# LUP-LuftbildUmweltPlanung/UNet

Measured on AMD Instinct MI355X. Metric: 512x512 tiles/sec fwd+bwd (4-ch->5-class U-Net), higher is better.
Workload: dtype f32

## Files before the change

include/unet_hip.h:

```cpp
#ifndef UNET_HIP_H
#define UNET_HIP_H

#include <stddef.h>
#include <stdint.h>

#ifdef __cplusplus
extern "C" {
#endif

#define UNET_OK 0
#define UNET_E_BADARG (-1)
#define UNET_E_UNSUPPORTED (-2)
#define UNET_E_HIP (-3)

#define UNET_ABI_VERSION 8

int unet_abi_version(void);
const char* unet_last_error(void);

#define UNET_F32 0
#define UNET_BF16 1
typedef uint16_t unet_bf16;

typedef struct {
    int conv_splitk;
    int mfma_shape;
    int f32_big_tile;
    int bf16_big_tile;
    int t256_tiles_per_wg;
    int t256_sliver;
    int conv1x1_gemm;
    int wgrad_mfma_shape;
    int wgrad_bf16_k4;
    int wgrad_1x1;
    int wgrad_narrow;
    int plan_batch;
    int wgrad_wgs;
    int conv_smallcin;
    int conv_head1x1;
} unet_tuning;
void unet_tuning_default(unet_tuning* t);


#define UNET_CONV_RELU 1
#define UNET_CONV_MASK 4

#define UNET_CONV_FWD 0
#define UNET_CONV_DGRAD 1

typedef struct {
    const float* x; int x_cs, x_co;
    const float* wp;
    const float* bias;
    const float* res; int res_cs, res_co;
    const float* mask; int mask_cs, mask_co;
    float* y; int y_cs, y_co;
    int N, IH, IW, Cin;
    int OH, OW, Cout;
    int ks, stride;
    int kind, flags;
    float* colsum;
    float* colsumsq;
    int cout_begin, cout_count;
    long long wp_img_stride;
    int dtype;
    int y_f32;
    float* splitk_ws;
    size_t splitk_ws_floats;
    const unet_tuning* tuning;
    int pixel_shuffle;
    const void* ps_tail;
    int ps_tail_cs, ps_tail_co;
    int ps_tail_c, ps_tail_at;
} unet_conv_desc;

int unet_conv2d_colsum_rows(const unet_conv_desc* d);
int unet_conv2d(const unet_conv_desc* d, void* stream);
size_t unet_conv2d_splitk_workspace(const unet_conv_desc* d);
int unet_conv2d_variant(const unet_conv_desc* d);
size_t unet_pack_weights_size(int Cout, int Cin, int ks, int mode);
int unet_pack_weights(const float* w, float* wp, int Cout, int Cin, int ks, int mode, void* stream);
int unet_pack_weights_strided(const float* w, long long so, long long sr, float* wp, int O, int R, void* stream);
size_t unet_pack_weights_size_bf16(int Cout, int Cin, int ks, int mode);
int unet_pack_weights_bf16(const float* w, unet_bf16* wp, int Cout, int Cin, int ks, int mode, void* stream);
typedef struct {
    const float* w;
    void* wp;
    int Cout, Cin, ks, mode;
    const float* out_scale;
} unet_pack_job;
size_t unet_pack_batch_table_bytes(int njobs);
int unet_pack_batch_build(const unet_pack_job* jobs, int njobs, int dtype, void* table_host, unsigned* total_blocks);
int unet_pack_batch_run(const void* table_dev, int njobs, unsigned total_blocks, int dtype, void* stream);
typedef struct {
    const float* x; int x_cs, x_co;
    const float* dy; int dy_cs, dy_co;
    float* dw;
    float* dbias;
    int N, IH, IW, Cin, OH, OW, Cout, ks, stride;
    float* workspace; size_t workspace_floats;
    int accumulate;
    int dtype;
    const unet_tuning* tuning;
} unet_wgrad_desc;
size_t unet_conv2d_wgrad_workspace(const unet_wgrad_desc* d);
int unet_conv2d_wgrad(const unet_wgrad_desc* d, void* stream);

int unet_bn_stats_rows(long long P);
int unet_bn_stats(const float* x, int x_cs, int x_co, long long P, int C, float* partial, void* stream);
int unet_bn_finalize(const float* psum, const float* psumsq, int rows, long long count, int C,
                     const float* gamma, const float* beta, float* running_mean, float* running_var,
                     float momentum, float eps,
                     float* scale, float* shift, float* save_mean, float* save_invstd, long long* batches_tracked, void* stream);
int unet_bn_eval_coeffs(const float* gamma, const float* beta, const float* running_mean, const float* running_var,
                        float eps, int C, float* scale, float* shift, void* stream);
int unet_affine_act(const float* x, int x_cs, int x_co, const float* scale, const float* shift,
                    const float* x2, int x2_cs, int x2_co, const float* scale2, const float* shift2,
                    float* y, int y_cs, int y_co, long long P, int C, int relu, void* stream);
int unet_bn_bwd_reduce(const float* dout, int d_cs, int d_co, const float* out, int o_cs, int o_co,
                       const float* x, int x_cs, int x_co, const float* mean, const float* invstd,
                       long long P, int C, float* partial, void* stream);
int unet_bn_bwd_finalize(const float* partial, int rows, long long count, int C,
                         float* dgamma, float* dbeta, float* c1, float* c2, void* stream);
int unet_bn_bwd_apply(const float* dout, int d_cs, int d_co, const float* out, int o_cs, int o_co,
                      const float* x, int x_cs, int x_co, const float* mean, const float* invstd,
                      const float* gamma, const float* c1, const float* c2,
                      float* dx, int dx_cs, int dx_co, float* gout, int g_cs, int g_co, int g_accumulate,
                      long long P, int C, void* stream);

int unet_maxpool3x3s2(const float* x, int x_cs, int x_co, float* y, int y_cs, int y_co, uint8_t* idx,
                      int N, int IH, int IW, int C, int OH, int OW, void* stream);
int unet_maxpool3x3s2_bwd(const float* dy, int dy_cs, int dy_co, const uint8_t* idx, float* dx, int dx_cs, int dx_co,
                          int N, int IH, int IW, int C, int OH, int OW, int accumulate, void* stream);
int unet_avgpool2_ceil(const float* x, int x_cs, int x_co, float* y, int y_cs, int y_co,
                       int N, int IH, int IW, int C, int OH, int OW, void* stream);
int unet_avgpool2_ceil_bwd(const float* dy, int dy_cs, int dy_co, float* dx, int dx_cs, int dx_co,
                           int N, int IH, int IW, int C, int OH, int OW, int accumulate, void* stream);

int unet_shuffle_blur(const float* yc, int yc_cs, int yc_co, float* X, int X_cs, int X_co,
                      int N, int h, int w, int Cu, int do_blur, void* stream);
int unet_shuffle_blur_bwd(const float* dX, int dX_cs, int dX_co, const float* yc, int yc_cs, int yc_co,
                          float* dyc, int dyc_cs, int dyc_co, int N, int h, int w, int Cu, int do_blur, void* stream);
int unet_shuffle_bwd_xmask(const float* dX, int dX_cs, int dX_co, const float* X, int X_cs, int X_co,
                           float* dyc, int dyc_cs, int dyc_co, int N, int h, int w, int Cu, void* stream);
int unet_resize_nearest(const float* x, int x_cs, int x_co, float* y, int y_cs, int y_co,
                        int N, int IH, int IW, int OH, int OW, int C, void* stream);
int unet_resize_nearest_bwd(const float* dy, int dy_cs, int dy_co, float* dx, int dx_cs, int dx_co,
                            int N, int IH, int IW, int OH, int OW, int C, void* stream);
int unet_nchw_to_nhwc(const float* x, float* y, int y_cs, int y_co, int N, int C, int H, int W, void* stream);
int unet_nhwc_to_nchw(const float* x, int x_cs, int x_co, float* y, int N, int C, int H, int W, void* stream);
int unet_copy_slice(const float* x, int x_cs, int x_co, float* y, int y_cs, int y_co, long long P, int C,
                    int accumulate, void* stream);
int unet_relu_mask(const float* g, int g_cs, int g_co, const float* ref, int r_cs, int r_co,
                   float* y, int y_cs, int y_co, long long P, int C, void* stream);
int unet_colsum(const float* x, int x_cs, int x_co, long long P, int C, float* out, float* workspace, void* stream);
size_t unet_colsum_workspace(long long P, int C);
int unet_dot(const float* x, int x_cs, int x_co, const float* y, int y_cs, int y_co, long long P, int C, float* out,
             float* workspace, void* stream);

size_t unet_ce_workspace(long long P);
int unet_ce_fwd(const float* z, int z_cs, int z_co, const int64_t* target, const float* weight, long long P, int C,
                float* loss , float* denom , float* workspace, void* stream);
int unet_ce_fwd_parts(const float* z, int z_cs, int z_co, const int64_t* target, const float* weight, long long P, int C,
                      float* numden , float* workspace, void* stream);
int unet_ce_bwd(const float* z, int z_cs, int z_co, const int64_t* target, const float* weight, long long P, int C,
                const float* denom, float gscale, float* dz, int dz_cs, int dz_co, void* stream);
int unet_ce_fwd_pw(const float* z, int z_cs, int z_co, const int64_t* target, const float* pixel_weight, long long P, int C,
                   float* loss , float* denom , float* workspace, void* stream);
int unet_ce_fwd_parts_pw(const float* z, int z_cs, int z_co, const int64_t* target, const float* pixel_weight, long long P, int C,
                         float* numden , float* workspace, void* stream);
int unet_ce_bwd_pw(const float* z, int z_cs, int z_co, const int64_t* target, const float* pixel_weight, long long P, int C,
                   const float* denom, float gscale, float* dz, int dz_cs, int dz_co, void* stream);
int unet_focal_fwd(const float* z, int z_cs, int z_co, const int64_t* target, const float* weight, long long P, int C, float gamma,
                   float* loss , float* workspace, void* stream);
int unet_focal_bwd(const float* z, int z_cs, int z_co, const int64_t* target, const float* weight, long long P, int C, float gamma,
                   float gscale, float* dz, int dz_cs, int dz_co, void* stream);
size_t unet_dice_workspace(int B, long long HW, int C);
int unet_dice_fwd(const float* z, int z_cs, int z_co, const int64_t* target, int B, long long HW, int C, float smooth, int square_in_union,
                  long long mean_div, float* loss , float* coef , float* workspace, void* stream);
int unet_dice_bwd(const float* z, int z_cs, int z_co, const int64_t* target, int B, long long HW, int C, int square_in_union,
                  const float* coef, float gscale, float* dz, int dz_cs, int dz_co, void* stream);
size_t unet_combined_workspace(int B, long long HW, int C);
int unet_combined_fwd(const float* z, int z_cs, int z_co, const int64_t* target, const float* weight, int B, long long HW, int C, float gamma,
                      float smooth, int square_in_union, long long mean_div, float* terms , float* coef , float* workspace,
                      void* stream);
int unet_combined_bwd(const float* z, int z_cs, int z_co, const int64_t* target, const float* weight, int B, long long HW, int C, float gamma,
                      int square_in_union, const float* coef, float fscale, float dscale, float* dz, int dz_cs, int dz_co, void* stream);
int unet_regloss_fwd(const float* z, int z_cs, int z_co, const float* target, long long P, int kind, float beta,
                     float* loss , float* workspace, void* stream);
int unet_regloss_bwd(const float* z, int z_cs, int z_co, const float* target, long long P, int kind, float beta, float gscale,
                     float* dz, int dz_cs, int dz_co, void* stream);
int unet_softmax_argmax(const float* z, int z_cs, int z_co, int N, int H, int W, int C,
                        float* probs_nchw , int64_t* argmax , void* stream);

int unet_row_softmax(const float* x, int x_cs, int x_co, float* y, int y_cs, int y_co, long long P, int C, void* stream);
int unet_row_softmax_bwd(const float* y, int y_cs, int y_co, const float* dy, int dy_cs, int dy_co,
                         float* dx, int dx_cs, int dx_co, long long P, int C, void* stream);

int unet_adam_step(float* p, const float* g, float* m, float* v, const uint8_t* code, long long n,
                   const float* lr , float mom, float sqr_mom, float eps, float wd, int step,
                   float grad_scale, void* stream);

int unet_adam_hyper_floats(void);
int unet_adam_fill_hyper(float* hyper_host, const float* lr , float mom, float sqr_mom, float eps, float wd, int step,
                         float grad_scale);
int unet_adam_step_dev(float* p, const float* g, float* m, float* v, const uint8_t* code, long long n,
                       const float* hyper_dev, void* stream);

int unet_mosaic_accumulate(const float* probs_nchw, int C, int th, int tw, float* mosaic ,
                           int32_t* count , int MH, int MW, int y0, int x0, void* stream);
int unet_mosaic_finalize(float* mosaic, const int32_t* count, int C, int MH, int MW, uint8_t* argmax, void* stream);
int unet_mosaic_accumulate_weighted(const float* probs_nchw, int C, int th, int tw, const float* wy, const float* wx, float* mosaic,
                                    int32_t* count, float* wsum, int MH, int MW, int y0, int x0, void* stream);

#define UNET_RASTER_U8 0
#define UNET_RASTER_U16 1
#define UNET_RASTER_I16 2
#define UNET_RASTER_I32 3
#define UNET_RASTER_F32 4
int unet_raster_nodata_zero(void* raster, int rtype, int bands, long long pixels, double nodata, void* stream);
int unet_window_nonzero(const void* raster, int rtype, int bands, long long band_stride, int row_stride, const int32_t* windows, int n,
                        int th, int tw, unsigned long long* counts, void* stream);
int unet_window_gather(const void* src, int rtype, int bands, long long src_stride, long long band_stride, int row_stride,
                       const int32_t* windows, int n, int th, int tw, int div255_twice, void* x, int x_cs, int x_co, int dtype, void* stream);
int unet_mosaic_accumulate_windows(const float* z, int z_cs, int z_co, int C, int th, int tw, const int32_t* windows, int n, int origin_y,
                                   int origin_x, int mode, float* mosaic, int32_t* count, int MH, int MW, int row_lo, int row_hi,
                                   void* stream);
int unet_mosaic_finalize_rows(float* mosaic, const int32_t* count, int C, int MH, int MW, int row0, int nrows, uint8_t* argmax,
                              const float* fill_host, void* stream);
int unet_mosaic_accumulate_windows_weighted(const float* z, int z_cs, int z_co, int C, int th, int tw, const int32_t* windows, int n,
                                            int origin_y, int origin_x, int mode, float* mosaic, int32_t* count, int MH, int MW, int row_lo,
                                            int row_hi, const float* wy, const float* wx, float* wsum, void* stream);
int unet_mosaic_finalize_rows_weighted(float* mosaic, const int32_t* count, const float* wsum, int C, int MH, int MW, int row0, int nrows,
                                       uint8_t* argmax, const float* fill_host, void* stream);
// ... 122 lines not shown
```

unet_amd/_lib.py:

```python
from __future__ import annotations

import ctypes as C
import os
import re
from pathlib import Path

import torch

_HERE = Path(__file__).resolve().parent
LIB_PATH = _HERE / "lib" / "libunet_hip.so"
HEADER = _HERE.parent / "include" / "unet_hip.h"

UNET_OK = 0
CONV_RELU = 1
CONV_MASK = 4
CONV_FWD = 0
CONV_DGRAD = 1
F32 = 0
BF16 = 1

c_float_p = C.POINTER(C.c_float)
vp = C.c_void_p


class Tuning(C.Structure):
    _fields_ = [(n, C.c_int) for n in ("conv_splitk", "mfma_shape", "f32_big_tile", "bf16_big_tile", "t256_tiles_per_wg", "t256_sliver",
                                       "conv1x1_gemm", "wgrad_mfma_shape", "wgrad_bf16_k4", "wgrad_1x1", "wgrad_narrow", "plan_batch", "wgrad_wgs", "conv_smallcin", "conv_head1x1")]

    @classmethod
    def default(cls, **over) -> "Tuning":
        t = cls()
        lib.unet_tuning_default(C.byref(t))
        for k, v in over.items():
            if k not in dict(cls._fields_):
                raise KeyError(f"unet_tuning has no field {k!r}")
            setattr(t, k, int(v))
        return t


class ConvDesc(C.Structure):
    _fields_ = [
        ("x", vp), ("x_cs", C.c_int), ("x_co", C.c_int),
        ("wp", vp),
        ("bias", vp),
        ("res", vp), ("res_cs", C.c_int), ("res_co", C.c_int),
        ("mask", vp), ("mask_cs", C.c_int), ("mask_co", C.c_int),
        ("y", vp), ("y_cs", C.c_int), ("y_co", C.c_int),
        ("N", C.c_int), ("IH", C.c_int), ("IW", C.c_int), ("Cin", C.c_int),
        ("OH", C.c_int), ("OW", C.c_int), ("Cout", C.c_int),
        ("ks", C.c_int), ("stride", C.c_int),
        ("kind", C.c_int), ("flags", C.c_int),
        ("colsum", vp),
        ("colsumsq", vp),
        ("cout_begin", C.c_int), ("cout_count", C.c_int),
        ("wp_img_stride", C.c_longlong),
        ("dtype", C.c_int), ("y_f32", C.c_int),
        ("splitk_ws", vp), ("splitk_ws_floats", C.c_size_t),
        ("tuning", C.POINTER(Tuning)),
        ("pixel_shuffle", C.c_int),
        ("ps_tail", vp), ("ps_tail_cs", C.c_int), ("ps_tail_co", C.c_int), ("ps_tail_c", C.c_int), ("ps_tail_at", C.c_int),
    ]


class WgradDesc(C.Structure):
    _fields_ = [
        ("x", vp), ("x_cs", C.c_int), ("x_co", C.c_int),
        ("dy", vp), ("dy_cs", C.c_int), ("dy_co", C.c_int),
        ("dw", vp),
        ("dbias", vp),
        ("N", C.c_int), ("IH", C.c_int), ("IW", C.c_int), ("Cin", C.c_int),
        ("OH", C.c_int), ("OW", C.c_int), ("Cout", C.c_int), ("ks", C.c_int), ("stride", C.c_int),
        ("workspace", vp), ("workspace_floats", C.c_size_t),
        ("accumulate", C.c_int),
        ("dtype", C.c_int),
        ("tuning", C.POINTER(Tuning)),
    ]


PIXEL_MAX_PROGS, PIXEL_MAX_OPS, PIXEL_MAX_RECTS, BLUR_MAX_IMAGES, BLUR_MAX_KSIZE = 8, 8, 32, 16, 31
PIXEL_BRIGHTNESS_CONTRAST, PIXEL_GAMMA, PIXEL_GAUSS_NOISE, PIXEL_FILL_RECTS, PIXEL_CHANNEL_DROP, PIXEL_CHANNEL_PERMUTE = 1, 2, 3, 4, 5, 6
PIXEL_PER_CHANNEL = 0x100


class PixelOp(C.Structure):
    _fields_ = [("code", C.c_uint32), ("u0", C.c_uint32), ("u1", C.c_uint32), ("f0", C.c_float), ("f1", C.c_float)]


class PixelProg(C.Structure):
    _fields_ = [("image", C.c_uint32), ("nops", C.c_uint32), ("nrects", C.c_uint32), ("reserved", C.c_uint32),
                ("ops", PixelOp * PIXEL_MAX_OPS), ("rects", (C.c_uint16 * 4) * PIXEL_MAX_RECTS)]


class RectSet(C.Structure):
    _fields_ = [("image", C.c_uint32), ("nrects", C.c_uint32), ("rects", (C.c_uint16 * 4) * PIXEL_MAX_RECTS)]


FIELD_MAX_IMAGES, FIELD_MAX_CELLS, ELASTIC_MAX_IMAGES, ELASTIC_MAX_KSIZE = 16, 16, 64, 401
FIELD_DENSE, FIELD_GRID, FIELD_OPTICAL = 0, 1, 2


class FieldImage(C.Structure):
    _fields_ = [("fired", C.c_int32), ("pre", C.c_float * 6), ("optical", C.c_float * 3), ("nodes", (C.c_float * (FIELD_MAX_CELLS + 1)) * 2)]


class ElasticImage(C.Structure):
    _fields_ = [("key0", C.c_uint32), ("key1", C.c_uint32), ("alpha", C.c_float), ("fired", C.c_int32), ("same_dxdy", C.c_int32)]


class PackJob(C.Structure):
    _fields_ = [("w", vp), ("wp", vp), ("Cout", C.c_int), ("Cin", C.c_int), ("ks", C.c_int), ("mode", C.c_int), ("out_scale", vp)]


def declared_symbols() -> list[str]:
    txt = HEADER.read_text()
    txt = re.sub(r"/\*.*?\*/", "", txt, flags=re.S)
    return sorted(set(re.findall(r"\b(unet_[a-z0-9_]+)\s*\(", txt)))


def _load() -> C.CDLL:
    if not LIB_PATH.exists():
        raise ImportError(
            f"{LIB_PATH} not found: build it with `python -m unet_amd.build` (hipcc --offload-arch=gfx950). "
            "The MI355X path has no CPU fallback.")
    lib = C.CDLL(str(LIB_PATH))
    missing = [s for s in declared_symbols() if not hasattr(lib, s)]
    if missing:
        raise ImportError(f"libunet_hip.so does not export: {missing}")
    return lib


lib = _load()

i, ll, f, sz = C.c_int, C.c_longlong, C.c_float, C.c_size_t
_sig = {
    "unet_abi_version": (i, []),
    "unet_last_error": (C.c_char_p, []),
    "unet_conv2d_colsum_rows": (i, [C.POINTER(ConvDesc)]),
    "unet_conv2d": (i, [C.POINTER(ConvDesc), vp]),
    "unet_conv2d_variant": (i, [C.POINTER(ConvDesc)]),
    "unet_conv2d_splitk_workspace": (sz, [C.POINTER(ConvDesc)]),
    "unet_tuning_default": (None, [C.POINTER(Tuning)]),
    "unet_pack_batch_table_bytes": (sz, [i]),
    "unet_pack_batch_build": (i, [C.POINTER(PackJob), i, i, vp, C.POINTER(C.c_uint)]),
    "unet_pack_batch_run": (i, [vp, i, C.c_uint, i, vp]),
    "unet_pack_weights_size": (sz, [i, i, i, i]),
    "unet_pack_weights": (i, [vp, vp, i, i, i, i, vp]),
    "unet_pack_weights_strided": (i, [vp, ll, ll, vp, i, i, vp]),
    "unet_row_softmax": (i, [vp, i, i, vp, i, i, ll, i, vp]),
    "unet_row_softmax_bwd": (i, [vp, i, i, vp, i, i, vp, i, i, ll, i, vp]),
    "unet_conv2d_wgrad_workspace": (sz, [C.POINTER(WgradDesc)]),
    "unet_conv2d_wgrad": (i, [C.POINTER(WgradDesc), vp]),
    "unet_bn_stats_rows": (i, [ll]),
    "unet_bn_stats": (i, [vp, i, i, ll, i, vp, vp]),
    "unet_bn_finalize": (i, [vp, vp, i, ll, i, vp, vp, vp, vp, f, f, vp, vp, vp, vp, vp, vp]),
    "unet_bn_eval_coeffs": (i, [vp, vp, vp, vp, f, i, vp, vp, vp]),
    "unet_affine_act": (i, [vp, i, i, vp, vp, vp, i, i, vp, vp, vp, i, i, ll, i, i, vp]),
    "unet_bn_bwd_reduce": (i, [vp, i, i, vp, i, i, vp, i, i, vp, vp, ll, i, vp, vp]),
    "unet_bn_bwd_finalize": (i, [vp, i, ll, i, vp, vp, vp, vp, vp]),
    "unet_bn_bwd_apply": (i, [vp, i, i, vp, i, i, vp, i, i, vp, vp, vp, vp, vp, vp, i, i, vp, i, i, i, ll, i, vp]),
    "unet_maxpool3x3s2": (i, [vp, i, i, vp, i, i, vp, i, i, i, i, i, i, vp]),
    "unet_maxpool3x3s2_bwd": (i, [vp, i, i, vp, vp, i, i, i, i, i, i, i, i, i, vp]),
    "unet_avgpool2_ceil": (i, [vp, i, i, vp, i, i, i, i, i, i, i, i, vp]),
    "unet_avgpool2_ceil_bwd": (i, [vp, i, i, vp, i, i, i, i, i, i, i, i, i, vp]),
    "unet_shuffle_blur": (i, [vp, i, i, vp, i, i, i, i, i, i, i, vp]),
    "unet_shuffle_blur_bwd": (i, [vp, i, i, vp, i, i, vp, i, i, i, i, i, i, i, vp]),
    "unet_shuffle_bwd_xmask": (i, [vp, i, i, vp, i, i, vp, i, i, i, i, i, i, vp]),
    "unet_resize_nearest": (i, [vp, i, i, vp, i, i, i, i, i, i, i, i, vp]),
    "unet_resize_nearest_bwd": (i, [vp, i, i, vp, i, i, i, i, i, i, i, i, vp]),
    "unet_nchw_to_nhwc": (i, [vp, vp, i, i, i, i, i, i, vp]),
    "unet_nhwc_to_nchw": (i, [vp, i, i, vp, i, i, i, i, vp]),
    "unet_copy_slice": (i, [vp, i, i, vp, i, i, ll, i, i, vp]),
    "unet_relu_mask": (i, [vp, i, i, vp, i, i, vp, i, i, ll, i, vp]),
    "unet_colsum": (i, [vp, i, i, ll, i, vp, vp, vp]),
    "unet_colsum_workspace": (sz, [ll, i]),
    "unet_dot": (i, [vp, i, i, vp, i, i, ll, i, vp, vp, vp]),
    "unet_ce_workspace": (sz, [ll]),
    "unet_ce_fwd": (i, [vp, i, i, vp, vp, ll, i, vp, vp, vp, vp]),
    "unet_ce_fwd_parts": (i, [vp, i, i, vp, vp, ll, i, vp, vp, vp]),
    "unet_ce_bwd": (i, [vp, i, i, vp, vp, ll, i, vp, f, vp, i, i, vp]),
    "unet_ce_fwd_pw": (i, [vp, i, i, vp, vp, ll, i, vp, vp, vp, vp]),
    "unet_ce_fwd_parts_pw": (i, [vp, i, i, vp, vp, ll, i, vp, vp, vp]),
    "unet_ce_bwd_pw": (i, [vp, i, i, vp, vp, ll, i, vp, f, vp, i, i, vp]),
    "unet_focal_fwd": (i, [vp, i, i, vp, vp, ll, i, f, vp, vp, vp]),
    "unet_focal_bwd": (i, [vp, i, i, vp, vp, ll, i, f, f, vp, i, i, vp]),
    "unet_dice_workspace": (sz, [i, ll, i]),
    "unet_dice_fwd": (i, [vp, i, i, vp, i, ll, i, f, i, ll, vp, vp, vp, vp]),
    "unet_dice_bwd": (i, [vp, i, i, vp, i, ll, i, i, vp, f, vp, i, i, vp]),
    "unet_combined_workspace": (sz, [i, ll, i]),
    "unet_combined_fwd": (i, [vp, i, i, vp, vp, i, ll, i, f, f, i, ll, vp, vp, vp, vp]),
    "unet_combined_bwd": (i, [vp, i, i, vp, vp, i, ll, i, f, i, vp, f, f, vp, i, i, vp]),
    "unet_regloss_fwd": (i, [vp, i, i, vp, ll, i, f, vp, vp, vp]),
    "unet_regloss_bwd": (i, [vp, i, i, vp, ll, i, f, f, vp, i, i, vp]),
    "unet_softmax_argmax": (i, [vp, i, i, i, i, i, i, vp, vp, vp]),
    "unet_adam_step": (i, [vp, vp, vp, vp, vp, ll, c_float_p, f, f, f, f, i, f, vp]),
    "unet_adam_hyper_floats": (i, []),
    "unet_adam_fill_hyper": (i, [c_float_p, c_float_p, f, f, f, f, i, f]),
    "unet_adam_step_dev": (i, [vp, vp, vp, vp, vp, ll, vp, vp]),
    "unet_mosaic_accumulate": (i, [vp, i, i, i, vp, vp, i, i, i, i, vp]),
    "unet_mosaic_finalize": (i, [vp, vp, i, i, i, vp, vp]),
    "unet_raster_nodata_zero": (i, [vp, i, i, ll, C.c_double, vp]),
    "unet_window_nonzero": (i, [vp, i, i, ll, i, vp, i, i, i, vp, vp]),
    "unet_window_gather": (i, [vp, i, i, ll, ll, i, vp, i, i, i, i, vp, i, i, i, vp]),
    "unet_mosaic_accumulate_windows": (i, [vp, i, i, i, i, i, vp, i, i, i, i, vp, vp, i, i, i, i, vp]),
    "unet_tiff_lzw_decode": (ll, [vp, ll, vp, ll]),
    "unet_tiff_packbits_decode": (ll, [vp, ll, vp, ll]),
    "unet_mosaic_finalize_rows": (i, [vp, vp, i, i, i, i, i, vp, c_float_p, vp]),
    "unet_tiles_stage": (i, [vp, i, i, i, i, i, i, C.c_ulonglong, C.c_ulonglong, vp, vp]),
    "unet_mask_stage": (i, [vp, i, i, i, i, C.c_ulonglong, C.c_ulonglong, vp, i, vp]),
    "unet_dice_counts": (i, [vp, vp, ll, i, vp, vp]),
    "unet_warp_affine": (i, [vp, vp, i, i, i, i, c_float_p, i, i, f, vp]),
    "unet_warp_affine_mask": (i, [vp, vp, i, i, i, i, c_float_p, i, C.c_double, vp]),
    "unet_warp_field": (i, [vp, vp, i, i, i, i, i, C.POINTER(FieldImage), vp, i, i, i, i, f, vp]),
    "unet_warp_field_mask": (i, [vp, vp, i, i, i, i, i, C.POINTER(FieldImage), vp, i, i, i, C.c_double, vp]),
    "unet_elastic_field": (i, [vp, vp, i, i, i, C.POINTER(ElasticImage), c_float_p, i, vp]),
    "unet_pixel_ops": (i, [vp, i, i, i, i, vp, i, vp]),
    "unet_fill_rects_mask": (i, [vp, i, i, i, i, vp, i, C.c_double, vp]),
    "unet_blur_separable": (i, [vp, vp, i, i, i, i, C.POINTER(C.c_int), c_float_p, vp]),
    "unet_window_gather_oriented": (i, [vp, i, i, ll, ll, i, vp, i, i, i, i, vp, i, i, i, i, vp]),
    "unet_nchw_to_nhwc_oriented": (i, [vp, vp, i, i, i, i, i, i, i, i, vp]),
    "unet_tta_accumulate": (i, [vp, i, i, i, i, i, i, i, i, i, vp, i, i, vp, vp, vp]),
    "unet_mosaic_accumulate_weighted": (i, [vp, i, i, i, vp, vp, vp, vp, vp, i, i, i, i, vp]),
    "unet_mosaic_accumulate_windows_weighted": (i, [vp, i, i, i, i, i, vp, i, i, i, i, vp, vp, i, i, i, i, vp, vp, vp, vp]),
    "unet_mosaic_finalize_rows_weighted": (i, [vp, vp, vp, i, i, i, i, i, vp, c_float_p, vp]),
    "unet_cc_tile_shape": (None, [C.POINTER(C.c_int), C.POINTER(C.c_int)]),
    "unet_cc_label": (i, [vp, i, i, i, vp, vp, vp]),
    "unet_cc_sizes": (i, [vp, i, i, vp, vp]),
    "unet_sieve_round": (i, [vp, vp, i, i, i, ll, i, vp, vp, vp, vp, vp]),
    "unet_majority_filter": (i, [vp, vp, i, i, i, i, vp]),
    "unet_postprocess_counters": (i, [vp, C.POINTER(C.c_int32), vp]),
    "unet_edt_workspace": (sz, [i, i, i]),
    "unet_border_edt": (i, [vp, i, i, i, i, i, vp, vp, vp]),
    "unet_border_weight": (i, [vp, vp, vp, i, f, C.c_double, ll, vp, vp]),
}
for _n in ("bn_stats", "affine_act", "bn_bwd_reduce", "bn_bwd_apply", "maxpool3x3s2", "maxpool3x3s2_bwd", "avgpool2_ceil",
           "avgpool2_ceil_bwd", "shuffle_blur", "shuffle_blur_bwd", "shuffle_bwd_xmask", "resize_nearest", "resize_nearest_bwd", "nchw_to_nhwc", "copy_slice", "ce_bwd", "ce_bwd_pw", "focal_bwd",
           "dice_bwd", "combined_bwd"):
    _sig[f"unet_{_n}_bf16"] = _sig[f"unet_{_n}"]
for _n in ("pack_weights_strided", "row_softmax", "row_softmax_bwd", "relu_mask", "dot"):
    _sig[f"unet_{_n}_bf16"] = _sig[f"unet_{_n}"]
_sig["unet_sa_fused_supported"] = (i, [i, i])
_sig["unet_sa_pack_elems"] = (sz, [i, i])
_sig["unet_sa_pack_bf16"] = (i, [vp, i, i, i, i, i, vp, vp])
_sig["unet_sa_fwd_bf16"] = (i, [vp, i, i, i, i, i, vp, vp, i, i, vp, vp])
_sig["unet_sa_rowdot_bf16"] = (i, [vp, i, i, vp, i, i, i, i, i, vp, vp])
_sig["unet_sa_bwd_bf16"] = (i, [vp, i, i, i, i, i, vp, i, i, vp, vp, vp, vp, vp, vp, vp])
_sig["unet_cast_slice_bf16"] = (i, [vp, i, i, vp, i, i, ll, i, vp])
_sig["unet_pack_weights_size_bf16"] = _sig["unet_pack_weights_size"]
_sig["unet_pack_weights_bf16"] = _sig["unet_pack_weights"]

for _name, (_res, _args) in _sig.items():
    _fn = getattr(lib, _name)
    _fn.restype = _res
    _fn.argtypes = _args

_undeclared = [s for s in declared_symbols() if s not in _sig]
if _undeclared:
    raise ImportError(f"ctypes signatures missing for: {_undeclared}")

if lib.unet_abi_version() != 8:
    raise ImportError("libunet_hip.so ABI version mismatch; rebuild with `python -m unet_amd.build --force`")


class UnetHipError(RuntimeError):
    pass


def check(rc: int, what: str = "") -> None:
    if rc != UNET_OK:
        msg = lib.unet_last_error().decode(errors="replace")
        raise UnetHipError(f"{what}: rc={rc}: {msg}")
```

unet_amd/csrc/conv_bf16.hip:

```cpp

#include "conv_common.h"

namespace {

using namespace unetconv;

typedef __bf16 bf16x8 __attribute__((ext_vector_type(8)));
typedef __bf16 bf16x4 __attribute__((ext_vector_type(4)));
typedef float f32x4 __attribute__((ext_vector_type(4)));
typedef unsigned short u16;

__device__ __forceinline__ f32x4 ld_bf16x4(const u16* p) {
    const uint2 u = *reinterpret_cast<const uint2*>(p);
    return (f32x4){__uint_as_float(u.x << 16), __uint_as_float(u.x & 0xffff0000u), __uint_as_float(u.y << 16), __uint_as_float(u.y & 0xffff0000u)};
}
__device__ __forceinline__ void st_bf16x4(u16* p, f32x4 v) {
    const bf16x4 h = {(__bf16)v[0], (__bf16)v[1], (__bf16)v[2], (__bf16)v[3]};
    *reinterpret_cast<uint2*>(p) = __builtin_bit_cast(uint2, h);
}

template <int TW, int MT, int NT, int WM, int WN, int HIT>
__global__ __launch_bounds__(WM* WN * 64, HIT == 4 ? 3 : 2) void conv_bf16_kernel(const KArgs a, const int y_f32) {
    constexpr int BM = WM * MT * 32, BN = WN * NT * 32, TH = BM / TW, NTH = WM * WN * 64;
    constexpr int M16 = 2 * MT, N16 = 2 * NT;
// ... 634 lines not shown
#pragma unroll
                        for (int m = 0; m < MH; ++m) v[m] += ld4(resb + (size_t)pidx[m] * a.res_cs + cc);
                    }
                    if (relu) {
#pragma unroll
                        for (int m = 0; m < MH; ++m)
#pragma unroll
                            for (int q = 0; q < 4; ++q) v[m][q] = fmaxf(v[m][q], 0.f);
                    }
                    if (maskb != nullptr) {
#pragma unroll
                        for (int m = 0; m < MH; ++m) {
                            const f32x4 mv = ld4(maskb + (size_t)pidx[m] * a.mask_cs + cc);
#pragma unroll
                            for (int q = 0; q < 4; ++q) v[m][q] = mv[q] > 0.f ? v[m][q] : 0.f;
                        }
                    }
                    float* yb = a.y + (a.cps ? (size_t)blockIdx.y * a.slab : (size_t)0) + img_pix * a.y_cs + a.y_co;
#pragma unroll
                    for (int m = 0; m < MH; ++m)
                        if (cvalid && pval[m]) *reinterpret_cast<f32x4*>(yb + (size_t)pidx[m] * a.y_cs + c4) = v[m];
                }
            }
        } else {
            f32x4 bvn[NL];
#pragma unroll
            for (int n = 0; n < NL; ++n) {
                const int c4 = n0c + TILE_COL(n) + 4 * kq;
                bvn[n] = (f32x4){0.f, 0.f, 0.f, 0.f};
                if (a.bias != nullptr) {
                    if (c4 + 3 < a.Cout) bvn[n] = *reinterpret_cast<const f32x4*>(a.bias + c4);
                    else {
#pragma unroll
                        for (int q = 0; q < 4; ++q) bvn[n][q] = (c4 + q < a.Cout) ? a.bias[c4 + q] : 0.f;
                    }
                }
            }
            int pidx2[2][MH / 2];
            bool pval2[2][MH / 2];
#pragma unroll
            for (int h = 0; h < 2; ++h)
#pragma unroll
                for (int j = 0; j < MH / 2; ++j) {
                    const int pix = (wm * M16 + ((h * MH + 2 * j + (kq & 1)) ^ (r * MH))) * 16 + l15;
                    const int oy = oy0c + pix / TW, ox = ox0c + pix % TW;
                    pval2[h][j] = oy < a.OH && ox < a.OW;
                    pidx2[h][j] = pval2[h][j] ? (oy * a.OW + ox) : 0;
                }
#pragma unroll
            for (int h = 0; h < 2; ++h) {
#pragma unroll
            for (int n = 0; n < NL; ++n) {
                if (n == NF && h != 0) continue;
                const int c8 = n0c + TILE_COL(n) + 8 * (kq >> 1);
                const int cc8 = c8 < a.n_end ? c8 : 0;
#pragma unroll
                for (int m = 0; m < MH; ++m) acc[h * MH + m][n] += bvn[n];
                if (resb != nullptr) {
                    uint4 rr[MH / 2];
#pragma unroll
                    for (int j = 0; j < MH / 2; ++j) rr[j] = *reinterpret_cast<const uint4*>(resb + (size_t)pidx2[h][j] * a.res_cs + cc8);
#pragma unroll
                    for (int j = 0; j < MH / 2; ++j) {
                        const auto s0 = __builtin_amdgcn_permlane16_swap(rr[j].x, rr[j].z, false, false);
                        const auto s1 = __builtin_amdgcn_permlane16_swap(rr[j].y, rr[j].w, false, false);
                        acc[h * MH + 2 * j][n] += unpack(s0[0], s1[0]);
                        acc[h * MH + 2 * j + 1][n] += unpack(s0[1], s1[1]);
                    }
                }
                if (relu) {
#pragma unroll
                    for (int m = 0; m < MH; ++m)
#pragma unroll
                        for (int q = 0; q < 4; ++q) acc[h * MH + m][n][q] = fmaxf(acc[h * MH + m][n][q], 0.f);
                }
                if (maskb != nullptr) {
                    uint4 rr[MH / 2];
#pragma unroll
                    for (int j = 0; j < MH / 2; ++j) rr[j] = *reinterpret_cast<const uint4*>(maskb + (size_t)pidx2[h][j] * a.mask_cs + cc8);
#pragma unroll
                    for (int j = 0; j < MH / 2; ++j) {
                        const auto s0 = __builtin_amdgcn_permlane16_swap(rr[j].x, rr[j].z, false, false);
                        const auto s1 = __builtin_amdgcn_permlane16_swap(rr[j].y, rr[j].w, false, false);
                        const f32x4 m0 = unpack(s0[0], s1[0]), m1 = unpack(s0[1], s1[1]);
#pragma unroll
                        for (int q = 0; q < 4; ++q) {
                            acc[h * MH + 2 * j][n][q] = m0[q] > 0.f ? acc[h * MH + 2 * j][n][q] : 0.f;
                            acc[h * MH + 2 * j + 1][n][q] = m1[q] > 0.f ? acc[h * MH + 2 * j + 1][n][q] : 0.f;
                        }
                    }
                }
            }
            }
            const __amdgpu_buffer_rsrc_t rsy = __builtin_amdgcn_make_buffer_rsrc(reinterpret_cast<u16*>(a.y) + img_pix * a.y_cs + a.y_co, 0,
                                                                                  __builtin_amdgcn_readfirstlane(a.OH * a.OW * a.y_cs * 2), 0x00020000);
#pragma unroll
            for (int h = 0; h < 2; ++h) {
#pragma unroll
            for (int j = 0; j < MH / 2; ++j) {
#pragma unroll
                for (int n = 0; n < NL; ++n) {
                    if (n == NF && h != 0) continue;
                    const int c8 = n0c + TILE_COL(n) + 8 * (kq >> 1);
                    const bool cvalid8 = c8 < a.n_end;
                    const f32x4 va = acc[h * MH + 2 * j][n], vb = acc[h * MH + 2 * j + 1][n];
                    const bf16x4 x_ = {(__bf16)va[0], (__bf16)va[1], (__bf16)va[2], (__bf16)va[3]};
                    const bf16x4 y_ = {(__bf16)vb[0], (__bf16)vb[1], (__bf16)vb[2], (__bf16)vb[3]};
                    const uint2 xu = __builtin_bit_cast(uint2, x_), yu = __builtin_bit_cast(uint2, y_);
                    const auto s0 = __builtin_amdgcn_permlane16_swap(xu.x, yu.x, false, false);
                    const auto s1 = __builtin_amdgcn_permlane16_swap(xu.y, yu.y, false, false);
                    typedef unsigned v4u __attribute__((ext_vector_type(4)));
                    const unsigned vo = (cvalid8 && pval2[h][j]) ? (unsigned)(pidx2[h][j] * a.y_cs + c8) * 2u : OOB;
                    __builtin_amdgcn_raw_buffer_store_b128((v4u){s0[0], s1[0], s0[1], s1[1]}, rsy, (int)vo, 0, 0);
                }
            }
            }
        }
#ifdef UNET_STAMPS
        ste_ += STAMP() - se0_;
#endif
        if (!more_tiles) break;
#pragma unroll
        for (int m = 0; m < M16; ++m)
#pragma unroll
            for (int n = 0; n < N16; ++n) acc[m][n] = (f32x4){0.f, 0.f, 0.f, 0.f};
    }
    wait_cnt<0, true>(b0, hreg);
#undef T256_MFMA
#undef T256_LOAD_HALO
#undef T256_STORE_HALO
#undef T256_STORE_HALO_T
#undef T256_SETUP
#undef MOFF
#undef TOFF
#undef TILE_COL
#ifdef UNET_STAMPS
    if (g_stamps != nullptr && tid == 0) {
        asm volatile("s_waitcnt vmcnt(0)" ::: "memory");
        unsigned long long* o = g_stamps + (size_t)blockIdx.x * 24;
#pragma unroll
        for (int i = 0; i < 10; ++i) o[8 + i] = stwt_[i];
        o[0] = st0_; o[1] = st1_; o[2] = stl_; o[3] = STAMP(); o[4] = stw_; o[5] = stb_; o[6] = (unsigned long long)__builtin_amdgcn_s_memrealtime();
        o[7] = 1; o[18] = ste_; o[19] = (unsigned long long)(tend - wg * tpw);
    }
#endif
}

#ifdef UNET_STAMPS
extern "C" int unet_debug_set_stamps(unsigned long long* buf) {
    return hipMemcpyToSymbol(HIP_SYMBOL(g_stamps), &buf, sizeof(buf)) == hipSuccess ? 0 : -3;
}
#endif


template <int NTOT, int TW, typename T, bool SLV = false>
int launch_t256n(const Plan& p, int y_f32, hipStream_t st) {
    const int ntiles = p.k.mtiles * p.k.ntn;
    int tpw = p.tune.t256_tiles_per_wg > 0 ? p.tune.t256_tiles_per_wg : ntiles / 2048;
    tpw = tpw < 1 ? 1 : (tpw > 16 ? 16 : tpw);
    dim3 grid = p.grid;
    grid.x = (unsigned)unet::roundup(unet::cdiv(ntiles, tpw), 8);
    return launch_big_lds<conv_bf16_t256_kernel<NTOT, TW, T, SLV>>(grid, dim3(256), (size_t)2 * (256 / TW + 2) * (TW + 2) * T256_ROWB, st, p.k, y_f32, tpw, p.bn);
}

template <int TW, typename T>
int launch_t256_tiles(const Plan& p, int tiles, int y_f32, hipStream_t st) {
    switch (tiles) {
        case 8: return launch_t256n<8, TW, T>(p, y_f32, st);
        case 7: return launch_t256n<7, TW, T>(p, y_f32, st);
        case 6: return launch_t256n<6, TW, T>(p, y_f32, st);
        case 5: return launch_t256n<5, TW, T>(p, y_f32, st);
        case 4: return launch_t256n<4, TW, T>(p, y_f32, st);
        case 3: return launch_t256n<3, TW, T>(p, y_f32, st);
        case 2: return launch_t256n<2, TW, T>(p, y_f32, st);
        case 1: return launch_t256n<1, TW, T>(p, y_f32, st);
    }
    unet::set_error("conv: %d channel tiles in the 256-pixel tile", tiles);
    return (int)UNET_E_UNSUPPORTED;
}

template <typename T>
int launch_t256(const Plan& p, int y_f32, hipStream_t st) {
    const int cols = p.k.n_end - p.k.n_base, nblk = p.k.ntn, full = p.bn / 16;
    const int last_tiles = (cols - (nblk - 1) * p.bn + 15) / 16;
    auto one = [&](const Plan& q, int tiles) {
        if constexpr (sizeof(T) == 4) {
            const int last_w = (q.k.n_end - q.k.n_base) - (q.k.ntn - 1) * q.bn - (tiles - 1) * 16;
            if (q.tune.t256_sliver && tiles == 7 && q.tw == 32 && last_w >= 1 && last_w <= 4) return launch_t256n<7, 32, T, true>(q, y_f32, st);
        }
        if (q.tw == 32) return launch_t256_tiles<32, T>(q, tiles, y_f32, st);
        if (q.tw == 16) return launch_t256_tiles<16, T>(q, tiles, y_f32, st);
        unet::set_error("conv: tile width %d in the 256-pixel tile", q.tw);
        return (int)UNET_E_UNSUPPORTED;
    };
    if (nblk == 1 || last_tiles == full) return one(p, nblk == 1 ? last_tiles : full);
    Plan q = p;
    q.k.ntn = nblk - 1; q.k.n_end = p.k.n_base + (nblk - 1) * p.bn;
    int rc = one(q, full);
    if (rc != UNET_OK) return rc;
    q = p;
    q.k.ntn = 1; q.k.n_base = p.k.n_base + (nblk - 1) * p.bn;
    return one(q, last_tiles);
}

__global__ void pack_weights_bf16_kernel(const float* __restrict__ w, u16* __restrict__ wp, int Cout, int Cin, int T, int mode, int nchunks,
                                         int outPad, size_t total) {
    for (size_t i = (size_t)blockIdx.x * blockDim.x + threadIdx.x; i < total; i += (size_t)gridDim.x * blockDim.x)
        wp[i] = __builtin_bit_cast(u16, (__bf16)bf16_image_value(w, Cout, Cin, T, mode, nchunks, outPad, i));
}

__global__ void pack_weights_strided_bf16_kernel(const u16* __restrict__ w, long long so, long long sr, u16* __restrict__ wp, int O, int R,
                                                 int outPad, size_t total) {
    for (size_t i = (size_t)blockIdx.x * blockDim.x + threadIdx.x; i < total; i += (size_t)gridDim.x * blockDim.x) {
        const int rr = (int)(i & 31);
        const size_t j = i >> 5;
        const int o = (int)(j % outPad), r = (int)(j / outPad) * 32 + rr;
        wp[i] = (o < O && r < R) ? w[(long long)o * so + (long long)r * sr] : (u16)0;
    }
}

struct IgemmBf16 {
    template <int TW, int MT, int NT, int WM, int WN, int HIT>
    static int launch(const Plan& p, int y_f32, hipStream_t st) {
        return launch_big_lds<conv_bf16_kernel<TW, MT, NT, WM, WN, HIT>>(p.grid, dim3(WM * WN * 64), p.lds_bytes, st, p.k, y_f32);
    }
};

}

int unetconv::conv_generic_bf16(const Plan& p, int y_f32, hipStream_t st) { return launch_generic<IgemmBf16>(p, y_f32, st); }

int unetconv::conv_t256(const Plan& p0, int dtype, int y_f32, hipStream_t st) {
    Plan p = p0;
    p.k.sliver = p.k.taps[0].dy[0] > 0 ? 1 : 0;
    if (dtype == UNET_BF16) return launch_t256<unsigned short>(p, y_f32, st);
    p.k.fold = 0;
    return launch_t256<float>(p, 1, st);
}

extern "C" size_t unet_pack_weights_size_bf16(int Cout, int Cin, int ks, int mode) {
    const int T = ks * ks;
    const int red = mode == 1 ? Cout : Cin, out = mode == 1 ? Cin : Cout;
    return bf16_image_elems(red, unet::roundup(out, 128), T);
}

extern "C" int unet_pack_weights_strided_bf16(const unet_bf16* w, long long so, long long sr, unet_bf16* wp, int O, int R, void* stream) {
    UNET_CHECK_ARG(w && wp && O > 0 && R > 0, "pack_weights_strided_bf16: bad args");
    const int outPad = unet::roundup(O, 128);
    const size_t total = bf16_image_elems(R, outPad, 1);
    hipLaunchKernelGGL(pack_weights_strided_bf16_kernel, dim3(unet::ew_grid((long long)total, 256)), dim3(256), 0, (hipStream_t)stream, w, so, sr, wp,
                       O, R, outPad, total);
    UNET_CHECK_LAUNCH();
    return UNET_OK;
}

extern "C" int unet_pack_weights_bf16(const float* w, unet_bf16* wp, int Cout, int Cin, int ks, int mode, void* stream) {
    UNET_CHECK_ARG(w && wp, "pack_weights_bf16: null pointer");
    UNET_CHECK_ARG((ks == 1 || ks == 3) && (mode == 0 || mode == 1 || (mode == 2 && ks == 1 && Cout % 64 == 0)) && Cout > 0 && Cin > 0, "pack_weights_bf16: bad args");
    const int T = ks * ks;
    const int red = mode == 1 ? Cout : Cin, out = mode == 1 ? Cin : Cout;
    const int nchunks = unet::cdiv(red, KCB), outPad = unet::roundup(out, 128);
    const size_t total = bf16_image_elems(red, outPad, T);
    hipLaunchKernelGGL(pack_weights_bf16_kernel, dim3(unet::ew_grid((long long)total, 256)), dim3(256), 0, (hipStream_t)stream, w, wp, Cout,
                       Cin, T, mode, nchunks, outPad, total);
    UNET_CHECK_LAUNCH();
    return UNET_OK;
}
```

unet_amd/csrc/conv_common.h:

```cpp
#pragma once
#include "common.h"

namespace unetconv {

constexpr int KC = 16;
constexpr int LDK = 20;
constexpr int KCB = 32;
constexpr int LDKB = 24;

struct TapSet {
    int n;
    int min_dy, min_dx;
    int ext_y, ext_x;
    int py, px;
    signed char dy[9], dx[9], widx[9];
    unsigned long long dpack, wpack;
};

struct KArgs {
    const float* x; const float* wp; const float* bias; const float* res; const float* mask;
    float* y; float* colsum; float* colsumsq;
    int x_cs, x_co, res_cs, res_co, mask_cs, mask_co, y_cs, y_co;
    int N, IH, IW, Cin, Cin4;
    int OH, OW, Cout;
    int S, OS, TSH, TSW, tiles_y, tiles_x, ntn;
    int nchunks, coutPad, flags, mtiles;
    int n_base, n_end;
    int fold;
    int sliver;
    const float* wsl;
    long long wp_stride;
    int cps;
    long long slab;
    TapSet taps[4];
};

__host__ __device__ inline bool f32_sliver(int out) { return out >= 16 && (out & 15) != 0 && (out & 15) <= 4; }
__host__ __device__ inline size_t f32_image_elems(int red, int out, int T) {
    const int nchunks = (red + 15) / 16, outPad = (out + 127) / 128 * 128;
    return (size_t)T * nchunks * outPad * 16 + (f32_sliver(out) ? (size_t)T * nchunks * 64 : 0);
}
__device__ inline float f32_sliver_value(const float* __restrict__ w, int Cout, int Cin, int T, int mode, int nchunks, size_t i) {
    const int pos = (int)(i & 15), j = (int)((i >> 4) & 3);
    const int chunk = (int)((i >> 6) % nchunks), tap = (int)((i >> 6) / nchunks);
    const int red = mode == 0 ? Cin : Cout, out = mode == 0 ? Cout : Cin;
    const bool tail = (red & 15) != 0 && chunk == nchunks - 1;
    const int r = chunk * 16 + (tail ? (4 * (pos & 3) + (pos >> 2)) : pos);
    const int o = (out & ~15) + j;
    if (r >= red || o >= out) return 0.f;
    return mode == 0 ? w[((size_t)o * Cin + r) * T + tap] : w[((size_t)r * Cin + o) * T + tap];
}

__host__ __device__ inline bool bf16_fold_tail(int red, int T) { return T == 9 && (red & 31) != 0 && (red & 31) <= 8; }
__host__ __device__ inline size_t bf16_image_elems(int red, int out_pad, int T) {
    return (size_t)(T * ((red + 31) / 32) + (bf16_fold_tail(red, T) ? 3 : 0)) * out_pad * 32;
}
__host__ __device__ inline int ps_filter_of(int q, int Cout) { const int nf = Cout >> 2; return 4 * (q % nf) + q / nf; }
__device__ inline float bf16_image_value(const float* __restrict__ w, int Cout, int Cin, int T, int mode, int nchunks, int outPad, size_t i) {
    const int rr = (int)(i & 31);
    size_t j = i >> 5;
    const int o = (int)(j % outPad);
    const int slab = (int)(j / outPad);
    const int red = mode == 1 ? Cout : Cin;
    int tap, r;
    if (slab < T * nchunks) {
        tap = slab / nchunks;
        r = (slab % nchunks) * 32 + rr;
    } else {
        tap = 4 * (slab - T * nchunks) + (rr >> 3);
        r = (nchunks - 1) * 32 + (rr & 7);
        if (tap >= T) return 0.f;
    }
    if (r >= red) return 0.f;
    if (mode == 2) return o < Cout ? w[((size_t)ps_filter_of(o, Cout) * Cin + r) * T + tap] : 0.f;
    if (mode == 0) return o < Cout ? w[((size_t)o * Cin + r) * T + tap] : 0.f;
    return o < Cin ? w[((size_t)r * Cin + o) * T + tap] : 0.f;
}

typedef float v4f __attribute__((ext_vector_type(4)));
typedef unsigned long long u64;
__device__ __forceinline__ u64 sgpr_ptr(const void* p) {
    const u64 b = reinterpret_cast<u64>(p);
    const unsigned lo = __builtin_amdgcn_readfirstlane((unsigned)b), hi = __builtin_amdgcn_readfirstlane((unsigned)(b >> 32));
    return ((u64)hi << 32) | lo;
}
template <int TSTR, int N>
__device__ __forceinline__ void gld_b(v4f (&d)[N], unsigned voff, const char* p) {
    static_assert(N == 2 || N == 4, "operand-B tiles per wave");
    const u64 s0 = sgpr_ptr(p);
    if constexpr (N == 2) {
        asm volatile("s_nop 4\n\tglobal_load_dwordx4 %0, %2, %3\n\tglobal_load_dwordx4 %1, %2, %3 offset:%4"
                     : "=&v"(d[0]), "=&v"(d[1]) : "v"(voff), "s"(s0), "n"(TSTR));
    } else {
        const u64 s1 = sgpr_ptr(p + 2 * TSTR);
        asm volatile("s_nop 4\n\tglobal_load_dwordx4 %0, %4, %5\n\tglobal_load_dwordx4 %1, %4, %5 offset:%7\n\t"
                     "global_load_dwordx4 %2, %4, %6\n\tglobal_load_dwordx4 %3, %4, %6 offset:%7"
                     : "=&v"(d[0]), "=&v"(d[1]), "=&v"(d[2]), "=&v"(d[3]) : "v"(voff), "s"(s0), "s"(s1), "n"(TSTR));
    }
}
template <int TSTR, int N>
__device__ __forceinline__ void gld_bl(v4f (&d)[N], unsigned voff, unsigned voff_last, const char* p) {
    static_assert(N == 2 || N == 4, "operand-B tiles per wave");
    const u64 s0 = sgpr_ptr(p);
    if constexpr (N == 2) {
        asm volatile("s_nop 4\n\tglobal_load_dwordx4 %0, %2, %4\n\tglobal_load_dwordx4 %1, %3, %4 offset:%5"
                     : "=&v"(d[0]), "=&v"(d[1]) : "v"(voff), "v"(voff_last), "s"(s0), "n"(TSTR));
    } else {
        const u64 s1 = sgpr_ptr(p + 2 * TSTR);
        asm volatile("s_nop 4\n\tglobal_load_dwordx4 %0, %4, %6\n\tglobal_load_dwordx4 %1, %4, %6 offset:%8\n\t"
                     "global_load_dwordx4 %2, %4, %7\n\tglobal_load_dwordx4 %3, %5, %7 offset:%8"
                     : "=&v"(d[0]), "=&v"(d[1]), "=&v"(d[2]), "=&v"(d[3]) : "v"(voff), "v"(voff_last), "s"(s0), "s"(s1), "n"(TSTR));
    }
}
template <int N>
__device__ __forceinline__ void gld_halo(v4f (&h)[N], const unsigned (&vo)[N], const void* p, bool fetch) {
    static_assert(N == 4 || N == 6 || N == 10, "halo items per thread");
    const u64 sb = sgpr_ptr(p);
    const u64 on = sgpr_ptr(reinterpret_cast<const void*>(fetch ? ~0ull : 0ull));
    u64 sv;
    if constexpr (N == 4) {
        asm volatile("s_and_saveexec_b64 %[sv], %[on]\n\ts_nop 4\n\t"
                     "global_load_dwordx4 %[h0], %[o0], %[sb]\n\tglobal_load_dwordx4 %[h1], %[o1], %[sb]\n\t"
                     "global_load_dwordx4 %[h2], %[o2], %[sb]\n\tglobal_load_dwordx4 %[h3], %[o3], %[sb]\n\t"
                     "s_mov_b64 exec, %[sv]"
                     : [h0] "+v"(h[0]), [h1] "+v"(h[1]), [h2] "+v"(h[2]), [h3] "+v"(h[3]), [sv] "=&s"(sv)
                     : [o0] "v"(vo[0]), [o1] "v"(vo[1]), [o2] "v"(vo[2]), [o3] "v"(vo[3]), [sb] "s"(sb), [on] "s"(on)
                     : "scc");
    } else if constexpr (N == 6) {
        asm volatile("s_and_saveexec_b64 %[sv], %[on]\n\ts_nop 4\n\t"
                     "global_load_dwordx4 %[h0], %[o0], %[sb]\n\tglobal_load_dwordx4 %[h1], %[o1], %[sb]\n\t"
                     "global_load_dwordx4 %[h2], %[o2], %[sb]\n\tglobal_load_dwordx4 %[h3], %[o3], %[sb]\n\t"
                     "global_load_dwordx4 %[h4], %[o4], %[sb]\n\tglobal_load_dwordx4 %[h5], %[o5], %[sb]\n\t"
                     "s_mov_b64 exec, %[sv]"
                     : [h0] "+v"(h[0]), [h1] "+v"(h[1]), [h2] "+v"(h[2]), [h3] "+v"(h[3]), [h4] "+v"(h[4]), [h5] "+v"(h[5]), [sv] "=&s"(sv)
                     : [o0] "v"(vo[0]), [o1] "v"(vo[1]), [o2] "v"(vo[2]), [o3] "v"(vo[3]), [o4] "v"(vo[4]), [o5] "v"(vo[5]), [sb] "s"(sb), [on] "s"(on)
                     : "scc");
    } else {
        asm volatile("s_and_saveexec_b64 %[sv], %[on]\n\ts_nop 4\n\t"
                     "global_load_dwordx4 %[h0], %[o0], %[sb]\n\tglobal_load_dwordx4 %[h1], %[o1], %[sb]\n\t"
                     "global_load_dwordx4 %[h2], %[o2], %[sb]\n\tglobal_load_dwordx4 %[h3], %[o3], %[sb]\n\t"
                     "global_load_dwordx4 %[h4], %[o4], %[sb]\n\tglobal_load_dwordx4 %[h5], %[o5], %[sb]\n\t"
                     "global_load_dwordx4 %[h6], %[o6], %[sb]\n\tglobal_load_dwordx4 %[h7], %[o7], %[sb]\n\t"
                     "global_load_dwordx4 %[h8], %[o8], %[sb]\n\tglobal_load_dwordx4 %[h9], %[o9], %[sb]\n\t"
                     "s_mov_b64 exec, %[sv]"
                     : [h0] "+v"(h[0]), [h1] "+v"(h[1]), [h2] "+v"(h[2]), [h3] "+v"(h[3]), [h4] "+v"(h[4]), [h5] "+v"(h[5]),
                       [h6] "+v"(h[6]), [h7] "+v"(h[7]), [h8] "+v"(h[8]), [h9] "+v"(h[9]), [sv] "=&s"(sv)
                     : [o0] "v"(vo[0]), [o1] "v"(vo[1]), [o2] "v"(vo[2]), [o3] "v"(vo[3]), [o4] "v"(vo[4]), [o5] "v"(vo[5]),
                       [o6] "v"(vo[6]), [o7] "v"(vo[7]), [o8] "v"(vo[8]), [o9] "v"(vo[9]), [sb] "s"(sb), [on] "s"(on)
                     : "scc");
    }
}
__device__ __forceinline__ void gld_halo4_sl(v4f (&h)[4], const unsigned (&vo)[4], const void* p, bool fetch, v4f& sl, unsigned vosl,
                                             const void* psl, u64 msl) {
    const u64 sb = sgpr_ptr(p), sbl = sgpr_ptr(psl);
    const u64 on = sgpr_ptr(reinterpret_cast<const void*>(fetch ? ~0ull : 0ull));
    const u64 ms = sgpr_ptr(reinterpret_cast<const void*>(msl));
    u64 sv;
    asm volatile("s_and_saveexec_b64 %[sv], %[on]\n\ts_nop 4\n\t"
                 "global_load_dwordx4 %[h0], %[o0], %[sb]\n\tglobal_load_dwordx4 %[h1], %[o1], %[sb]\n\t"
                 "global_load_dwordx4 %[h2], %[o2], %[sb]\n\tglobal_load_dwordx4 %[h3], %[o3], %[sb]\n\t"
                 "s_and_b64 exec, exec, %[ms]\n\ts_nop 0\n\t"
                 "global_load_dwordx4 %[sl], %[osl], %[sbl]\n\t"
                 "s_mov_b64 exec, %[sv]"
                 : [h0] "+v"(h[0]), [h1] "+v"(h[1]), [h2] "+v"(h[2]), [h3] "+v"(h[3]), [sl] "+v"(sl), [sv] "=&s"(sv)
                 : [o0] "v"(vo[0]), [o1] "v"(vo[1]), [o2] "v"(vo[2]), [o3] "v"(vo[3]), [osl] "v"(vosl), [sb] "s"(sb), [sbl] "s"(sbl),
                   [on] "s"(on), [ms] "s"(ms)
                 : "scc");
}
__device__ __forceinline__ void wait_loads_sl(v4f (&b)[4], v4f (&h)[4], v4f& sl) {
    asm volatile("s_waitcnt vmcnt(0)" : "+v"(b[0]), "+v"(b[1]), "+v"(b[2]), "+v"(b[3]), "+v"(h[0]), "+v"(h[1]), "+v"(h[2]), "+v"(h[3]), "+v"(sl));
}
template <int NB, int NH>
__device__ __forceinline__ void wait_loads(v4f (&b)[NB], v4f (&h)[NH]) {
    static_assert((NB == 2 || NB == 4) && (NH == 4 || NH == 6 || NH == 10), "register groups");
#define UNET_H4 "+v"(h[0]), "+v"(h[1]), "+v"(h[2]), "+v"(h[3])
#define UNET_H6 UNET_H4, "+v"(h[4]), "+v"(h[5])
#define UNET_H10 UNET_H4, "+v"(h[4]), "+v"(h[5]), "+v"(h[6]), "+v"(h[7]), "+v"(h[8]), "+v"(h[9])
    if constexpr (NB == 4 && NH == 6) asm volatile("s_waitcnt vmcnt(0)" : "+v"(b[0]), "+v"(b[1]), "+v"(b[2]), "+v"(b[3]), UNET_H6);
    else if constexpr (NB == 2 && NH == 6) asm volatile("s_waitcnt vmcnt(0)" : "+v"(b[0]), "+v"(b[1]), UNET_H6);
    else if constexpr (NB == 2 && NH == 4) asm volatile("s_waitcnt vmcnt(0)" : "+v"(b[0]), "+v"(b[1]), UNET_H4);
    else if constexpr (NB == 2) asm volatile("s_waitcnt vmcnt(0)" : "+v"(b[0]), "+v"(b[1]), UNET_H10);
    else if constexpr (NH == 4) asm volatile("s_waitcnt vmcnt(0)" : "+v"(b[0]), "+v"(b[1]), "+v"(b[2]), "+v"(b[3]), UNET_H4);
    else asm volatile("s_waitcnt vmcnt(0)" : "+v"(b[0]), "+v"(b[1]), "+v"(b[2]), "+v"(b[3]), UNET_H10);
#undef UNET_H4
#undef UNET_H6
#undef UNET_H10
}

struct Plan {
    KArgs k;
    int tw, bm, bn, hit, nparity, mf, max_hpix;
    size_t lds_bytes;
    dim3 grid;
    int splits, cp;
    size_t ws_floats;
    unet_tuning tune;
};


__device__ __forceinline__ float ld_act(const float* p) { return *p; }
__device__ __forceinline__ float ld_act(const unsigned short* p) { return __uint_as_float((unsigned)*p << 16); }
__device__ __forceinline__ void st_act(float* p, float v) { *p = v; }
__device__ __forceinline__ void st_act(unsigned short* p, float v) { *p = __builtin_bit_cast(unsigned short, (__bf16)v); }

template <auto Kern, typename... Args>
int launch_big_lds(dim3 grid, dim3 block, size_t lds_bytes, hipStream_t st, const Args&... args) {
    static unsigned long long configured = 0;
    if (unet::first_use_on_device(&configured))
        UNET_CHECK_HIP(hipFuncSetAttribute((const void*)Kern, hipFuncAttributeMaxDynamicSharedMemorySize, 160 * 1024));
    hipLaunchKernelGGL(Kern, grid, block, lds_bytes, st, args...);
    UNET_CHECK_LAUNCH();
    return UNET_OK;
}

template <typename K, int TW, int HIT>
int launch_bn(const Plan& p, int y_f32, hipStream_t st) {
    if (p.bm == 64) {
        if (p.bn == 64) return K::template launch<TW, 1, 1, 2, 2, HIT>(p, y_f32, st);
        return K::template launch<TW, 1, 2, 2, 2, HIT>(p, y_f32, st);
    }
    switch (p.bn) {
        case 32: return K::template launch<TW, 1, 1, 4, 1, HIT>(p, y_f32, st);
        case 64: return K::template launch<TW, 2, 1, 2, 2, HIT>(p, y_f32, st);
        default: return K::template launch<TW, 2, 2, 2, 2, HIT>(p, y_f32, st);
    }
}
template <typename K, int HIT>
int launch_tw(const Plan& p, int y_f32, hipStream_t st) {
    switch (p.tw) {
        case 32: return launch_bn<K, 32, HIT>(p, y_f32, st);
        case 16: return launch_bn<K, 16, HIT>(p, y_f32, st);
        default: return launch_bn<K, 8, HIT>(p, y_f32, st);
    }
}
template <typename K>
int launch_generic(const Plan& p, int y_f32, hipStream_t st) {
    if (p.bm == 256 || p.hit == 6) {
        unet::set_error("conv: inconsistent plan (the 256-pixel tile / halo item count 6 on the generic kernels)");
        return UNET_E_UNSUPPORTED;
    }
    return p.hit == 10 ? launch_tw<K, 10>(p, y_f32, st) : launch_tw<K, 4>(p, y_f32, st);
}

int conv_generic_f32(const Plan& p, hipStream_t st);
int conv_generic_bf16(const Plan& p, int y_f32, hipStream_t st);
int conv_t256(const Plan& p, int dtype, int y_f32, hipStream_t st);
int splitk_reduce(const unet_conv_desc* d, const Plan& p, hipStream_t st);
bool conv_smallk_applies(const unet_conv_desc* d);
int conv_smallk(const unet_conv_desc* d, hipStream_t st);
bool conv_smallcin_applies(const unet_conv_desc* d);
int conv_smallcin(const unet_conv_desc* d, hipStream_t st);
bool conv_head1x1_applies(const unet_conv_desc* d);
int conv_head1x1(const unet_conv_desc* d, hipStream_t st);
bool conv_gemm1x1_applies(const unet_conv_desc* d);
int conv_gemm1x1(const unet_conv_desc* d, hipStream_t st);
int conv_gemm1x1_ps_check(const unet_conv_desc* d);

}
```

unet_amd/csrc/conv_dispatch.hip:

```cpp
#include <stdlib.h>

#include "conv_common.h"

namespace unetconv {
static int env_int(const char* name, int dflt) {
    const char* e = getenv(name);
    return (e != nullptr && e[0] != 0) ? atoi(e) : dflt;
}
const unet_tuning& tuning_defaults() {
    static const unet_tuning t = [] {
        unet_tuning v;
        v.conv_splitk = env_int("UNET_CONV_SPLITK", 1);
        v.mfma_shape = 16;
        v.f32_big_tile = 1;
        v.bf16_big_tile = 1;
        v.t256_tiles_per_wg = 0;
        v.t256_sliver = env_int("UNET_T256_SLIVER", 1);
        v.conv1x1_gemm = env_int("UNET_CONV1X1_GEMM", 0);
        v.wgrad_mfma_shape = 32;
        v.wgrad_bf16_k4 = 1;
        v.wgrad_1x1 = 1;
        v.wgrad_narrow = 1;
        v.plan_batch = 0;
        v.wgrad_wgs = env_int("UNET_WGRAD_WGS", 0);
        v.conv_smallcin = env_int("UNET_CONV_SMALLCIN", 1);
        v.conv_head1x1 = env_int("UNET_CONV_HEAD1X1", 1);
        return v;
    }();
    return t;
}
}

extern "C" void unet_tuning_default(unet_tuning* t) {
    if (t != nullptr) *t = unetconv::tuning_defaults();
}

namespace {

using namespace unetconv;

int make_plan(const unet_conv_desc* d, Plan* p, int kc, int vec, int mf, int big_tile, int splitk, int plan_batch) {
    UNET_CHECK_ARG(d != nullptr, "conv: null desc");
    UNET_CHECK_ARG(d->x && d->wp && d->y, "conv: null tensor pointer");
    UNET_CHECK_ARG(d->ks == 1 || d->ks == 3, "conv: ks must be 1 or 3 (got %d)", d->ks);
    UNET_CHECK_ARG(d->stride == 1 || d->stride == 2, "conv: stride must be 1 or 2 (got %d)", d->stride);
    UNET_CHECK_ARG(!(d->ks == 1 && d->stride != 1), "conv: 1x1 stride 2 unsupported");
    UNET_CHECK_ARG(d->N > 0 && d->IH > 0 && d->IW > 0 && d->OH > 0 && d->OW > 0 && d->Cin > 0 && d->Cout > 0, "conv: bad dims");
    UNET_CHECK_ARG(unet::slice_ok_v(d->x_cs, d->x_co, d->Cin, vec), "conv: bad x slice cs=%d co=%d C=%d", d->x_cs, d->x_co, d->Cin);
    UNET_CHECK_ARG(unet::slice_ok_v(d->y_cs, d->y_co, d->Cout, d->y_f32 ? 4 : vec), "conv: bad y slice cs=%d co=%d C=%d", d->y_cs, d->y_co, d->Cout);
    UNET_CHECK_ARG(unet::aligned16(d->x) && unet::aligned16(d->wp), "conv: x/wp must be 16-byte aligned");
    if (d->res) UNET_CHECK_ARG(unet::slice_ok_v(d->res_cs, d->res_co, d->Cout, vec), "conv: bad res slice");
    if (d->flags & UNET_CONV_MASK) UNET_CHECK_ARG(d->mask && unet::slice_ok_v(d->mask_cs, d->mask_co, d->Cout, vec), "conv: bad mask slice");
    const int pad = (d->ks - 1) / 2;
    if (d->kind == UNET_CONV_FWD) {
        UNET_CHECK_ARG(d->OH == (d->IH + 2 * pad - d->ks) / d->stride + 1 && d->OW == (d->IW + 2 * pad - d->ks) / d->stride + 1,
                       "conv fwd: output dims %dx%d inconsistent with input %dx%d ks %d stride %d", d->OH, d->OW, d->IH, d->IW, d->ks, d->stride);
    } else if (d->kind == UNET_CONV_DGRAD) {
        UNET_CHECK_ARG(d->IH == (d->OH + 2 * pad - d->ks) / d->stride + 1 && d->IW == (d->OW + 2 * pad - d->ks) / d->stride + 1,
                       "conv dgrad: grad dims %dx%d inconsistent with input dims %dx%d", d->IH, d->IW, d->OH, d->OW);
    } else {
        UNET_CHECK_ARG(false, "conv: bad kind %d", d->kind);
    }
    UNET_CHECK_ARG((long long)d->IH * d->IW * d->x_cs < (1ll << 31) && (long long)d->OH * d->OW * d->y_cs < (1ll << 31) &&
                       (long long)d->OH * d->OW * (d->res ? d->res_cs : 1) < (1ll << 31) &&
                       (long long)d->OH * d->OW * ((d->flags & UNET_CONV_MASK) ? d->mask_cs : 1) < (1ll << 31),
                   "conv: image too large for 32-bit in-image offsets");

    KArgs& k = p->k;
    memset(&k, 0, sizeof(k));
    k.x = d->x; k.wp = d->wp; k.bias = d->bias; k.res = d->res; k.mask = (d->flags & UNET_CONV_MASK) ? d->mask : nullptr;
    k.y = d->y; k.colsum = d->colsum; k.colsumsq = d->colsumsq;
    k.x_cs = d->x_cs; k.x_co = d->x_co; k.res_cs = d->res_cs; k.res_co = d->res_co;
    k.mask_cs = d->mask_cs; k.mask_co = d->mask_co; k.y_cs = d->y_cs; k.y_co = d->y_co;
    k.N = d->N; k.IH = d->IH; k.IW = d->IW; k.Cin = d->Cin; k.Cin4 = unet::roundup(d->Cin, vec);
    k.OH = d->OH; k.OW = d->OW; k.Cout = d->Cout;
    const int cols = d->cout_count > 0 ? d->cout_count : d->Cout;
    UNET_CHECK_ARG(d->cout_begin >= 0 && (d->cout_begin & 15) == 0 && d->cout_begin + cols <= d->Cout, "conv: bad cout range [%d,+%d) of %d",
                   d->cout_begin, cols, d->Cout);
    k.n_base = d->cout_begin; k.n_end = d->cout_begin + cols;
    UNET_CHECK_ARG(d->wp_img_stride >= 0 && (d->wp_img_stride & 3) == 0, "conv: bad wp_img_stride");
    k.wp_stride = d->wp_img_stride;
    k.flags = d->flags;
    k.nchunks = unet::cdiv(d->Cin, kc);
    k.coutPad = unet::roundup(d->Cout, 128);
    p->nparity = 1;
    k.S = 1; k.OS = 1; k.TSH = d->OH; k.TSW = d->OW;

    const int T = d->ks * d->ks;
    if (d->kind == UNET_CONV_FWD) {
        k.S = d->stride;
        TapSet& t = k.taps[0];
        t.n = T; t.min_dy = -pad; t.min_dx = -pad; t.ext_y = d->ks; t.ext_x = d->ks; t.py = t.px = 0;
        for (int r = 0; r < d->ks; ++r)
            for (int s = 0; s < d->ks; ++s) {
                const int i = r * d->ks + s;
                t.dy[i] = (signed char)(r - pad); t.dx[i] = (signed char)(s - pad); t.widx[i] = (signed char)i;
            }
    } else if (d->stride == 1) {
        TapSet& t = k.taps[0];
        t.n = T; t.min_dy = -pad; t.min_dx = -pad; t.ext_y = d->ks; t.ext_x = d->ks; t.py = t.px = 0;
        for (int r = 0; r < d->ks; ++r)
            for (int s = 0; s < d->ks; ++s) {
                const int i = r * d->ks + s;
                t.dy[i] = (signed char)(pad - r); t.dx[i] = (signed char)(pad - s); t.widx[i] = (signed char)i;
            }
    } else {
        k.OS = 2; k.TSH = (d->OH + 1) / 2; k.TSW = (d->OW + 1) / 2;
        p->nparity = 4;
        for (int py = 0; py < 2; ++py)
            for (int px = 0; px < 2; ++px) {
                TapSet& t = k.taps[py * 2 + px];
                int rs[2], rdy[2], nr, ss[2], sdx[2], ns;
                if (py == 0) { nr = 1; rs[0] = 1; rdy[0] = 0; } else { nr = 2; rs[0] = 0; rdy[0] = 1; rs[1] = 2; rdy[1] = 0; }
                if (px == 0) { ns = 1; ss[0] = 1; sdx[0] = 0; } else { ns = 2; ss[0] = 0; sdx[0] = 1; ss[1] = 2; sdx[1] = 0; }
                t.n = nr * ns; t.min_dy = 0; t.min_dx = 0; t.ext_y = (py == 0) ? 1 : 2; t.ext_x = (px == 0) ? 1 : 2;
                t.py = py; t.px = px;
                int i = 0;
                for (int a = 0; a < nr; ++a)
                    for (int b = 0; b < ns; ++b, ++i) {
                        t.dy[i] = (signed char)rdy[a]; t.dx[i] = (signed char)sdx[b]; t.widx[i] = (signed char)(rs[a] * 3 + ss[b]);
                    }
            }
    }

    for (int z = 0; z < p->nparity; ++z) {
        TapSet& t = k.taps[z];
        t.dpack = 0; t.wpack = 0;
        for (int i = 0; i < t.n; ++i) {
            const int dyi = t.dy[i] - t.min_dy, dxi = t.dx[i] - t.min_dx;
            UNET_CHECK_ARG(dyi >= 0 && dyi < 4 && dxi >= 0 && dxi < 4 && t.widx[i] >= 0 && t.widx[i] < 16, "conv: tap table out of range");
            t.dpack |= (unsigned long long)(dyi | (dxi << 2)) << (4 * i);
            t.wpack |= (unsigned long long)t.widx[i] << (4 * i);
        }
    }

    p->tw = k.TSW >= 32 ? 32 : (k.TSW >= 16 ? 16 : 8);
    p->bn = cols <= 32 ? 32 : (cols <= 64 ? 64 : 128);
    p->bm = 128;
    p->hit = (k.S == 2) ? 10 : 4;
    p->mf = mf;
    auto blocks = [&](int bm, int bn) {
        const int th_ = bm / p->tw;
        return (long long)(plan_batch > 0 ? plan_batch : d->N) * unet::cdiv(k.TSH, th_) * unet::cdiv(k.TSW, p->tw) * unet::cdiv(cols, bn) * p->nparity;
    };
    p->splits = 1; p->cp = 0; p->ws_floats = 0;
    bool split = false;
    int nb_first = 0;
    if (kc == 16 && big_tile && big_tile != 2 && d->ks == 3 && k.S == 1 && p->nparity == 1 && mf == 16 && d->colsum == nullptr && d->colsumsq == nullptr &&
        (p->tw == 32 || p->tw == 16) && p->bn == 128 && blocks(256, 128) < 256)
        nb_first = blocks(256, 64) >= 256 ? 64 : (blocks(256, 32) >= 256 ? 32 : 0);
    if (nb_first) p->bn = nb_first;
    if (!nb_first && splitk && mf == 16 && p->nparity == 1 && d->colsum == nullptr && d->colsumsq == nullptr && k.nchunks >= 8 && blocks(128, p->bn) < (splitk > 1 ? splitk : (kc == 32 ? 400 : 256))) {
        const int smax = k.nchunks / 2 < 32 ? k.nchunks / 2 : 32;
        if (p->bn >= 64 && blocks(128, p->bn) * smax < 384) {
            p->bm = 64;
            if (p->bn == 128 && blocks(64, 128) * smax < 384) p->bn = 64;
        }
        const long long b = blocks(p->bm, p->bn);
        int sp = (int)((384 + b - 1) / b);
        if (sp > smax) sp = smax;
        if (sp >= 2) {
            split = true;
            k.cps = unet::cdiv(k.nchunks, sp);
            p->splits = unet::cdiv(k.nchunks, k.cps);
            p->cp = unet::roundup(cols, 4);
            k.slab = (long long)d->N * d->OH * d->OW * p->cp;
            p->ws_floats = (size_t)p->splits * k.slab;
        } else {
            p->bm = 128;
            p->bn = cols <= 32 ? 32 : (cols <= 64 ? 64 : 128);
        }
    }
    const bool f32_fit = kc != 16 || (mf == 16 && d->colsum == nullptr && d->colsumsq == nullptr);
    const bool big_ok = big_tile && f32_fit && d->ks == 3 && p->bm == 128 && (p->bn == 128 || big_tile != 2) && (p->tw == 32 || (p->tw == 16 && big_tile != 2)) && k.S == 1 && p->nparity == 1 &&
                        blocks(256, p->bn) >= (big_tile >= 3 ? 64 * (big_tile - 2) : (big_tile == 2 ? 512 : (kc == 16 ? 256 : 64))) &&
                        (long long)d->IH * d->IW * d->x_cs * (kc == 16 ? 4 : 2) < (1ll << 31) - 65536 &&
                        (long long)d->OH * d->OW * d->y_cs * 4 < (1ll << 31) - 65536;
    if (!split && !(big_ok && big_tile != 2) && p->bn >= 64 && blocks(128, p->bn) < 400) {
        p->bm = 64;
        if (p->bn == 128 && blocks(64, 128) < 400) p->bn = 64;
    }
    if (big_ok && p->bm == 128) {
        p->bm = 256;
        p->hit = 6;
    }
    const int th = p->bm / p->tw;
    k.tiles_y = unet::cdiv(k.TSH, th);
    k.tiles_x = unet::cdiv(k.TSW, p->tw);
    k.ntn = unet::cdiv(cols, p->bn);
    UNET_CHECK_ARG(k.n_base + k.ntn * p->bn <= k.coutPad, "conv: cout range leaves the packed filter image");
    UNET_CHECK_ARG((long long)d->IH * d->IW * d->x_cs < (1ll << 31) && (long long)d->OH * d->OW * d->y_cs < (1ll << 31) &&
                   (d->res == nullptr || (long long)d->OH * d->OW * d->res_cs < (1ll << 31)) &&
                   (d->mask == nullptr || (long long)d->OH * d->OW * d->mask_cs < (1ll << 31)),
                   "conv: one image of a tensor exceeds 2^31 elements");
    const long long mtiles_ll = (long long)d->N * k.tiles_y * k.tiles_x;
    UNET_CHECK_ARG(mtiles_ll * k.ntn < (1ll << 31) - 8, "conv: grid too large (%lld pixel tiles x %d channel blocks)", mtiles_ll, k.ntn);
    k.mtiles = (int)mtiles_ll;
    int max_hpix = 0;
    for (int z = 0; z < p->nparity; ++z) {
        const int hh = (th - 1) * k.S + k.taps[z].ext_y, hw = (p->tw - 1) * k.S + k.taps[z].ext_x;
        if (hh * hw > max_hpix) max_hpix = hh * hw;
    }
    UNET_CHECK_ARG(max_hpix * 4 <= p->hit * 256, "conv: halo tile too large (%d pixels)", max_hpix);
    p->max_hpix = max_hpix;
    p->lds_bytes = (size_t)(32 + 2 * max_hpix * LDK + (p->mf == 16 ? 0 : 2 * p->bn * LDK)) * sizeof(float);
    k.sliver = 0; k.wsl = nullptr;
    if (kc == 16 && p->mf == 16 && p->bm == 128 && p->bn == 128 && p->hit == 4 && p->nparity == 1 && f32_sliver(d->Cout) && k.n_end == d->Cout &&
        d->wp_img_stride == 0 && d->colsum == nullptr && d->colsumsq == nullptr && p->splits == 1) {
        k.sliver = 1;
        k.wsl = d->wp + (size_t)T * k.nchunks * k.coutPad * 16;
        p->lds_bytes += (size_t)2 * 9 * 64 * sizeof(float);
    }
    p->grid = dim3((unsigned)unet::roundup((int)((long long)k.mtiles * k.ntn), p->mf == 16 ? 8 : 1), (unsigned)p->splits, (unsigned)p->nparity);
    UNET_CHECK_ARG((long long)k.mtiles * k.ntn < (1ll << 31), "conv: grid too large");
    return UNET_OK;
}

bool splitk_redirect(const unet_conv_desc* d, Plan* p) {
    if (p->splits <= 1) return true;
    if (d->splitk_ws == nullptr || d->splitk_ws_floats < p->ws_floats) return false;
    KArgs& k = p->k;
    k.bias = nullptr; k.res = nullptr; k.mask = nullptr; k.flags = 0;
    k.y = d->splitk_ws - k.n_base;
    k.y_cs = p->cp; k.y_co = 0;
    return true;
}

int plan_f32(const unet_conv_desc* d, Plan* p, int splitk = -1) {
    UNET_CHECK_ARG(d != nullptr, "conv: null desc");
    const unet_tuning t = tuning_of(d->tuning);
    UNET_CHECK_ARG(t.mfma_shape == 16 || t.mfma_shape == 32, "conv: unet_tuning.mfma_shape must be 16 or 32 (start from unet_tuning_default())");
    const int rc = make_plan(d, p, KC, 4, t.mfma_shape, t.f32_big_tile ? 1 : 0, splitk < 0 ? t.conv_splitk : splitk, t.plan_batch);
    p->tune = t;
    return rc;
}
int plan_bf16(const unet_conv_desc* d, Plan* p, int splitk = -1) {
    UNET_CHECK_ARG(d != nullptr, "conv: null desc");
    const unet_tuning t = tuning_of(d->tuning);
    int rc = make_plan(d, p, KCB, 8, 16, t.bf16_big_tile, splitk < 0 ? t.conv_splitk : splitk, t.plan_batch);
    p->tune = t;
    if (rc != UNET_OK) return rc;
    UNET_CHECK_ARG(d->colsum == nullptr && d->colsumsq == nullptr, "conv bf16: column sums are not available in the bf16 kernel");
    p->lds_bytes = (size_t)(32 + 2 * p->max_hpix * LDKB) * sizeof(float);
    p->k.fold = (p->nparity == 1 && p->splits == 1 && bf16_fold_tail(d->Cin, d->ks * d->ks)) ? 1 : 0;
    UNET_CHECK_ARG(d->Cout % 4 == 0 || d->y_co + unet::roundup(d->Cout, 4) <= d->y_cs, "conv bf16: the output slice must own its 4-channel padding");
    UNET_CHECK_ARG(unet::aligned16(d->y) && (!d->res || unet::aligned16(d->res)) && (!d->mask || unet::aligned16(d->mask)),
                   "conv bf16: y/res/mask must be 16-byte aligned");
    return UNET_OK;
}
int plan(const unet_conv_desc* d, Plan* p, int splitk = -1) {
    return d != nullptr && d->dtype == UNET_BF16 ? plan_bf16(d, p, splitk) : plan_f32(d, p, splitk);
}

enum class Family { PixelShuffle, SmallK, SmallCin, Head1x1, Gemm1x1, T256, Generic };

int choose(const unet_conv_desc* d, Family* f, Plan* p) {
    if (d != nullptr && d->pixel_shuffle) {
        *f = Family::PixelShuffle;
        return conv_gemm1x1_ps_check(d);
    }
    int rc = plan(d, p);
    if (rc == UNET_OK && !splitk_redirect(d, p)) rc = plan(d, p, 0);
    if (rc != UNET_OK) return rc;
    if (conv_smallk_applies(d)) *f = Family::SmallK;
    else if (conv_smallcin_applies(d)) *f = Family::SmallCin;
    else if (conv_head1x1_applies(d)) *f = Family::Head1x1;
    else if (conv_gemm1x1_applies(d)) *f = Family::Gemm1x1;
    else *f = p->hit == 6 ? Family::T256 : Family::Generic;
    return UNET_OK;
}

int variant_id(Family f, const Plan& p) {
    switch (f) {
        case Family::PixelShuffle: case Family::Gemm1x1: return 8;
        case Family::SmallK: return 9;
        case Family::SmallCin: return 10;
        case Family::Head1x1: return 11;
        default: break;
    }
    const bool large = p.bm == 256 && p.bn == 128 && p.tw == 32 && (long long)p.k.mtiles * p.k.ntn >= 512;
    return p.tw * 10000 + p.bn * 10 + (p.hit == 10 ? 1 : 0) + (p.bm == 64 ? 5 : 0) + (p.bm == 256 ? (large ? 7 : 6) : 0) + (p.splits > 1 ? 1000000 * p.splits : 0);
}

}

extern "C" int unet_conv2d(const unet_conv_desc* d, void* stream) {
    UNET_CHECK_ARG(d == nullptr || d->pixel_shuffle || d->dtype == UNET_F32 || d->dtype == UNET_BF16, "conv: unknown dtype %d", d->dtype);
    Family f;
    Plan p;
    int rc = choose(d, &f, &p);
    if (rc != UNET_OK) return rc;
    hipStream_t st = (hipStream_t)stream;
    const bool bf = d->dtype == UNET_BF16;
    const int y_f32 = p.splits > 1 ? 1 : d->y_f32;
    switch (f) {
        case Family::PixelShuffle: case Family::Gemm1x1: return conv_gemm1x1(d, st);
        case Family::SmallK: return conv_smallk(d, st);
        case Family::SmallCin: return conv_smallcin(d, st);
        case Family::Head1x1: return conv_head1x1(d, st);
        case Family::T256: rc = conv_t256(p, d->dtype, y_f32, st); break;
        case Family::Generic: rc = bf ? conv_generic_bf16(p, y_f32, st) : conv_generic_f32(p, st); break;
    }
    if (rc != UNET_OK || p.splits <= 1) return rc;
    return splitk_reduce(d, p, st);
}

extern "C" int unet_conv2d_variant(const unet_conv_desc* d) {
    Family f;
    Plan p;
    const int rc = choose(d, &f, &p);
    return rc == UNET_OK ? variant_id(f, p) : rc;
}

extern "C" size_t unet_conv2d_splitk_workspace(const unet_conv_desc* d) {
    Plan p;
    if (d == nullptr || d->pixel_shuffle) return 0;
    return plan(d, &p) == UNET_OK ? p.ws_floats : 0;
}

extern "C" int unet_conv2d_colsum_rows(const unet_conv_desc* d) {
    Plan p;
    const int rc = plan_f32(d, &p, 0);
    if (rc != UNET_OK) return rc;
    const int wm = (p.bn == 32 && p.bm == 128) ? 4 : 2;
    return p.nparity * p.k.mtiles * wm;
}
```

unet_amd/csrc/conv_igemm.hip:

```cpp

#include "conv_common.h"

namespace {

using namespace unetconv;

typedef float f32x16 __attribute__((ext_vector_type(16)));


template <int HIT, int NTH>
__device__ __forceinline__ void ld_halo(float4 (&hreg)[HIT], const int (&goff)[HIT], const float* xb, int c0, int Cin4, int tid) {
#pragma unroll
    for (int it = 0; it < HIT; ++it) {
        const int q = (tid + it * NTH) & 3;
        const bool ok = goff[it] >= 0 && (c0 + 4 * q) < Cin4;
        hreg[it] = ok ? *reinterpret_cast<const float4*>(xb + goff[it] + c0) : make_float4(0.f, 0.f, 0.f, 0.f);
    }
}
template <int HIT, int NTH>
__device__ __forceinline__ void st_halo(const float4 (&hreg)[HIT], float* dst, int hpix4, int tid) {
#pragma unroll
    for (int it = 0; it < HIT; ++it) {
        const int e = tid + it * NTH;
        if (e < hpix4) *reinterpret_cast<float4*>(dst + (e >> 2) * LDK + (e & 3) * 4) = hreg[it];
// ... 794 lines not shown
    static constexpr int VEC = 8;
    __device__ static float w(const unsigned short* wp, int outPad, int tap, int o, int r) { return __uint_as_float((unsigned)wp[((size_t)tap * outPad + o) * 32 + r] << 16); }
};

typedef float f32x2 __attribute__((ext_vector_type(2)));

template <typename T, int PX, int NX>
__global__ __launch_bounds__(256) void conv3x3_smallcin_kernel(const T* __restrict__ x, int x_cs, int x_co, const T* __restrict__ wp, int Cin, int outPad,
                                                               const float* __restrict__ bias, T* __restrict__ y, int y_cs, int y_co, int IH, int IW,
                                                               int OH, int OW, int stride, long long P, int Cout, int groups, int relu) {
    constexpr int VEC = SmallK<T>::VEC;
    __shared__ float wl[9 * 8 * 64];
    const int cp = groups * 8;
    for (int i = threadIdx.x; i < 9 * 8 * cp; i += 256) {
        const int o = i % cp, r = (i / cp) & 7, t = i / (8 * cp);
        wl[i] = (r < Cin && o < Cout) ? SmallCin<T>::w(wp, outPad, t, o, r) : 0.f;
    }
    __syncthreads();
    const int ppb = 256 / groups;
    const int pl = (int)threadIdx.x / groups, gi = (int)threadIdx.x - pl * groups;
    if (pl >= ppb) return;
    const int c0 = VEC == 8 ? gi * 8 : gi * 4, c1 = VEC == 8 ? gi * 8 + 4 : groups * 4 + gi * 4;
    float bv[8];
#pragma unroll
    for (int j = 0; j < 4; ++j) {
        bv[j] = (bias != nullptr && c0 + j < Cout) ? bias[c0 + j] : 0.f;
        bv[4 + j] = (bias != nullptr && c1 + j < Cout) ? bias[c1 + j] : 0.f;
    }
    for (unsigned pb = blockIdx.x * (unsigned)(ppb * PX); pb < (unsigned)P; pb += gridDim.x * (unsigned)(ppb * PX)) {
        f32x2 o[PX][4];
        const T* xp[PX];
        int iy0[PX], ix0[PX];
#pragma unroll
        for (int q = 0; q < PX; ++q) {
            unsigned p = pb + (unsigned)(q * ppb + pl);
            if (p >= (unsigned)P) p = (unsigned)P - 1;
            const unsigned row = p / (unsigned)OW, img = row / (unsigned)OH;
            const int ox = (int)(p - row * (unsigned)OW), oy = (int)(row - img * (unsigned)OH);
            iy0[q] = oy * stride - 1;
            ix0[q] = ox * stride - 1;
            xp[q] = x + (size_t)img * IH * IW * x_cs + x_co + (iy0[q] * IW + ix0[q]) * x_cs;
#pragma unroll
            for (int j = 0; j < 4; ++j) o[q][j] = f32x2{0.f, 0.f};
        }
        float cur[PX][NX * VEC], nxt[PX][NX * VEC];
        auto load = [&](int t, float (&d)[PX][NX * VEC]) {
            const int ky = t / 3, kx = t - 3 * ky;
#pragma unroll
            for (int q = 0; q < PX; ++q) {
                const int iy = iy0[q] + ky, ix = ix0[q] + kx;
                const bool in = (unsigned)iy < (unsigned)IH && (unsigned)ix < (unsigned)IW;
#pragma unroll
                for (int h = 0; h < NX; ++h) {
                    float v[VEC];
                    SmallK<T>::ld(in ? xp[q] + (ky * IW + kx) * x_cs + h * VEC : x + x_co, v);
#pragma unroll
                    for (int j = 0; j < VEC; ++j) d[q][h * VEC + j] = in ? v[j] : 0.f;
                }
            }
        };
        load(0, cur);
#pragma unroll 1
        for (int t = 0; t < 9; ++t) {
            if (t < 8) load(t + 1, nxt);
            const float* wt = wl + t * 8 * cp;
#pragma unroll
            for (int r = 0; r < NX * VEC; ++r) {
                if (r < Cin) {
                    const f32x2 wa = *reinterpret_cast<const f32x2*>(wt + r * cp + c0), wb = *reinterpret_cast<const f32x2*>(wt + r * cp + c0 + 2);
                    const f32x2 wc = *reinterpret_cast<const f32x2*>(wt + r * cp + c1), wd = *reinterpret_cast<const f32x2*>(wt + r * cp + c1 + 2);
#pragma unroll
                    for (int q = 0; q < PX; ++q) {
                        const f32x2 a = {cur[q][r], cur[q][r]};
                        o[q][0] = __builtin_elementwise_fma(a, wa, o[q][0]);
                        o[q][1] = __builtin_elementwise_fma(a, wb, o[q][1]);
                        o[q][2] = __builtin_elementwise_fma(a, wc, o[q][2]);
                        o[q][3] = __builtin_elementwise_fma(a, wd, o[q][3]);
                    }
                }
            }
#pragma unroll
            for (int q = 0; q < PX; ++q)
#pragma unroll
                for (int r = 0; r < NX * VEC; ++r) cur[q][r] = nxt[q][r];
        }
#pragma unroll
        for (int q = 0; q < PX; ++q) {
            const unsigned p = pb + (unsigned)(q * ppb + pl);
            if (p >= (unsigned)P) break;
            float e[8];
#pragma unroll
            for (int j = 0; j < 8; ++j) {
                e[j] = o[q][j >> 1][j & 1] + bv[j];
                if (relu) e[j] = fmaxf(e[j], 0.f);
                if ((j < 4 ? c0 + j : c1 + j - 4) >= Cout) e[j] = 0.f;
            }
            T* yo = y + (size_t)p * y_cs + y_co;
            if constexpr (VEC == 8) SmallK<T>::st(yo + c0, e);
            else {
                const float lo[4] = {e[0], e[1], e[2], e[3]}, hi[4] = {e[4], e[5], e[6], e[7]};
                if (c0 < Cout) SmallK<T>::st(yo + c0, lo);
                if (c1 < Cout) SmallK<T>::st(yo + c1, hi);
            }
        }
    }
}

}

bool unetconv::conv_smallcin_applies(const unet_conv_desc* d) {
    const unet_tuning t = tuning_of(d->tuning);
    const int vec = d->dtype == UNET_BF16 ? 8 : 4;
    const int plan_n = t.plan_batch > 0 ? t.plan_batch : d->N;
    return t.conv_smallcin != 0 && d->ks == 3 && (d->stride == 1 || d->stride == 2) && d->kind == UNET_CONV_FWD && d->Cin <= 8 && d->Cout >= 16 && d->Cout <= 32 &&
           d->Cout % vec == 0 && d->res == nullptr && !(d->flags & UNET_CONV_MASK) && d->colsum == nullptr && d->colsumsq == nullptr &&
           d->cout_begin == 0 && (d->cout_count == 0 || d->cout_count == d->Cout) && d->wp_img_stride == 0 && !d->pixel_shuffle &&
           !(d->dtype == UNET_BF16 && d->y_f32) && d->Cout <= d->y_cs - d->y_co && unet::roundup(d->Cin, vec) <= d->x_cs - d->x_co &&
           (d->dtype != UNET_BF16 || (long long)plan_n * d->OH * d->OW >= (1ll << 18)) &&
           (long long)d->N * d->OH * d->OW < (1ll << 31) - 256 * 12 * 1024 && (long long)d->IH * d->IW * d->x_cs < (1ll << 31);
}

namespace {
template <typename T, int PX>
int launch_smallcin_px(const unet_conv_desc* d, hipStream_t st) {
    const long long P = (long long)d->N * d->OH * d->OW;
    const int groups = unet::cdiv(d->Cout, 8), ppb = 256 / groups * PX;
    long long blocks = (P + ppb - 1) / ppb;
    if (blocks > 256 * 12) blocks = 256 * 12;
    auto kern = conv3x3_smallcin_kernel<T, PX, 1>;
    if (d->Cin > SmallK<T>::VEC) kern = conv3x3_smallcin_kernel<T, PX, 8 / SmallK<T>::VEC>;
    hipLaunchKernelGGL(kern, dim3((unsigned)blocks), dim3(256), 0, st, (const T*)d->x, d->x_cs, d->x_co, (const T*)d->wp, d->Cin,
                       unet::roundup(d->Cout, 128), d->bias, (T*)d->y, d->y_cs, d->y_co, d->IH, d->IW, d->OH, d->OW, d->stride, P, d->Cout, groups,
                       (d->flags & UNET_CONV_RELU) ? 1 : 0);
    UNET_CHECK_LAUNCH();
    return UNET_OK;
}
template <typename T>
int launch_smallcin(const unet_conv_desc* d, hipStream_t st) {
    const long long P = (long long)d->N * d->OH * d->OW;
    const int ppb4 = 256 / unet::cdiv(d->Cout, 8) * 4;
    return (P + ppb4 - 1) / ppb4 >= 1024 ? launch_smallcin_px<T, 4>(d, st) : launch_smallcin_px<T, 1>(d, st);
}
}

int unetconv::conv_smallk(const unet_conv_desc* d, hipStream_t st) {
    return d->dtype == UNET_BF16 ? launch_smallk<unsigned short>(d, st) : launch_smallk<float>(d, st);
}
int unetconv::conv_smallcin(const unet_conv_desc* d, hipStream_t st) {
    return d->dtype == UNET_BF16 ? launch_smallcin<unsigned short>(d, st) : launch_smallcin<float>(d, st);
}

extern "C" size_t unet_pack_weights_size(int Cout, int Cin, int ks, int mode) {
    const int T = ks * ks;
    const int red = mode == 1 ? Cout : Cin, out = mode == 1 ? Cin : Cout;
    return unetconv::f32_image_elems(red, out, T);
}

extern "C" int unet_pack_weights_strided(const float* w, long long so, long long sr, float* wp, int O, int R, void* stream) {
    UNET_CHECK_ARG(w && wp && O > 0 && R > 0, "pack_weights_strided: bad args");
    const int nchunks = unet::cdiv(R, KC), outPad = unet::roundup(O, 128);
    const size_t total = (size_t)nchunks * outPad * KC;
    hipLaunchKernelGGL(pack_weights_strided_kernel, dim3(unet::ew_grid((long long)total, 256)), dim3(256), 0, (hipStream_t)stream, w, so, sr,
                       wp, O, R, nchunks, outPad, total);
    UNET_CHECK_LAUNCH();
    return UNET_OK;
}

extern "C" int unet_pack_weights(const float* w, float* wp, int Cout, int Cin, int ks, int mode, void* stream) {
    UNET_CHECK_ARG(w && wp, "pack_weights: null pointer");
    UNET_CHECK_ARG((ks == 1 || ks == 3) && (mode == 0 || mode == 1 || (mode == 2 && ks == 1 && Cout % 64 == 0)) && Cout > 0 && Cin > 0, "pack_weights: bad args");
    const int T = ks * ks;
    const int red = mode == 1 ? Cout : Cin, out = mode == 1 ? Cin : Cout;
    const int nchunks = unet::cdiv(red, KC), outPad = unet::roundup(out, 128);
    const size_t total = (size_t)T * nchunks * outPad * KC;
    hipLaunchKernelGGL(pack_weights_kernel, dim3(unet::ew_grid((long long)total, 256)), dim3(256), 0, (hipStream_t)stream,
                       w, wp, Cout, Cin, T, mode, nchunks, outPad, total);
    UNET_CHECK_LAUNCH();
    return UNET_OK;
}
```

unet_amd/csrc/pack_batch.hip:

```cpp

#include "conv_common.h"

namespace {

struct Job {
    const float* w;
    void* wp;
    const float* scale;
    int Cout, Cin, T, mode, nchunks, outPad;
    unsigned block_begin, pad_;
};
static_assert(sizeof(Job) == 56, "job table entry size");

constexpr int ELEMS_PER_BLOCK = 2048;

__global__ __launch_bounds__(256) void pack_batch_kernel(const Job* __restrict__ jobs, int njobs, int bf16) {
    int lo = 0, hi = njobs - 1;
    while (lo < hi) {
        const int mid = (lo + hi + 1) >> 1;
        if (jobs[mid].block_begin <= blockIdx.x) lo = mid; else hi = mid - 1;
    }
    const Job j = jobs[lo];
    const int KC = bf16 ? 32 : 16, sh = bf16 ? 5 : 4;
    const int red = j.mode == 1 ? j.Cout : j.Cin;
    const int out = j.mode == 1 ? j.Cin : j.Cout;
    const size_t main_f32 = (size_t)j.T * j.nchunks * j.outPad * KC;
    const size_t total = bf16 ? unetconv::bf16_image_elems(red, j.outPad, j.T) : unetconv::f32_image_elems(red, out, j.T);
    const size_t base = (size_t)(blockIdx.x - j.block_begin) * ELEMS_PER_BLOCK;
#pragma unroll
    for (int k = 0; k < ELEMS_PER_BLOCK / 256; ++k) {
        const size_t i = base + threadIdx.x + k * 256;
        if (i >= total) break;
        const bool scaled = j.scale != nullptr && j.mode == 0;
        if (bf16) {
            float v = unetconv::bf16_image_value(j.w, j.Cout, j.Cin, j.T, j.mode, j.nchunks, j.outPad, i);
            const int o = (int)((i >> 5) % j.outPad);
            if (scaled && o < j.Cout) v *= j.scale[o];
            reinterpret_cast<unsigned short*>(j.wp)[i] = __builtin_bit_cast(unsigned short, (__bf16)v);
            continue;
        }
        if (i >= main_f32) {
            float v = unetconv::f32_sliver_value(j.w, j.Cout, j.Cin, j.T, j.mode, j.nchunks, i - main_f32);
            const int o = (out & ~15) + (int)(((i - main_f32) >> 4) & 3);
            if (scaled && o < j.Cout) v *= j.scale[o];
            reinterpret_cast<float*>(j.wp)[i] = v;
            continue;
        }
        const int rr = (int)(i & (KC - 1));
        size_t q = i >> sh;
        const int o = (int)(q % j.outPad); q /= j.outPad;
        const int chunk = (int)(q % j.nchunks);
        const int tap = (int)(q / j.nchunks);
        const bool tail = (red & 15) != 0 && chunk == j.nchunks - 1;
        const int r = chunk * 16 + (tail ? (4 * (rr & 3) + (rr >> 2)) : rr);
        float v = 0.f;
        if (j.mode == 2) {
            if (o < j.Cout && r < j.Cin) v = j.w[((size_t)unetconv::ps_filter_of(o, j.Cout) * j.Cin + r) * j.T + tap];
        } else if (j.mode == 0) {
            if (o < j.Cout && r < j.Cin) v = j.w[((size_t)o * j.Cin + r) * j.T + tap] * (scaled ? j.scale[o] : 1.f);
        } else {
            if (o < j.Cin && r < j.Cout) v = j.w[((size_t)r * j.Cin + o) * j.T + tap];
        }
        reinterpret_cast<float*>(j.wp)[i] = v;
    }
}

}

extern "C" size_t unet_pack_batch_table_bytes(int njobs) { return (size_t)(njobs > 0 ? njobs : 0) * sizeof(Job); }

extern "C" int unet_pack_batch_build(const unet_pack_job* jobs, int njobs, int dtype, void* table_host, unsigned* total_blocks) {
    UNET_CHECK_ARG(jobs && table_host && total_blocks && njobs > 0, "pack_batch_build: bad args");
    UNET_CHECK_ARG(dtype == UNET_F32 || dtype == UNET_BF16, "pack_batch_build: unknown dtype %d", dtype);
    Job* t = reinterpret_cast<Job*>(table_host);
    const int KC = dtype == UNET_BF16 ? 32 : 16;
    unsigned long long blocks = 0;
    for (int i = 0; i < njobs; ++i) {
        const unet_pack_job& s = jobs[i];
        UNET_CHECK_ARG(s.w && s.wp && (s.ks == 1 || s.ks == 3) && (s.mode == 0 || s.mode == 1 || s.mode == 2) && s.Cout > 0 && s.Cin > 0,
                       "pack_batch_build: bad job %d", i);
        UNET_CHECK_ARG(s.mode != 2 || (s.ks == 1 && s.Cout % 64 == 0 && s.out_scale == nullptr), "pack_batch_build: job %d: mode 2 is a 1x1 filter with Cout %% 64 == 0", i);
        const int red = s.mode == 1 ? s.Cout : s.Cin, out = s.mode == 1 ? s.Cin : s.Cout;
        Job& j = t[i];
        j.w = s.w; j.wp = s.wp; j.scale = s.out_scale; j.Cout = s.Cout; j.Cin = s.Cin; j.T = s.ks * s.ks; j.mode = s.mode;
        j.nchunks = unet::cdiv(red, KC); j.outPad = unet::roundup(out, 128);
        j.block_begin = (unsigned)blocks; j.pad_ = 0;
        const size_t total = dtype == UNET_BF16 ? unetconv::bf16_image_elems(red, j.outPad, j.T) : unetconv::f32_image_elems(red, out, j.T);
        blocks += (total + ELEMS_PER_BLOCK - 1) / ELEMS_PER_BLOCK;
        UNET_CHECK_ARG(blocks < (1ull << 31), "pack_batch_build: too many blocks");
    }
    *total_blocks = (unsigned)blocks;
    return UNET_OK;
}

extern "C" int unet_pack_batch_run(const void* table_dev, int njobs, unsigned total_blocks, int dtype, void* stream) {
    UNET_CHECK_ARG(table_dev && njobs > 0 && total_blocks > 0, "pack_batch_run: bad args");
    UNET_CHECK_ARG(dtype == UNET_F32 || dtype == UNET_BF16, "pack_batch_run: unknown dtype %d", dtype);
    hipLaunchKernelGGL(pack_batch_kernel, dim3(total_blocks), dim3(256), 0, (hipStream_t)stream, reinterpret_cast<const Job*>(table_dev), njobs,
                       dtype == UNET_BF16 ? 1 : 0);
    UNET_CHECK_LAUNCH();
    return UNET_OK;
}
```

unet_amd/model.py:

```python
from __future__ import annotations

import contextlib
import os
from typing import Dict, List, Optional, Sequence, Tuple

import torch
import torch.nn as nn

from . import ops
from .modules import (BN_EPS, BN_MOM, ConvLayer, Ctx, Encoder, PixelShuffle_ICNR, ResBlock, UnetBlock, _BNExec, _ConvExec,
                      _kaiming_init)
from .ops import TS


class _Marker(nn.Module):
    def __init__(self, name):
        super().__init__()
        self._name = name

    def extra_repr(self):
        return self._name

    def forward(self, *a, **k):
        raise RuntimeError(f"{self._name} runs only inside HipDynamicUnet")


@contextlib.contextmanager
def skip_weight_init():
    saved = nn.init.kaiming_uniform_, nn.init.kaiming_normal_
    nn.init.kaiming_uniform_ = nn.init.kaiming_normal_ = lambda tensor, *a, **k: tensor
    try:
        yield
    finally:
        nn.init.kaiming_uniform_, nn.init.kaiming_normal_ = saved


class HipDynamicUnet(nn.Module):
    fold_eval_bn = os.environ.get("UNET_FOLD_BN", "1") != "0"

    def __init__(self, arch: str, n_in: int, n_out: int, img_size: Sequence[int] = (512, 512), self_attention: bool = False,
                 device="cuda", act_dtype: str = "f32"):
        super().__init__()
        if act_dtype not in ("f32", "bf16"):
            raise ValueError(f"act_dtype must be 'f32' or 'bf16', not {act_dtype!r}")
        self.act_dtype = act_dtype
        self.self_attention = bool(self_attention)
        self.arch, self.n_in, self.n_out = arch, n_in, n_out
        self.img_size = tuple(img_size)
        enc = Encoder(arch, n_in)
        self.sz_chg_idxs = sorted(enc.skip_channels, reverse=True)
        ni = enc.out_channels
        post_bn = nn.BatchNorm2d(ni, eps=BN_EPS, momentum=BN_MOM)
        with torch.no_grad():
            post_bn.bias.fill_(1e-3)
        middle = nn.Sequential(ConvLayer(ni, ni * 2, norm=None), ConvLayer(ni * 2, ni, norm=None))
        layers: List[nn.Module] = [enc, post_bn, nn.ReLU(), middle]
        xc = ni
        prev_sa = False
        for i, idx in enumerate(self.sz_chg_idxs):
            not_final = i != len(self.sz_chg_idxs) - 1
            sa = self_attention and (i == len(self.sz_chg_idxs) - 3)
            blk = UnetBlock(xc, enc.skip_channels[idx], final_div=not_final, blur=True, self_attention=sa, up_is_relu=not prev_sa)
            layers.append(blk)
            xc = blk.out_channels
            prev_sa = sa
        layers.append(PixelShuffle_ICNR(xc))
        layers.append(_Marker("ResizeToOrig"))
        layers.append(_Marker("MergeLayer(dense=True)"))
        self.up_c = xc
        xc += n_in
        layers.append(ResBlock(1, xc, xc, norm=None))
        layers.append(ConvLayer(xc, n_out, ks=1, norm=None, act=False))
        _kaiming_init(layers[3], layers[-2])
        self.layers = nn.ModuleList(layers)
        self.cat_c = xc
        vec = 8 if act_dtype == "bf16" else 4
        blocks = layers[4:4 + len(self.sz_chg_idxs)]
        ragged = [b.cu for b in blocks if b.cu % vec] + ([self.up_c] if act_dtype == "bf16" and self.up_c % vec else [])
        self.up_off, self.cat_p = self.up_c, self.cat_c
        if ragged and act_dtype == "bf16":
            for b in blocks:
                if b.cu % vec:
                    b.set_gap(vec)
            if self.up_c % vec:
                self.up_off = (self.up_c + vec - 1) // vec * vec
                self.cat_p = self.up_off + n_in
                gap = (self.up_c, self.up_off - self.up_c)
                rb, head = layers[-2], layers[-1]
                for cl in (rb.convpath[0], rb.convpath[1]):
                    cl.cx.set_gaps(in_gap=gap, out_gap=gap)
                    cl.nf = self.cat_p
                rb.nf = self.cat_p
                head.cx.set_gaps(in_gap=gap)
        elif ragged:
            raise ValueError(f"{arch}: decoder widths {ragged} are not multiples of {vec} channels")
        self._post_bx = _BNExec(post_bn)
        self._device = torch.device(device)
        self.ctx: Optional[Ctx] = None
        self._pack_tables: Dict[tuple, tuple] = {}
        self.flat_param: Optional[torch.Tensor] = None
        self.flat_grad: Optional[torch.Tensor] = None
        self._last: Dict[str, object] = {}
        self.grad_ready_hook = None
        if self._device.type == "cuda":
            self._materialize()

    def __getitem__(self, i):
        if isinstance(i, slice):
            return nn.Sequential(*list(self.layers)[i])
        return self.layers[i]

    def __len__(self):
        return len(self.layers)

    def _materialize(self):
        dev = self._device
        for b_name, b in list(self.named_buffers()):
            b.data = b.data.to(dev)
        params = list(self.parameters())
        offs, total = [], 0
        for p in params:
            offs.append(total)
            total += (p.numel() + 3) // 4 * 4
        self.flat_param = torch.zeros(total, dtype=torch.float32, device=dev)
        self.flat_grad = torch.zeros(total, dtype=torch.float32, device=dev)
        self._param_offsets = {}
        for p, o in zip(params, offs):
            view = self.flat_param[o:o + p.numel()].view(p.shape)
            view.copy_(p.data)
            p.data = view
            p.grad = self.flat_grad[o:o + p.numel()].view(p.shape)
            self._param_offsets[id(p)] = (o, p.numel())
        self.ctx = Ctx(dev, torch.bfloat16 if self.act_dtype == "bf16" else torch.float32)
        enc = self.layers[0]
        self._enc_child_offset = {}
        for i, child in enumerate(enc):
            ps = list(child.parameters())
            if ps:
                self._enc_child_offset[i] = min(self._param_offsets[id(p)][0] for p in ps)
        self._decoder_offset = min(self._param_offsets[id(p)][0] for l in list(self.layers)[1:] for p in l.parameters())
        self._layer_offset = {}
        for i, l in enumerate(self.layers):
            ps = list(l.parameters())
            if i >= 1 and ps:
                self._layer_offset[i] = min(self._param_offsets[id(p)][0] for p in ps)
        for m in self.modules():
            cx = getattr(m, "cx", None)
            if isinstance(cx, _ConvExec):
                cx.ctx = self.ctx

    def _pack_all(self, training: bool):
        cxs = self.__dict__.get("_cxs")
        if cxs is None:
            cxs = self.__dict__["_cxs"] = [m.cx for m in self.modules() if isinstance(getattr(m, "cx", None), _ConvExec)]
        jobs, marks = [], []
        for cx in cxs:
            cx.ensure_buffers(training)
            ver = cx.version()
            if cx._ver_f != ver:
                jobs.append((cx.wsrc(), cx.wp_f, 0, cx.fold_scale()))
                marks.append((cx, 0, ver))
            if training and cx._ver_d != ver:
                jobs.append((cx.wsrc(), cx.wp_d, 1, None))
                marks.append((cx, 1, ver))
            if cx.wp_s is not None and cx.wp_s.dtype == self.ctx.act_dtype and cx._ver_s != ver and not cx.gapped:
                jobs.append((cx.conv.weight.data, cx.wp_s, 2, None))
                marks.append((cx, 2, ver))
        if not jobs:
            return
        bf = self.ctx.act_dtype == torch.bfloat16
        side = self.ctx.side() if (training and self.ctx.overlap_now()) else None
        if side is None:
            ops.pack_jobs(jobs, bf, self._device, self._pack_tables)
        else:
            fwd = [j for j in jobs if j[2] != 1]
            bwd = [j for j in jobs if j[2] == 1]
            if fwd:
                ops.pack_jobs(fwd, bf, self._device, self._pack_tables)
            if bwd:
                ready = torch.cuda.Event()
                ready.record()
                side.wait_event(ready)
                with torch.cuda.stream(side):
                    ops.pack_jobs(bwd, bf, self._device, self._pack_tables)
                    self.ctx.pack_d_event = torch.cuda.Event()
                    self.ctx.pack_d_event.record()
                self.ctx._side_dirty = True
        for cx, mode, ver in marks:
            if mode == 0:
                cx._ver_f = ver
            elif mode == 2:
                cx._ver_s = ver
            else:
                cx._ver_d = ver

    def param_span(self, p: nn.Parameter) -> Tuple[int, int]:
        return self._param_offsets[id(p)]

    def mark_weights_dirty(self):
        self.ctx.weights_epoch += 1

    def zero_grad(self, set_to_none: bool = False):
        self.flat_grad.zero_()

    def _apply(self, fn, recurse=True):
        probe = fn(torch.zeros(1, device=self._device))
        if probe.device != self._device or probe.dtype != torch.float32:
            raise RuntimeError("HipDynamicUnet is bound to its device/dtype at construction (fp32 on cuda)")
        return self

    def load_state_dict(self, state_dict, strict=True):
        r = super().load_state_dict(state_dict, strict=strict)
        self.mark_weights_dirty()
        return r

    def _hip_forward(self, x: torch.Tensor, training: bool, orient: Optional[int] = None) -> TS:
        if isinstance(x, ops.WindowBatch):
            assert x.src.C == self.n_in, (x.src.C, self.n_in)
            N, H, W = x.n, x.th, x.tw
            put = x.write if orient is None else (lambda buf, at, _x=x: _x.write(buf, at, orient))
        else:
            assert x.is_cuda and x.dtype == torch.float32 and x.dim() == 4 and x.shape[1] == self.n_in, x.shape
            x = x.contiguous()
            N, _, H, W = x.shape
            if orient is None:
                put = lambda buf, at, _x=x: ops.nchw_to_nhwc(_x, ops.TS(buf, 0, buf.shape[3]), at=at)
            else:
                put = lambda buf, at, _x=x: ops.nchw_to_nhwc_oriented(_x, buf, at, orient)
        ctx = self.ctx
        ctx.training = training
        ctx.main_stream = None
        ctx.step_pixels = N * H * W
        ctx.fold_bn = bool(self.fold_eval_bn) and not training
        self._pack_all(training and ctx.need_grad)
        L = self.layers
        enc: Encoder = L[0]
        x0 = ctx.act(self, "x0", N, H, W, self.n_in, zero=True)
        put(x0.buf, 0)
        skips: Dict[int, TS] = {}
        h = x0
        for i, child in enumerate(enc):
            if i == 3:
                OH, OW = (h.H + 2 - 3) // 2 + 1, (h.W + 2 - 3) // 2 + 1
                y = ctx.act(child, "y", N, OH, OW, h.C)
                idx = ctx.vec(child, f"idx{N}x{OH}x{OW}", N * OH * OW * h.C, dtype=torch.uint8)
                ops.maxpool(h, y, idx)
                ctx.saved[(id(child), "x")] = h
                h = y
            elif i < 3:
                h = child.hip_fwd(ctx, h)
            else:
                for blk in child:
                    h = blk.hip_fwd(ctx, h)
            if i in self.sz_chg_idxs:
                skips[i] = h
        e = h
        scale, shift = self._post_bx.coeffs(ctx, e)
        m0 = ctx.act(self, "m0", e.N, e.H, e.W, e.C)
        ops.affine_act(e, m0, scale, shift, relu=True)
        ctx.saved[(id(self), "e")] = e
        h = m0
        for cl in L[3]:
            a = ctx.act(cl, "a", h.N, h.H, h.W, cl.nf)
            cl.cx.fwd(h, a, relu=True)
            ctx.saved[(id(cl), "x")] = h
            h = a
        for k, idx in enumerate(self.sz_chg_idxs):
            h = L[4 + k].hip_fwd(ctx, h, skips[idx])
        nb = 4 + len(self.sz_chg_idxs)
        X = ctx.act(self, "xcat", N, H, W, self.cat_p, zero=True)
        if not L[nb].hip_fwd(ctx, h, X.sub(0, self.up_c), (H, W), tail=(x0, self.up_off)):
            put(X.buf, self.up_off)
        o = L[nb + 3].hip_fwd(ctx, X)
        z = ctx.act(self, "logits", N, H, W, self.n_out, zero=True, dtype=torch.float32)
        head: ConvLayer = L[nb + 4]
        head.cx.fwd(o, z)
        ctx.saved[(id(head), "x")] = o
        self._last = {"skips": skips, "N": N, "H": H, "W": W, "z": z, "training": training}
        return z

    def _hip_backward(self, dz: TS):
        ctx = self.ctx
        L = self.layers
        enc: Encoder = L[0]
        last = self._last
        assert last.get("training", False), "backward needs a preceding training-mode forward"
        ctx.main_stream = torch.cuda.current_stream()
        if getattr(ctx, "pack_d_event", None) is not None:
            ctx.main_stream.wait_event(ctx.pack_d_event)
            ctx.pack_d_event = None
        skips: Dict[int, TS] = last["skips"]
        nb = 4 + len(self.sz_chg_idxs)
        head: ConvLayer = L[nb + 4]
        o: TS = ctx.saved[(id(head), "x")]
        do = head.bwd_from_dy(ctx, dz, mask=o)
        dX = L[nb + 3].bwd_nonorm(ctx, do, dx_channels=self.up_c)
        ctx.free(do)
        d = L[nb].hip_bwd(ctx, dX.sub(0, self.up_c))
        ctx.free(dX)
        hook = self.grad_ready_hook
        if hook is not None:
            user_hook = hook

            def hook(offset, _h=user_hook, _c=ctx):
                _c.side_join()
                _h(offset)
        if hook is not None:
            hook(self._layer_offset[nb])
        dskips: Dict[int, TS] = {}
        for k in range(len(self.sz_chg_idxs) - 1, -1, -1):
            idx = self.sz_chg_idxs[k]
            s = skips[idx]
            ds = ctx.tmp(s.N, s.H, s.W, s.C)
            dn = L[4 + k].hip_bwd(ctx, d, ds, False)
            ctx.free(d)
            d = dn
            dskips[idx] = ds
            if hook is not None:
                hook(self._layer_offset[4 + k])
        mids = list(L[3])
        for j in range(len(mids) - 1, -1, -1):
            xin: TS = ctx.saved[(id(mids[j]), "x")]
            dn = mids[j].bwd_from_dy(ctx, d, mask=xin)
            ctx.free(d)
            d = dn
        e: TS = ctx.saved[(id(self), "e")]
        de = ctx.tmp(e.N, e.H, e.W, e.C)
        self._post_bx.bwd(ctx, d, None, e, de)
        ctx.free(d)
        if hook is not None:
            hook(self._decoder_offset)
        d = de
        children = list(enc)
        for i in range(len(children) - 1, -1, -1):
            child = children[i]
            if i in dskips and i != len(children) - 1:
                ops.copy_slice(dskips[i], d, accumulate=True)
                ctx.free(dskips.pop(i))
            if i > 3:
                for blk in reversed(list(child)):
                    dn = blk.hip_bwd(ctx, d)
                    ctx.free(d)
                    d = dn
            elif i == 3:
                xin: TS = ctx.saved[(id(child), "x")]
# ... 270 lines not shown
```

unet_amd/modules.py:

```python
from __future__ import annotations

import collections
import math
import os
from typing import Dict, List, Optional, Tuple

import torch
import torch.nn as nn

from . import ops
from .ops import TS

BN_EPS = 1e-5
BN_MOM = 0.1



class Ctx:
    def __init__(self, device, act_dtype=torch.float32):
        self.device = device
        self.act_dtype = act_dtype
        self.training = True
        self.need_grad = True
        self._acts: Dict[tuple, TS] = {}
        self._vecs: Dict[tuple, torch.Tensor] = {}
        self._pool: Dict[tuple, list] = {}
        self._pool_all: List[torch.Tensor] = []
        self._pool_key: Dict[int, tuple] = {}
        self._pool_live: set = set()
        self._pool_flat: Dict[int, torch.Tensor] = {}
        self._ws: Optional[torch.Tensor] = None
        self.saved: Dict[tuple, object] = {}
        self.weights_epoch = 0
        self.bn_epoch = 0
        self.fold_bn = False
        mode = os.environ.get("UNET_WGRAD_STREAM", "1")
        self.wgrad_overlap = mode != "0"
        big = 1 << 62
        if mode == "all":
            self.wgrad_overlap_pixels, self.wgrad_overlap_min_pixels = big, 0
        elif act_dtype == torch.float32:
            self.wgrad_overlap_pixels, self.wgrad_overlap_min_pixels = 1 << 20, 0
        else:
            self.wgrad_overlap_pixels, self.wgrad_overlap_min_pixels = big, 1 << 20
        self.step_pixels = 0
        self.main_stream = None
        self._side: Optional[torch.cuda.Stream] = None
        self._side_ws: Optional[torch.Tensor] = None
        self._side_dirty = False
        self._side_tag: Dict[int, torch.cuda.Event] = {}
        self._side_pending = collections.deque()
        self.side_depth = int(os.environ.get("UNET_SIDE_DEPTH", "3"))

    def act(self, owner, tag, N, H, W, C, zero=False, dtype=None) -> TS:
        key = (id(owner), tag, N, H, W, C)
        t = self._acts.get(key)
        if t is None:
            t = ops.new_act(N, H, W, C, self.device, zero=zero, dtype=self.act_dtype if dtype is None else dtype)
            self._acts[key] = t
        return t

    def tmp(self, N, H, W, C, dtype=None) -> TS:
        dt = self.act_dtype if dtype is None else dtype
        cs = ops.rupv(C, dt)
        n = N * H * W * cs
        if cs != C:
            key = ("exact", N, H, W, C, dt)
            free = self._pool.setdefault(key, [])
            flat = free.pop() if free else None
        else:
            key = ("flat", dt)
            free = self._pool.setdefault(key, [])
            best = -1
            for i, b in enumerate(free):
                if b.numel() >= n and (best < 0 or b.numel() < free[best].numel()):
                    best = i
            flat = free.pop(best) if best >= 0 else None
        if flat is None:
            flat = torch.zeros(n, dtype=dt, device=self.device)
            self._pool_all.append(flat)
            self._pool_key[flat.data_ptr()] = key
        self._pool_live.add(flat.data_ptr())
        self._pool_flat[flat.data_ptr()] = flat
        return TS(flat[:n].view(N, H, W, cs), 0, C)

    def free(self, t: Optional[TS]):
        if t is None:
            return
        ptr = t.buf.data_ptr()
        key = self._pool_key.get(ptr)
        if key is None:
            return
        if ptr not in self._pool_live:
            raise RuntimeError("backward temporary freed twice")
        self._pool_live.discard(ptr)
        ev = self._side_tag.pop(ptr, None)
        if ev is not None:
            self._side_pending.append((ptr, key, ev))
            while len(self._side_pending) > self.side_depth:
                self._side_release_oldest()
            return
        self._pool[key].append(self._pool_flat[ptr])

    def side(self) -> Optional["torch.cuda.Stream"]:
        if not self.wgrad_overlap or self.device.type != "cuda":
            return None
        if self._side is None:
            self._side = torch.cuda.Stream(device=self.device)
        return self._side

    def overlap_now(self) -> bool:
        return self.wgrad_overlap and self.wgrad_overlap_min_pixels <= self.step_pixels <= self.wgrad_overlap_pixels

    def side_workspace(self, nfloats: int) -> torch.Tensor:
        if self._side_ws is None or self._side_ws.numel() < nfloats:
            old = self._side_ws
            with torch.cuda.stream(self._side):
                self._side_ws = torch.empty(max(nfloats, 1 << 20), dtype=torch.float32, device=self.device)
            if old is not None:
                old.record_stream(self._side)
        return self._side_ws

    def side_reads(self, t: Optional[TS], ev) -> None:
        if t is not None and t.buf.data_ptr() in self._pool_key:
            self._side_tag[t.buf.data_ptr()] = ev

    def _side_release_oldest(self):
        ptr, key, ev = self._side_pending.popleft()
        (self.main_stream or torch.cuda.current_stream()).wait_event(ev)
        self._pool[key].append(self._pool_flat[ptr])

    def side_join(self):
        if self._side is not None and self._side_dirty:
            (self.main_stream or torch.cuda.current_stream()).wait_stream(self._side)
            self._side_dirty = False
        while self._side_pending:
            ptr, key, _ = self._side_pending.popleft()
            self._pool[key].append(self._pool_flat[ptr])
        self._side_tag.clear()

    def vec(self, owner, tag, n, dtype=torch.float32) -> torch.Tensor:
        key = (id(owner), tag, n, dtype)
        t = self._vecs.get(key)
        if t is None:
            t = torch.zeros(n, dtype=dtype, device=self.device)
            self._vecs[key] = t
        return t

    def workspace(self, nfloats: int) -> torch.Tensor:
        if self._ws is None or self._ws.numel() < nfloats:
            self._ws = torch.empty(max(nfloats, 1 << 20), dtype=torch.float32, device=self.device)
        return self._ws

    def bytes_allocated(self) -> int:
        n = sum(t.buf.numel() * t.buf.element_size() for t in self._acts.values()) + sum(v.numel() * v.element_size() for v in self._vecs.values())
        n += sum(b.numel() * b.element_size() for b in self._pool_all)
        return n + (0 if self._ws is None else self._ws.numel() * 4)


def _no_forward(self, *a, **k):
    raise RuntimeError(f"{type(self).__name__} runs only inside HipDynamicUnet (HIP path); it has no eager forward")



FUSE_BN_STATS = False
FUSE_SHUFFLE = os.environ.get("UNET_FUSE_SHUFFLE", "1") != "0"
FUSE_CONCAT_TAIL = os.environ.get("UNET_FUSE_CONCAT_TAIL", "1") != "0"


class _ConvExec:

    def __init__(self, conv: nn.Conv2d):
        self.conv = conv
        self.ks = conv.kernel_size[0]
        self.stride = conv.stride[0]
        self.wp_f: Optional[torch.Tensor] = None
        self.wp_d: Optional[torch.Tensor] = None
        self.wp_s: Optional[torch.Tensor] = None
        self._ver_f = None
        self._ver_d = None
        self._ver_s = None
        self.ctx: Optional["Ctx"] = None
        self.fold: Optional["_BNExec"] = None
        self.in_gap: Optional[Tuple[int, int]] = None
        self.out_gap: Optional[Tuple[int, int]] = None
        self._wpad = self._bpad = self._gwpad = self._gbpad = None
        self._ver_pad = None
        self._ws_sizes: Dict[tuple, int] = {}

    def set_gaps(self, in_gap=None, out_gap=None):
        self.in_gap = in_gap if in_gap and in_gap[1] else None
        self.out_gap = out_gap if out_gap and out_gap[1] else None
        self._wpad = None

    @property
    def gapped(self) -> bool:
        return self.in_gap is not None or self.out_gap is not None

    @staticmethod
    def _segs(n, gap):
        if gap is None:
            return [(slice(0, n), slice(0, n))], n
        at, g = gap
        return [(slice(0, at), slice(0, at)), (slice(at, n), slice(at + g, n + g))], n + g

    def wsrc(self) -> torch.Tensor:
        w = self.conv.weight.data
        if not self.gapped:
            return w
        Cout, Cin = w.shape[:2]
        si, ci = self._segs(Cin, self.in_gap)
        so, co = self._segs(Cout, self.out_gap)
        if self._wpad is None:
            self._wpad = torch.zeros((co, ci) + tuple(w.shape[2:]), dtype=w.dtype, device=w.device)
            self._gwpad = torch.zeros_like(self._wpad)
            if self.conv.bias is not None:
                self._bpad = torch.zeros(co, dtype=w.dtype, device=w.device)
                self._gbpad = torch.zeros_like(self._bpad)
            self._ver_pad = None
        ver = (self.conv.weight._version, w.data_ptr(), 0 if self.ctx is None else self.ctx.weights_epoch)
        if self._ver_pad != ver:
            for lo, po in so:
                for li, pi in si:
                    self._wpad[po, pi].copy_(w[lo, li])
                if self._bpad is not None:
                    self._bpad[po].copy_(self.conv.bias.data[lo])
            self._ver_pad = ver
        return self._wpad

    def bsrc(self) -> Optional[torch.Tensor]:
        b = self.conv.bias
        if b is None:
            return None
        if not self.gapped:
            return b.data
        self.wsrc()
        return self._bpad

    def fold_scale(self) -> Optional[torch.Tensor]:
        if self.fold is None or self.ctx is None or not self.ctx.fold_bn:
            return None
        return self.fold.coeffs(self.ctx, None)[0]

    def packed(self, mode: int) -> torch.Tensor:
        ver = self.version()
        if mode == 0:
            if self.wp_f is None or self._ver_f != ver:
                self.ensure_buffers(False)
                ops.pack_jobs([(self.wsrc(), self.wp_f, 0, self.fold_scale())], self.wp_f.dtype == torch.bfloat16, self.wp_f.device)
                self._ver_f = ver
            return self.wp_f
        if mode == 2:
            dt = torch.float32 if self.ctx is None else self.ctx.act_dtype
            if self.wp_s is None or self.wp_s.dtype != dt or self._ver_s != ver:
                self.wp_s = ops.pack_weights(self.conv.weight.data, 2, self.wp_s, dtype=dt)
                self._ver_s = ver
            return self.wp_s
        if self.wp_d is None or self._ver_d != ver:
            self.ensure_buffers(True)
            ops.pack_jobs([(self.wsrc(), self.wp_d, 1, None)], self.wp_d.dtype == torch.bfloat16, self.wp_d.device)
            self._ver_d = ver
        return self.wp_d

    def version(self):
        w = self.conv.weight
        c = self.ctx
        folded = c is not None and c.fold_bn and self.fold is not None
        if not folded:
            return (w._version, w.data_ptr(), 0 if c is None else c.weights_epoch, -1)
        bn = self.fold.bn
        return (w._version, w.data_ptr(), c.weights_epoch, c.bn_epoch, bn.weight._version, bn.running_var._version, bn.running_mean._version,
                bn.bias._version)

    def ensure_buffers(self, with_dgrad: bool):
        dt = torch.float32 if self.ctx is None else self.ctx.act_dtype
        w = self.wsrc() if self.gapped else self.conv.weight
        Cout, Cin, ks, _ = w.shape
        size = ops.lib.unet_pack_weights_size_bf16 if dt == torch.bfloat16 else ops.lib.unet_pack_weights_size
        if self.wp_f is None or self.wp_f.dtype != dt:
            self.wp_f = torch.empty(size(Cout, Cin, ks, 0), dtype=dt, device=w.device)
            self._ver_f = None
        if with_dgrad and (self.wp_d is None or self.wp_d.dtype != dt):
            self.wp_d = torch.empty(size(Cout, Cin, ks, 1), dtype=dt, device=w.device)
            self._ver_d = None

    def out_hw(self, H, W):
        return ops.conv_out_hw(H, W, self.ks, self.stride)

    def fwd(self, x: TS, y: TS, relu=False, res: Optional[TS] = None):
        ops.conv2d(x, self.packed(0), y, self.ks, self.stride, bias=self.bsrc(), res=res, relu=relu)

    def fwd_stats(self, ctx: Ctx, x: TS, y: TS):
        assert self.conv.bias is None
        wp = self.packed(0)
        rows = ops.conv_colsum_rows(x, wp, y, self.ks, self.stride, 0)
        part = ctx.workspace(2 * rows * y.C)
        cs, cq = part[:rows * y.C], part[rows * y.C:]
        ops.conv2d(x, wp, y, self.ks, self.stride, colsum=cs, colsumsq=cq)
        return cs, cq, rows

    def bwd_w(self, ctx: Ctx, x: TS, dy: TS):
        side = ctx.side()
        if side is None or not ctx.overlap_now():
            self._bwd_w(ctx, x, dy, ctx.workspace)
            return
        main = ctx.main_stream or torch.cuda.current_stream()
        ready = torch.cuda.Event()
        ready.record(main)
        side.wait_event(ready)
        if self.gapped or ctx._side_ws is None:
            with torch.cuda.stream(side):
                self._bwd_w(ctx, x, dy, ctx.side_workspace)
        else:
            ops.set_stream_override(side.cuda_stream)
            try:
                self._bwd_w(ctx, x, dy, ctx.side_workspace)
            finally:
                ops.set_stream_override(None)
        done = torch.cuda.Event()
        done.record(side)
        ctx._side_dirty = True
        ctx.side_reads(dy, done)
        ctx.side_reads(x, done)

    def _bwd_w(self, ctx: Ctx, x: TS, dy: TS, workspace):
        w, b = self.conv.weight, self.conv.bias
        key = (x.N, x.H, x.W, x.C, x.cs, dy.C, dy.cs, x.bf16, ops.wgrad_tuning_key())
        n = self._ws_sizes.get(key)
        if n is None:
            n = self._ws_sizes[key] = ops.wgrad_workspace(x, dy, self.ks, self.stride, with_bias=b is not None)
        if self.gapped:
            self.wsrc()
            ops.conv2d_wgrad(x, dy, self._gwpad, self.ks, self.stride, workspace(n), dbias=None if b is None else self._gbpad)
            si, _ = self._segs(w.shape[1], self.in_gap)
            so, _ = self._segs(w.shape[0], self.out_gap)
            for lo, po in so:
                for li, pi in si:
                    w.grad[lo, li].copy_(self._gwpad[po, pi])
                if b is not None:
                    b.grad[lo].copy_(self._gbpad[po])
            return
        ops.conv2d_wgrad(x, dy, w.grad, self.ks, self.stride, workspace(n), dbias=None if b is None else b.grad)

    def bwd_x(self, dy: TS, dx: TS, res: Optional[TS] = None, mask: Optional[TS] = None):
        ops.conv2d_dgrad(dy, self.packed(1), dx, self.ks, self.stride, res=res, mask=mask)


class _BNExec:

    def __init__(self, bn: nn.BatchNorm2d):
        self.bn = bn
        self.C = bn.num_features

    def coeffs(self, ctx: Ctx, x: TS, partials=None) -> Tuple[torch.Tensor, torch.Tensor]:
        bn, C_ = self.bn, self.C
        scale, shift = ctx.vec(self, "scale", C_), ctx.vec(self, "shift", C_)
        if ctx.training:
            P = x.P
            if partials is None:
                rows = ops.bn_stats_rows(P)
                part = ctx.workspace(2 * rows * C_)
                ops.bn_stats(x, part)
                ps, pq = part, part[rows * C_:]
            else:
                ps, pq, rows = partials
            mean, invstd = ctx.vec(self, "mean", C_), ctx.vec(self, "invstd", C_)
            ops.bn_finalize(ps, pq, rows, P, C_, bn.weight.data, bn.bias.data, bn.running_mean, bn.running_var,
                            BN_MOM, BN_EPS, scale, shift, mean, invstd, bn.num_batches_tracked)
            ctx.bn_epoch += 1
            self._eval_key = None
        else:
            key = (ctx.weights_epoch, ctx.bn_epoch, bn.weight.data_ptr(), bn.running_mean.data_ptr(), bn.weight._version, bn.bias._version,
                   bn.running_mean._version, bn.running_var._version)
            if getattr(self, "_eval_key", None) != key:
                ops.bn_eval_coeffs(bn.weight.data, bn.bias.data, bn.running_mean, bn.running_var, BN_EPS, scale, shift)
                self._eval_key = key
        return scale, shift

    def bwd(self, ctx: Ctx, dout: TS, out: Optional[TS], x: TS, dx: TS, gout: Optional[TS] = None, g_accumulate=False):
        bn, C_ = self.bn, self.C
        P = x.P
        mean, invstd = ctx.vec(self, "mean", C_), ctx.vec(self, "invstd", C_)
        rows = ops.bn_stats_rows(P)
        part = ctx.workspace(2 * rows * C_)
        ops.bn_bwd_reduce(dout, out, x, mean, invstd, part)
        c1, c2 = ctx.vec(self, "c1", C_), ctx.vec(self, "c2", C_)
        ops.bn_bwd_finalize(part, rows, P, C_, bn.weight.grad, bn.bias.grad, c1, c2)
        ops.bn_bwd_apply(dout, out, x, mean, invstd, bn.weight.data, c1, c2, dx, gout=gout, g_accumulate=g_accumulate)



class ConvLayer(nn.Sequential):
    forward = _no_forward

    def __init__(self, ni, nf, ks=3, stride=1, norm: Optional[str] = "batch", act=True, bias_std=0.01, xtra: Optional[nn.Module] = None):
        bn = norm in ("batch", "batchzero")
        conv = nn.Conv2d(ni, nf, ks, stride=stride, padding=(ks - 1) // 2, bias=not bn)
        with torch.no_grad():
            if conv.bias is not None:
                conv.bias.normal_(0, bias_std) if bias_std != 0 else conv.bias.zero_()
            if act:
                nn.init.kaiming_uniform_(conv.weight)
        layers: List[nn.Module] = [conv]
        if bn:
            b = nn.BatchNorm2d(nf, eps=BN_EPS, momentum=BN_MOM)
            with torch.no_grad():
                b.bias.fill_(1e-3)
                b.weight.fill_(0.0 if norm == "batchzero" else 1.0)
            layers.append(b)
        if act:
            layers.append(nn.ReLU())
        if xtra is not None:
            layers.append(xtra)
        super().__init__(*layers)
        self.has_bn, self.has_act = bn, act
        self.cx = _ConvExec(conv)
        self.bx = _BNExec(self[1]) if bn else None
        self.cx.fold = self.bx
        self.nf = nf

    def hip_fwd(self, ctx: Ctx, x: TS) -> TS:
        OH, OW = self.cx.out_hw(x.H, x.W)
        if self.has_bn and ctx.fold_bn:
            a = ctx.act(self, "a", x.N, OH, OW, self.nf)
            self.fold_fwd(ctx, x, a)
        elif self.has_bn:
            y = ctx.act(self, "y", x.N, OH, OW, self.nf)
            scale, shift = self._conv_bn(ctx, x, y)
            a = ctx.act(self, "a", x.N, OH, OW, self.nf)
            ops.affine_act(y, a, scale, shift, relu=self.has_act)
        else:
            a = ctx.act(self, "a", x.N, OH, OW, self.nf)
            self.cx.fwd(x, a, relu=self.has_act)
        ctx.saved[(id(self), "x")] = x
        return a

    def fold_fwd(self, ctx: Ctx, x: TS, out: TS, res: Optional[TS] = None, relu: Optional[bool] = None):
        _, shift = self.bx.coeffs(ctx, None)
        ops.conv2d(x, self.cx.packed(0), out, self.cx.ks, self.cx.stride, bias=shift, res=res, relu=self.has_act if relu is None else relu)

    def raw_fwd(self, ctx: Ctx, x: TS) -> Tuple[TS, torch.Tensor, torch.Tensor]:
        OH, OW = self.cx.out_hw(x.H, x.W)
        y = ctx.act(self, "y", x.N, OH, OW, self.nf)
        scale, shift = self._conv_bn(ctx, x, y)
        ctx.saved[(id(self), "x")] = x
        return y, scale, shift

    def _conv_bn(self, ctx: Ctx, x: TS, y: TS):
        if ctx.training and FUSE_BN_STATS and ctx.act_dtype == torch.float32 and not (self.nf > 128 and 0 < self.nf % 128 <= 64):
            return self.bx.coeffs(ctx, y, self.cx.fwd_stats(ctx, x, y))
        self.cx.fwd(x, y)
        return self.bx.coeffs(ctx, y)

    def hip_bwd(self, ctx: Ctx, da: TS, need_dx=True, dx_res: Optional[TS] = None) -> Optional[TS]:
        assert self.has_bn
        x: TS = ctx.saved[(id(self), "x")]
        y = ctx.act(self, "y", da.N, da.H, da.W, self.nf)
        a = ctx.act(self, "a", da.N, da.H, da.W, self.nf)
        dy = ctx.tmp(da.N, da.H, da.W, self.nf)
        self.bx.bwd(ctx, da, a if self.has_act else None, y, dy)
        dx = self.bwd_from_dy(ctx, dy, need_dx, dx_res)
        ctx.free(dy)
        return dx

    def bwd_from_dy(self, ctx: Ctx, dy: TS, need_dx=True, dx_res: Optional[TS] = None, mask: Optional[TS] = None,
                    dx_channels: Optional[int] = None) -> Optional[TS]:
        x: TS = ctx.saved[(id(self), "x")]
        self.cx.bwd_w(ctx, x, dy)
        if not need_dx:
            return None
        dx = ctx.tmp(x.N, x.H, x.W, x.C)
        if dx_channels is not None and dx_channels < x.C and (dx_channels + 127) // 128 == (x.C + 127) // 128:
            self.cx.bwd_x(dy, dx.sub(0, dx_channels), res=None if dx_res is None else dx_res.sub(0, dx_channels),
                          mask=None if mask is None else mask.sub(0, dx_channels))
        else:
            self.cx.bwd_x(dy, dx, res=dx_res, mask=mask)
        return dx


class ResBlock(nn.Module):
    forward = _no_forward

    def __init__(self, expansion, ni, nf, stride=1, norm: Optional[str] = "batch"):
        super().__init__()
        norm2 = "batchzero" if norm == "batch" else norm
        nh = nf
        nf, ni = nf * expansion, ni * expansion
        if expansion == 1:
            convpath = [ConvLayer(ni, nh, 3, stride=stride, norm=norm), ConvLayer(nh, nf, 3, norm=norm2, act=False)]
        else:
            convpath = [ConvLayer(ni, nh, 1, norm=norm), ConvLayer(nh, nh, 3, stride=stride, norm=norm),
                        ConvLayer(nh, nf, 1, norm=norm2, act=False)]
        self.convpath = nn.Sequential(*convpath)
        idpath: List[nn.Module] = []
        if ni != nf:
            idpath.append(ConvLayer(ni, nf, 1, norm="batch", act=False))
        if stride != 1:
            idpath.insert(0, nn.AvgPool2d(stride, ceil_mode=True))
# ... 478 lines not shown
```

unet_amd/ops.py:

```python
from __future__ import annotations

import ctypes as C
from dataclasses import dataclass
from typing import Optional

import torch

from . import _lib as L
from ._lib import ConvDesc, WgradDesc, check, lib


import contextlib
import threading

_TUNE = threading.local()


@contextlib.contextmanager
def tuning(**fields):
    prev = getattr(_TUNE, "cur", None)
    cur = L.Tuning.default() if prev is None else L.Tuning.from_buffer_copy(prev)
    for k, v in fields.items():
        if k not in dict(L.Tuning._fields_):
            raise KeyError(f"unet_tuning has no field {k!r}")
# ... 174 lines not shown
    ent = None if cache is None else cache.get(key)
    if ent is None:
        arr = (L.PackJob * len(jobs))()
        for j, (w, wp, mode, sc) in zip(arr, jobs):
            assert w.is_contiguous() and w.dtype == torch.float32 and (sc is None or (sc.dtype == torch.float32 and sc.numel() >= w.shape[0]))
            j.w, j.wp = w.data_ptr(), wp.data_ptr()
            j.Cout, j.Cin, j.ks, j.mode = w.shape[0], w.shape[1], w.shape[2], mode
            j.out_scale = None if sc is None else sc.data_ptr()
        dt = L.BF16 if bf16 else L.F32
        host = torch.zeros(int(lib.unet_pack_batch_table_bytes(len(jobs))), dtype=torch.uint8)
        blocks = C.c_uint(0)
        check(lib.unet_pack_batch_build(arr, len(jobs), dt, host.data_ptr(), C.byref(blocks)), "pack_batch_build")
        ent = (host.to(device), len(jobs), int(blocks.value), dt)
        if cache is not None:
            cache[key] = ent
    table, n, blocks, dt = ent
    check(lib.unet_pack_batch_run(table.data_ptr(), n, blocks, dt, _stream()), "pack_batch_run")


def pack_weights_strided(w_base_ptr: int, so: int, sr: int, O: int, R: int, out: torch.Tensor) -> torch.Tensor:
    if out.dtype == torch.bfloat16:
        assert out.numel() >= lib.unet_pack_weights_size_bf16(O, R, 1, 0)
        check(lib.unet_pack_weights_strided_bf16(w_base_ptr, so, sr, out.data_ptr(), O, R, _stream()), "pack_weights_strided_bf16")
        return out
    assert out.numel() >= lib.unet_pack_weights_size(O, R, 1, 0)
    check(lib.unet_pack_weights_strided(w_base_ptr, so, sr, out.data_ptr(), O, R, _stream()), "pack_weights_strided")
    return out


def pack_size(O: int, R: int, dtype) -> int:
    return int((lib.unet_pack_weights_size_bf16 if dtype == torch.bfloat16 else lib.unet_pack_weights_size)(O, R, 1, 0))


def row_softmax(x: "TS", y: "TS"):
    _need_f32("row_softmax (logits)", x)
    fn = lib.unet_row_softmax_bf16 if y.bf16 else lib.unet_row_softmax
    check(fn(x.ptr, x.cs, x.co, y.ptr, y.cs, y.co, x.P, x.C, _stream()), "row_softmax")


def row_softmax_bwd(y: "TS", dy: "TS", dx: "TS"):
    _need_f32("row_softmax_bwd (dy)", dy)
    assert y.bf16 == dx.bf16
    fn = lib.unet_row_softmax_bwd_bf16 if y.bf16 else lib.unet_row_softmax_bwd
    check(fn(y.ptr, y.cs, y.co, dy.ptr, dy.cs, dy.co, dx.ptr, dx.cs, dx.co, y.P, y.C, _stream()), "row_softmax_bwd")


def sa_fused_supported(dp: int, C: int) -> bool:
    return bool(lib.unet_sa_fused_supported(int(dp), int(C)))


def sa_pack_elems(N: int, cc: int) -> int:
    return int(lib.unet_sa_pack_elems(int(N), int(cc)))


def sa_pack(x: "TS", out: torch.Tensor):
    assert x.bf16 and out.dtype == torch.bfloat16 and out.numel() >= x.N * sa_pack_elems(x.H * x.W, x.C)
    check(lib.unet_sa_pack_bf16(x.ptr, x.cs, x.co, x.C, x.N, x.H * x.W, out.data_ptr(), _stream()), "sa_pack")


def sa_rows(N: int) -> int:
    return (N + 63) // 64 * 64


def sa_fwd(qkv: "TS", dp: int, C: int, vpack: torch.Tensor, O: "TS", lse: torch.Tensor):
    assert qkv.bf16 and O.bf16 and qkv.co == 0 and lse.dtype == torch.float32 and O.C == C and O.P == qkv.P
    assert lse.numel() >= qkv.N * sa_rows(qkv.H * qkv.W) and vpack.numel() >= qkv.N * sa_pack_elems(qkv.H * qkv.W, C)
    check(lib.unet_sa_fwd_bf16(qkv.ptr, qkv.cs, dp, C, qkv.N, qkv.H * qkv.W, vpack.data_ptr(), O.ptr, O.cs, O.co, lse.data_ptr(), _stream()), "sa_fwd")


def sa_rowdot(a: "TS", o: "TS", D: torch.Tensor):
    assert a.bf16 and o.bf16 and a.C == o.C and a.P == o.P and D.dtype == torch.float32 and D.numel() >= a.N * sa_rows(a.H * a.W)
    check(lib.unet_sa_rowdot_bf16(a.ptr, a.cs, a.co, o.ptr, o.cs, o.co, a.N, a.H * a.W, a.C, D.data_ptr(), _stream()), "sa_rowdot")


def sa_bwd(qkv: "TS", dp: int, C: int, dO: "TS", dopack: torch.Tensor, gpack: torch.Tensor, fpack: torch.Tensor, lse: torch.Tensor,
           D: torch.Tensor, dqkv: "TS"):
    assert qkv.bf16 and dO.bf16 and dqkv.bf16 and qkv.co == 0 and dqkv.co == 0 and dqkv.cs == qkv.cs and dO.C == C and dO.P == qkv.P
    rows, N = qkv.N * sa_rows(qkv.H * qkv.W), qkv.H * qkv.W
    assert lse.dtype == torch.float32 and D.dtype == torch.float32 and lse.numel() >= rows and D.numel() >= rows
    assert dopack.numel() >= qkv.N * sa_pack_elems(N, C) and min(gpack.numel(), fpack.numel()) >= qkv.N * sa_pack_elems(N, dp)
    check(lib.unet_sa_bwd_bf16(qkv.ptr, qkv.cs, dp, C, qkv.N, qkv.H * qkv.W, dO.ptr, dO.cs, dO.co, dopack.data_ptr(), gpack.data_ptr(),
                               fpack.data_ptr(), lse.data_ptr(), D.data_ptr(), dqkv.ptr, _stream()), "sa_bwd")


def cast_slice(x: "TS", y: "TS"):
    assert not x.bf16 and y.bf16 and x.P == y.P and x.C == y.C
    check(lib.unet_cast_slice_bf16(x.ptr, x.cs, x.co, y.ptr, y.cs, y.co, x.P, x.C, _stream()), "cast_slice")


def _conv_desc(x: TS, wp: torch.Tensor, y: TS, ks: int, stride: int, kind: int, bias=None, res: Optional[TS] = None,
               mask: Optional[TS] = None, relu=False, colsum=None, colsumsq=None) -> ConvDesc:
    d = ConvDesc()
    d.x, d.x_cs, d.x_co = x.ptr, x.cs, x.co
    d.wp = wp.data_ptr()
    d.bias = _p(bias)
    if res is not None:
        d.res, d.res_cs, d.res_co = res.ptr, res.cs, res.co
    flags = L.CONV_RELU if relu else 0
    if mask is not None:
        d.mask, d.mask_cs, d.mask_co = mask.ptr, mask.cs, mask.co
        flags |= L.CONV_MASK
    d.y, d.y_cs, d.y_co = y.ptr, y.cs, y.co
    d.N, d.IH, d.IW, d.Cin = x.N, x.H, x.W, x.C
    d.OH, d.OW, d.Cout = y.H, y.W, y.C
    d.ks, d.stride, d.kind, d.flags = ks, stride, kind, flags
    d.colsum, d.colsumsq = _p(colsum), _p(colsumsq)
    d.tuning = _tuning_ptr()
    if x.bf16:
        assert wp.dtype == torch.bfloat16 and (res is None or res.bf16) and (mask is None or mask.bf16)
        d.dtype, d.y_f32 = L.BF16, int(not y.bf16)
    else:
        assert wp.dtype == torch.float32 and not y.bf16
    return d


class ConvProbe:

    def __init__(self, variant: int):
        self.variant = variant
        self.events = []
        self.flops = 0.0
        self.bytes = 0.0
        self.detail = []
        self.exclusive_of = None

    def summary(self):
        ms = [a.elapsed_time(b) for a, b in self.events]
        return {"launches": len(ms), "total_ms": sum(ms), "avg_ms": sum(ms) / max(1, len(ms)), "flops": self.flops, "bytes": self.bytes}


CONV_PROBE: Optional[ConvProbe] = None


_SPLITK_WS = {}
_SPLITK_RETIRED = []


def _splitk_ws(d: ConvDesc):
    need = int(lib.unet_conv2d_splitk_workspace(C.byref(d)))
    if need == 0:
        d.splitk_ws, d.splitk_ws_floats = None, 0
        return
    dev = _device_index()
    buf = _SPLITK_WS.get(dev)
    if buf is None or buf.numel() < need:
        if torch.cuda.is_current_stream_capturing():
            raise L.UnetHipError("split-K workspace would have to grow inside a hipGraph capture: run the eager warm-up at this geometry first")
        if buf is not None:
            _SPLITK_RETIRED.append(buf)
        buf = _SPLITK_WS[dev] = torch.empty(max(need, 1 << 22), dtype=torch.float32, device=f"cuda:{dev}")
    d.splitk_ws, d.splitk_ws_floats = buf.data_ptr(), buf.numel()


def _launch_conv_part(d: ConvDesc, what: str, alg_flops: float):
    _splitk_ws(d)
    pr = CONV_PROBE
    if pr is not None and lib.unet_conv2d_variant(C.byref(d)) % 1000000 == pr.variant:
        e0, e1 = torch.cuda.Event(enable_timing=True), torch.cuda.Event(enable_timing=True)
        if pr.exclusive_of is not None:
            torch.cuda.current_stream().wait_stream(pr.exclusive_of)
        e0.record()
        check(lib.unet_conv2d(C.byref(d), _stream()), what)
        e1.record()
        pr.events.append((e0, e1))
        pr.flops += alg_flops
        es = 2 if d.dtype == L.BF16 else 4
        co = d.cout_count or d.Cout
        pix_in, pix_out = d.N * d.IH * d.IW, d.N * d.OH * d.OW
        pr.bytes += (es * (pix_in * d.Cin + pix_out * co * (1 + (1 if d.res else 0) + (1 if d.mask else 0)))
                     + (4 - es) * pix_out * co * d.y_f32 + es * d.ks * d.ks * d.Cin * co)
        pr.detail.append((what, d.N, d.OH, d.OW, d.Cin, d.cout_count or d.Cout, d.ks, d.stride, alg_flops))
        return
    check(lib.unet_conv2d(C.byref(d), _stream()), what)


def _launch_conv(d: ConvDesc, what: str, alg_flops: float):
    Co = d.Cout
    r = Co % 128
    if Co > 128 and 0 < r <= 64 and not d.colsum:
        for b, n in ((0, Co - r), (Co - r, r)):
            d.cout_begin, d.cout_count = b, n
            _launch_conv_part(d, what, alg_flops * n / Co)
        d.cout_begin = d.cout_count = 0
        return
    _launch_conv_part(d, what, alg_flops)


def conv2d(x: TS, wp: torch.Tensor, y: TS, ks: int, stride: int = 1, bias=None, res=None, mask=None, relu=False,
           colsum=None, colsumsq=None, wp_img_stride: int = 0):
    d = _conv_desc(x, wp, y, ks, stride, L.CONV_FWD, bias, res, mask, relu, colsum, colsumsq)
    d.wp_img_stride = wp_img_stride
    _launch_conv(d, "conv2d", 2.0 * y.P * x.C * y.C * ks * ks)


def _ps_desc(x: TS, wp: torch.Tensor, X: TS, bias, relu: bool) -> ConvDesc:
    assert X.H == 2 * x.H and X.W == 2 * x.W and X.N == x.N and x.bf16 == X.bf16
    d = ConvDesc()
    d.x, d.x_cs, d.x_co = x.ptr, x.cs, x.co
    d.wp, d.bias = wp.data_ptr(), _p(bias)
    d.y, d.y_cs, d.y_co = X.ptr, X.cs, X.co
    d.N, d.IH, d.IW, d.Cin = x.N, x.H, x.W, x.C
    d.OH, d.OW, d.Cout = x.H, x.W, 4 * X.C
    d.ks, d.stride, d.kind, d.flags = 1, 1, L.CONV_FWD, (L.CONV_RELU if relu else 0)
    d.dtype = L.BF16 if x.bf16 else L.F32
    d.tuning = _tuning_ptr()
    d.pixel_shuffle = 1
    return d


def conv1x1_shuffle_applies(x: TS, X: TS) -> bool:
    d = _ps_desc(x, torch.empty(0), X, None, True)
    d.wp = 16
    return int(lib.unet_conv2d_variant(C.byref(d))) == 8


def conv1x1_shuffle_tail_ok(X: TS, tail: TS, at: int) -> bool:
    return (tail.bf16 == X.bf16 and (tail.N, tail.H, tail.W) == (X.N, X.H, X.W) and tail.cs % 4 == 0 and tail.co % 4 == 0 and at % 4 == 0
            and tail.co + rup4(tail.C) <= tail.cs and at >= X.co + X.C and at + rup4(tail.C) <= X.cs)


def conv1x1_shuffle(x: TS, wp_ps: torch.Tensor, X: TS, bias=None, relu=True, tail: Optional[TS] = None, tail_at: int = 0):
    d = _ps_desc(x, wp_ps, X, bias, relu)
    if tail is not None:
        assert conv1x1_shuffle_tail_ok(X, tail, tail_at)
        d.ps_tail, d.ps_tail_cs, d.ps_tail_co, d.ps_tail_c, d.ps_tail_at = tail.ptr, tail.cs, tail.co, tail.C, tail_at
    check(lib.unet_conv2d(C.byref(d), _stream()), "conv1x1_shuffle")


def shuffle_bwd_xmask(dX: TS, X: TS, dyc: TS):
    assert dyc.C == 4 * dX.C and dX.H == 2 * dyc.H and dX.W == 2 * dyc.W and X.C == dX.C
    check(_fn("shuffle_bwd_xmask", dX)(dX.ptr, dX.cs, dX.co, X.ptr, X.cs, X.co, dyc.ptr, dyc.cs, dyc.co, dyc.N, dyc.H, dyc.W, dX.C, _stream()),
          "shuffle_bwd_xmask")


def conv2d_variant(x: TS, wp: torch.Tensor, y: TS, ks: int, stride: int = 1, kind: int = 0) -> int:
    d = _conv_desc(x, wp, y, ks, stride, kind)
    _splitk_ws(d)
    return int(lib.unet_conv2d_variant(C.byref(d)))


def conv2d_dgrad(dy: TS, wp_dgrad: torch.Tensor, dx: TS, ks: int, stride: int = 1, res=None, mask=None, colsum=None):
    d = _conv_desc(dy, wp_dgrad, dx, ks, stride, L.CONV_DGRAD, None, res, mask, False, colsum, None)
    _launch_conv(d, "conv2d_dgrad", 2.0 * dy.P * dy.C * dx.C * ks * ks)


def conv_colsum_rows(x: TS, wp, y: TS, ks, stride, kind) -> int:
    d = _conv_desc(x, wp, y, ks, stride, kind)
    r = lib.unet_conv2d_colsum_rows(C.byref(d))
    if r < 0:
        check(r, "conv2d_colsum_rows")
    return r


def _wgrad_desc(x: TS, dy: TS, dw, dbias, ks, stride, ws, accumulate) -> WgradDesc:
    d = WgradDesc()
    d.x, d.x_cs, d.x_co = x.ptr, x.cs, x.co
    d.dy, d.dy_cs, d.dy_co = dy.ptr, dy.cs, dy.co
    d.dw, d.dbias = _p(dw), _p(dbias)
    d.N, d.IH, d.IW, d.Cin = x.N, x.H, x.W, x.C
    d.OH, d.OW, d.Cout = dy.H, dy.W, dy.C
    d.ks, d.stride = ks, stride
    d.workspace = _p(ws)
    d.workspace_floats = 0 if ws is None else ws.numel()
    d.accumulate = int(accumulate)
    d.tuning = _tuning_ptr()
    assert x.bf16 == dy.bf16
    d.dtype = L.BF16 if x.bf16 else L.F32
    return d


def wgrad_workspace(x: TS, dy: TS, ks, stride, with_bias=False) -> int:
    d = _wgrad_desc(x, dy, torch.empty(0), None, ks, stride, None, 0)
    d.dw = 1
    return int(lib.unet_conv2d_wgrad_workspace(C.byref(d)))


def conv2d_wgrad(x: TS, dy: TS, dw: torch.Tensor, ks: int, stride: int, ws: torch.Tensor, dbias=None, accumulate=False):
    d = _wgrad_desc(x, dy, dw, dbias, ks, stride, ws, accumulate)
    check(lib.unet_conv2d_wgrad(C.byref(d), _stream()), "conv2d_wgrad")



def bn_stats_rows(P: int) -> int:
    return lib.unet_bn_stats_rows(P)


def bn_stats(x: TS, partial: torch.Tensor):
    check(_fn("bn_stats", x)(x.ptr, x.cs, x.co, x.P, x.C, partial.data_ptr(), _stream()), "bn_stats")


def bn_finalize(psum, psumsq, rows, count, C_, gamma, beta, rmean, rvar, momentum, eps, scale, shift, smean, sinvstd, tracked=None):
    assert tracked is None or tracked.dtype == torch.int64
    check(lib.unet_bn_finalize(_p(psum), _p(psumsq), rows, count, C_, _p(gamma), _p(beta), _p(rmean), _p(rvar), momentum, eps,
                               _p(scale), _p(shift), _p(smean), _p(sinvstd), _p(tracked), _stream()), "bn_finalize")


def bn_eval_coeffs(gamma, beta, rmean, rvar, eps, scale, shift):
    check(lib.unet_bn_eval_coeffs(_p(gamma), _p(beta), _p(rmean), _p(rvar), eps, rmean.numel(), _p(scale), _p(shift), _stream()),
          "bn_eval_coeffs")


def affine_act(x: TS, y: TS, scale=None, shift=None, x2: Optional[TS] = None, scale2=None, shift2=None, relu=False):
    check(_fn("affine_act", x)(x.ptr, x.cs, x.co, _p(scale), _p(shift),
                              None if x2 is None else x2.ptr, 0 if x2 is None else x2.cs, 0 if x2 is None else x2.co,
                              _p(scale2), _p(shift2), y.ptr, y.cs, y.co, x.P, x.C, int(relu), _stream()), "affine_act")


def bn_bwd_reduce(dout: TS, out: Optional[TS], x: TS, mean, invstd, partial):
    check(_fn("bn_bwd_reduce", x)(dout.ptr, dout.cs, dout.co, None if out is None else out.ptr, 0 if out is None else out.cs,
                                 0 if out is None else out.co, x.ptr, x.cs, x.co, _p(mean), _p(invstd), x.P, x.C,
                                 partial.data_ptr(), _stream()), "bn_bwd_reduce")


def bn_bwd_finalize(partial, rows, count, C_, dgamma, dbeta, c1, c2):
    check(lib.unet_bn_bwd_finalize(_p(partial), rows, count, C_, _p(dgamma), _p(dbeta), _p(c1), _p(c2), _stream()), "bn_bwd_finalize")


def bn_bwd_apply(dout: TS, out: Optional[TS], x: TS, mean, invstd, gamma, c1, c2, dx: TS, gout: Optional[TS] = None,
                 g_accumulate=False):
    check(_fn("bn_bwd_apply", x)(dout.ptr, dout.cs, dout.co, None if out is None else out.ptr, 0 if out is None else out.cs,
                                0 if out is None else out.co, x.ptr, x.cs, x.co, _p(mean), _p(invstd), _p(gamma), _p(c1), _p(c2),
                                dx.ptr, dx.cs, dx.co, None if gout is None else gout.ptr, 0 if gout is None else gout.cs,
                                0 if gout is None else gout.co, int(g_accumulate), x.P, x.C, _stream()), "bn_bwd_apply")



def maxpool(x: TS, y: TS, idx: Optional[torch.Tensor]):
    check(_fn("maxpool3x3s2", x)(x.ptr, x.cs, x.co, y.ptr, y.cs, y.co, _p(idx), x.N, x.H, x.W, x.C, y.H, y.W, _stream()), "maxpool")


def maxpool_bwd(dy: TS, idx: torch.Tensor, dx: TS, accumulate=False):
    check(_fn("maxpool3x3s2_bwd", dy)(dy.ptr, dy.cs, dy.co, idx.data_ptr(), dx.ptr, dx.cs, dx.co, dx.N, dx.H, dx.W, dx.C, dy.H, dy.W,
                                    int(accumulate), _stream()), "maxpool_bwd")


def avgpool(x: TS, y: TS):
    check(_fn("avgpool2_ceil", x)(x.ptr, x.cs, x.co, y.ptr, y.cs, y.co, x.N, x.H, x.W, x.C, y.H, y.W, _stream()), "avgpool")


def avgpool_bwd(dy: TS, dx: TS, accumulate=False):
    check(_fn("avgpool2_ceil_bwd", dy)(dy.ptr, dy.cs, dy.co, dx.ptr, dx.cs, dx.co, dx.N, dx.H, dx.W, dx.C, dy.H, dy.W, int(accumulate),
                                     _stream()), "avgpool_bwd")



def shuffle_blur(yc: TS, X: TS, blur: bool):
    assert yc.C == 4 * X.C and X.H == 2 * yc.H and X.W == 2 * yc.W
    check(_fn("shuffle_blur", yc)(yc.ptr, yc.cs, yc.co, X.ptr, X.cs, X.co, yc.N, yc.H, yc.W, X.C, int(blur), _stream()), "shuffle_blur")


def shuffle_blur_bwd(dX: TS, yc: TS, dyc: TS, blur: bool):
    assert yc.C == 4 * dX.C and dX.H == 2 * yc.H and dX.W == 2 * yc.W
    check(_fn("shuffle_blur_bwd", dX)(dX.ptr, dX.cs, dX.co, yc.ptr, yc.cs, yc.co, dyc.ptr, dyc.cs, dyc.co, yc.N, yc.H, yc.W, dX.C,
                                    int(blur), _stream()), "shuffle_blur_bwd")


def resize_nearest(x: TS, y: TS):
    assert x.bf16 == y.bf16
    check(_fn("resize_nearest", x)(x.ptr, x.cs, x.co, y.ptr, y.cs, y.co, x.N, x.H, x.W, y.H, y.W, x.C, _stream()), "resize_nearest")


def resize_nearest_bwd(dy: TS, dx: TS):
    assert dy.bf16 == dx.bf16
    check(_fn("resize_nearest_bwd", dy)(dy.ptr, dy.cs, dy.co, dx.ptr, dx.cs, dx.co, dx.N, dx.H, dx.W, dy.H, dy.W, dx.C, _stream()),
          "resize_nearest_bwd")


def nchw_to_nhwc(x: torch.Tensor, y: TS, at: Optional[int] = None):
    N, C_, H, W = x.shape
    if at is None:
        assert x.is_contiguous() and y.C == C_
        check(_fn("nchw_to_nhwc", y)(x.data_ptr(), y.ptr, y.cs, y.co, N, C_, H, W, _stream()), "nchw_to_nhwc")
    else:
        assert x.is_contiguous() and y.co == 0 and at + C_ <= y.cs
        check(_fn("nchw_to_nhwc", y)(x.data_ptr(), y.ptr, y.cs, at, N, C_, H, W, _stream()), "nchw_to_nhwc")


def nhwc_to_nchw(x: TS, y: torch.Tensor):
    _need_f32("nhwc_to_nchw", x)
    assert y.is_contiguous()
    check(lib.unet_nhwc_to_nchw(x.ptr, x.cs, x.co, y.data_ptr(), x.N, x.C, x.H, x.W, _stream()), "nhwc_to_nchw")


def copy_slice(x: TS, y: TS, accumulate=False):
    check(_fn("copy_slice", x)(x.ptr, x.cs, x.co, y.ptr, y.cs, y.co, x.P, x.C, int(accumulate), _stream()), "copy_slice")


def relu_mask(g: TS, ref: TS, y: TS):
    assert g.bf16 == ref.bf16 == y.bf16
    check(_fn("relu_mask", g)(g.ptr, g.cs, g.co, ref.ptr, ref.cs, ref.co, y.ptr, y.cs, y.co, g.P, g.C, _stream()), "relu_mask")


def colsum_workspace(P, C_) -> int:
    return int(lib.unet_colsum_workspace(P, C_))


# ... 778 lines not shown
```

Before: 148.8.

## Add split-bf16 MFMA path for f32 3x3 dgrad convolutions

Adds a new dgrad kernel for f32 3x3 stride-1 convolutions that splits activations into three bf16 parts in LDS and multiplies them against pre-split weights using bf16 MFMA instructions, emulating f32 accuracy. A new weight-packing mode (mode 3) produces the split weight image, and the Python side queries a per-shape heuristic to decide when to use it. The aim is to replace slower f32 matrix math on the backward data-gradient path with faster bf16 matrix cores. In exchange it adds extra MFMA work, extra weight packing per weight version, and some risk to precision.

After: 148.5. About the same (-0.2%).

```diff
diff --git a/include/unet_hip.h b/include/unet_hip.h
--- a/include/unet_hip.h
+++ b/include/unet_hip.h
@@ -38,6 +38,7 @@
     int wgrad_wgs;
     int conv_smallcin;
     int conv_head1x1;
+    int dgrad_split;
 } unet_tuning;
 void unet_tuning_default(unet_tuning* t);
 
@@ -78,8 +79,10 @@
 int unet_conv2d(const unet_conv_desc* d, void* stream);
 size_t unet_conv2d_splitk_workspace(const unet_conv_desc* d);
 int unet_conv2d_variant(const unet_conv_desc* d);
+int unet_conv2d_dgrad_split(const unet_conv_desc* d);
 size_t unet_pack_weights_size(int Cout, int Cin, int ks, int mode);
 int unet_pack_weights(const float* w, float* wp, int Cout, int Cin, int ks, int mode, void* stream);
+int unet_pack_weights_split_host(const float* w, unet_bf16* wp, int Cout, int Cin, int ks);
 int unet_pack_weights_strided(const float* w, long long so, long long sr, float* wp, int O, int R, void* stream);
 size_t unet_pack_weights_size_bf16(int Cout, int Cin, int ks, int mode);
 int unet_pack_weights_bf16(const float* w, unet_bf16* wp, int Cout, int Cin, int ks, int mode, void* stream);
diff --git a/unet_amd/_lib.py b/unet_amd/_lib.py
--- a/unet_amd/_lib.py
+++ b/unet_amd/_lib.py
@@ -25,7 +25,7 @@
 
 class Tuning(C.Structure):
     _fields_ = [(n, C.c_int) for n in ("conv_splitk", "mfma_shape", "f32_big_tile", "bf16_big_tile", "t256_tiles_per_wg", "t256_sliver",
-                                       "conv1x1_gemm", "wgrad_mfma_shape", "wgrad_bf16_k4", "wgrad_1x1", "wgrad_narrow", "plan_batch", "wgrad_wgs", "conv_smallcin", "conv_head1x1")]
+                                       "conv1x1_gemm", "wgrad_mfma_shape", "wgrad_bf16_k4", "wgrad_1x1", "wgrad_narrow", "plan_batch", "wgrad_wgs", "conv_smallcin", "conv_head1x1", "dgrad_split")]
 
     @classmethod
     def default(cls, **over) -> "Tuning":
@@ -143,6 +143,8 @@
     "unet_pack_batch_table_bytes": (sz, [i]),
     "unet_pack_batch_build": (i, [C.POINTER(PackJob), i, i, vp, C.POINTER(C.c_uint)]),
     "unet_pack_batch_run": (i, [vp, i, C.c_uint, i, vp]),
+    "unet_conv2d_dgrad_split": (i, [C.POINTER(ConvDesc)]),
+    "unet_pack_weights_split_host": (i, [vp, vp, i, i, i]),
     "unet_pack_weights_size": (sz, [i, i, i, i]),
     "unet_pack_weights": (i, [vp, vp, i, i, i, i, vp]),
     "unet_pack_weights_strided": (i, [vp, ll, ll, vp, i, i, vp]),
diff --git a/unet_amd/csrc/conv_bf16.hip b/unet_amd/csrc/conv_bf16.hip
--- a/unet_amd/csrc/conv_bf16.hip
+++ b/unet_amd/csrc/conv_bf16.hip
@@ -810,6 +810,316 @@
 }
 #endif
 
+constexpr int SPL_ROWB = 96;
+typedef unsigned u32x2 __attribute__((ext_vector_type(2)));
+
+__device__ __forceinline__ void split3_x4(const v4f v, u32x2& p1, u32x2& p2, u32x2& p3) {
+    const bf16x4 h1 = {(__bf16)v[0], (__bf16)v[1], (__bf16)v[2], (__bf16)v[3]};
+    const v4f r1 = {v[0] - (float)h1[0], v[1] - (float)h1[1], v[2] - (float)h1[2], v[3] - (float)h1[3]};
+    const bf16x4 h2 = {(__bf16)r1[0], (__bf16)r1[1], (__bf16)r1[2], (__bf16)r1[3]};
+    const v4f r2 = {r1[0] - (float)h2[0], r1[1] - (float)h2[1], r1[2] - (float)h2[2], r1[3] - (float)h2[3]};
+    const bf16x4 h3 = {(__bf16)r2[0], (__bf16)r2[1], (__bf16)r2[2], (__bf16)r2[3]};
+    p1 = __builtin_bit_cast(u32x2, h1); p2 = __builtin_bit_cast(u32x2, h2); p3 = __builtin_bit_cast(u32x2, h3);
+}
+
+template <int NF>
+__device__ __forceinline__ void gld_fs(v4f (&d)[4], unsigned v, const char* p) {
+    static_assert(NF >= 1 && NF <= 4, "filter tiles per wave");
+    if constexpr (NF == 4)
+        asm volatile("s_nop 4\n\tglobal_load_dwordx4 %0, %4, %5\n\tglobal_load_dwordx4 %1, %4, %5 offset:1024\n\t"
+                     "global_load_dwordx4 %2, %4, %5 offset:2048\n\tglobal_load_dwordx4 %3, %4, %5 offset:3072"
+                     : "=&v"(d[0]), "=&v"(d[1]), "=&v"(d[2]), "=&v"(d[3]) : "v"(v), "s"(p));
+    else if constexpr (NF == 3)
+        asm volatile("s_nop 4\n\tglobal_load_dwordx4 %0, %3, %4\n\tglobal_load_dwordx4 %1, %3, %4 offset:1024\n\t"
+                     "global_load_dwordx4 %2, %3, %4 offset:2048"
+                     : "=&v"(d[0]), "=&v"(d[1]), "=&v"(d[2]) : "v"(v), "s"(p));
+    else if constexpr (NF == 2)
+        asm volatile("s_nop 4\n\tglobal_load_dwordx4 %0, %2, %3\n\tglobal_load_dwordx4 %1, %2, %3 offset:1024"
+                     : "=&v"(d[0]), "=&v"(d[1]) : "v"(v), "s"(p));
+    else
+        asm volatile("s_nop 4\n\tglobal_load_dwordx4 %0, %1, %2" : "=&v"(d[0]) : "v"(v), "s"(p));
+}
+__device__ __forceinline__ void gld_halo2_buf(v4f (&h)[2], const unsigned (&vo)[2], v4i rs, int soff) {
+    asm volatile("s_nop 4\n\tbuffer_load_dwordx4 %[h0], %[o0], %[rs], %[so] offen\n\tbuffer_load_dwordx4 %[h1], %[o1], %[rs], %[so] offen"
+                 : [h0] "+v"(h[0]), [h1] "+v"(h[1]) : [o0] "v"(vo[0]), [o1] "v"(vo[1]), [rs] "s"(rs), [so] "s"(soff));
+}
+template <int N, bool H, int NF>
+__device__ __forceinline__ void wait_cnt_fs(v4f (&x)[4], v4f (&h)[2]) {
+#define UNET_FS1 "+v"(x[0])
+#define UNET_FS2 UNET_FS1, "+v"(x[1])
+#define UNET_FS3 UNET_FS2, "+v"(x[2])
+#define UNET_FS4 UNET_FS3, "+v"(x[3])
+#define UNET_FSW(ops_) do { if constexpr (H) asm volatile("s_waitcnt vmcnt(%[n])" : ops_, "+v"(h[0]), "+v"(h[1]) : [n] "n"(N)); \
+                            else asm volatile("s_waitcnt vmcnt(%[n])" : ops_ : [n] "n"(N)); } while (0)
+    if constexpr (NF == 4) UNET_FSW(UNET_FS4);
+    else if constexpr (NF == 3) UNET_FSW(UNET_FS3);
+    else if constexpr (NF == 2) UNET_FSW(UNET_FS2);
+    else UNET_FSW(UNET_FS1);
+#undef UNET_FSW
+#undef UNET_FS4
+#undef UNET_FS3
+#undef UNET_FS2
+#undef UNET_FS1
+}
+template <int NF>
+__device__ __forceinline__ void wait_first_fs(v4f (&x)[4], v4f (&y)[4], v4f (&h)[6]) {
+#define UNET_H6 "+v"(h[0]), "+v"(h[1]), "+v"(h[2]), "+v"(h[3]), "+v"(h[4]), "+v"(h[5])
+    if constexpr (NF == 4) asm volatile("s_waitcnt vmcnt(0)" : "+v"(x[0]), "+v"(y[0]), "+v"(x[1]), "+v"(y[1]), "+v"(x[2]), "+v"(y[2]), "+v"(x[3]), "+v"(y[3]), UNET_H6);
+    else if constexpr (NF == 3) asm volatile("s_waitcnt vmcnt(0)" : "+v"(x[0]), "+v"(y[0]), "+v"(x[1]), "+v"(y[1]), "+v"(x[2]), "+v"(y[2]), UNET_H6);
+    else if constexpr (NF == 2) asm volatile("s_waitcnt vmcnt(0)" : "+v"(x[0]), "+v"(y[0]), "+v"(x[1]), "+v"(y[1]), UNET_H6);
+    else asm volatile("s_waitcnt vmcnt(0)" : "+v"(x[0]), "+v"(y[0]), UNET_H6);
+#undef UNET_H6
+}
+
+template <int NF>
+__global__ __launch_bounds__(256, 2) void conv_split_t256_kernel(const KArgs a, const int tpw, const int bn) {
+    constexpr int TW = 32, TH = 8, M16 = 8, MH = 4, HIT = 6, NTH = 256;
+    constexpr int HW = TW + 2, HPIX = (TH + 2) * HW, BUFB = HPIX * SPL_ROWB;
+    static_assert(HPIX * 4 <= HIT * NTH, "pixel patch of the 256-pixel tile");
+    extern __shared__ __attribute__((aligned(16))) char lds[];
+
+    const int tid = threadIdx.x, lane = tid & 63, wave = __builtin_amdgcn_readfirstlane(tid >> 6);
+    const int wm = wave >> 1, wn = wave & 1;
+    const int l15 = lane & 15, kq = lane >> 4;
+    const TapSet& ts = a.taps[0];
+
+    const int per_xcd = (int)(gridDim.x >> 3);
+    const int wg = (int)(blockIdx.x & 7) * per_xcd + (int)(blockIdx.x >> 3);
+    const int ntiles = a.mtiles * a.ntn;
+    int tile = wg * tpw;
+    const int tend = tile + tpw < ntiles ? tile + tpw : ntiles;
+    if (tile >= tend) return;
+    const int rev = a.sliver;
+    const int nchunks = a.nchunks, last = nchunks - 1;
+
+    constexpr unsigned OOB = 0x80000000u;
+    int oy0, ox0, n0, img;
+    const char *wbase, *w0;
+    v4i rs;
+    unsigned goff[HIT];
+    const size_t plane_b = (size_t)a.coutPad * 32, slab_b = 3 * plane_b;
+    const long long tap_step = (rev ? -1ll : 1ll) * (long long)nchunks * (long long)slab_b;
+#define SPL_SETUP(tile_) do { \
+        int id_ = (tile_); \
+        const int nt_ = __builtin_amdgcn_readfirstlane(id_ % a.ntn); id_ /= a.ntn; \
+        const int tx_ = __builtin_amdgcn_readfirstlane(id_ % a.tiles_x); id_ /= a.tiles_x; \
+        const int ty_ = __builtin_amdgcn_readfirstlane(id_ % a.tiles_y); \
+        img = __builtin_amdgcn_readfirstlane(id_ / a.tiles_y); \
+        oy0 = ty_ * TH; ox0 = tx_ * TW; n0 = a.n_base + nt_ * bn; \
+        wbase = reinterpret_cast<const char*>(sgpr_ptr(reinterpret_cast<const char*>(a.wp) + (size_t)n0 * 32)); \
+        w0 = wbase + (rev ? 8ll * nchunks * (long long)slab_b : 0ll);        \
+        const u64 xb_ = sgpr_ptr(reinterpret_cast<const char*>(a.x) + (size_t)img * a.IH * a.IW * a.x_cs * 4); \
+        rs[0] = (int)(unsigned)xb_; rs[1] = (int)(unsigned)(xb_ >> 32); \
+        rs[2] = __builtin_amdgcn_readfirstlane(a.IH * a.IW * a.x_cs * 4); rs[3] = 0x00020000; \
+        const int iy0_ = oy0 + ts.min_dy, ix0_ = ox0 + ts.min_dx; \
+        int tid_ = tid; \
+        asm volatile("" : "+v"(tid_));       \
+        _Pragma("unroll") for (int it = 0; it < HIT; ++it) { \
+            const int e = tid_ + it * NTH; \
+            const int p = e >> 2, q = e & 3; \
+            const int hy = p / HW, hx = p - hy * HW; \
+            const int iy = iy0_ + hy, ix = ix0_ + hx; \
+            const bool inb = (e < HPIX * 4) && iy >= 0 && iy < a.IH && ix >= 0 && ix < a.IW; \
+            goff[it] = inb ? (unsigned)((iy * a.IW + ix) * a.x_cs + a.x_co + 4 * q) * 4u : OOB; \
+        } } while (0)
+    const bool tail_cut = last * 16 + 4 * (tid & 3) >= a.Cin4;
+    const unsigned vst = (unsigned)((tid >> 2) * SPL_ROWB + (tid & 3) * 8);
+    const bool st5 = tid + 5 * NTH < HPIX * 4;
+#define SPL_STORE_ITEM(buf_, it_, v_) do { \
+        if ((it_) < 5 || st5) { \
+            char* d_ = lds + (buf_) * BUFB + vst + (it_) * (NTH / 4) * SPL_ROWB; \
+            u32x2 p1_, p2_, p3_; \
+            split3_x4((v_), p1_, p2_, p3_); \
+            *reinterpret_cast<u32x2*>(d_) = p1_; *reinterpret_cast<u32x2*>(d_ + 32) = p2_; *reinterpret_cast<u32x2*>(d_ + 64) = p3_; \
+        } } while (0)
+    v4f hreg[2];
+    hreg[0] = hreg[1] = (v4f){0.f, 0.f, 0.f, 0.f};
+
+    const unsigned vrow = (unsigned)((wn * 16 + l15) * 32 + 16 * (kq & 1));
+    const unsigned voffa = vrow + (kq >= 2 ? (unsigned)plane_b : 0u);
+    const unsigned voffb = vrow + (kq >= 2 ? 2u * (unsigned)plane_b : 0u);
+    v4f a0[4], a1[4], c0[4];
+#pragma unroll
+    for (int n = 0; n < 4; ++n) a0[n] = a1[n] = c0[n] = (v4f){0.f, 0.f, 0.f, 0.f};
+#define TILE_COL(n_) (((n_) * 2 + wn) * 16)
+
+    f32x4 acc[M16][4];
+
+    const unsigned vbase = (unsigned)(((wm * 128 / TW) * HW + l15) * SPL_ROWB + 16 * (kq & 1));
+    const unsigned vbase3 = vbase + (kq < 2 ? 64u : 0u);
+    constexpr int HALF_B = (64 / TW) * HW * SPL_ROWB;
+#define MOFF(m_) (((((m_) * 16) / TW) * HW + ((m_) * 16) % TW) * SPL_ROWB)
+#define TOFF(t_) ((((t_) / 3) * HW + (t_) % 3) * SPL_ROWB)
+#define SPL_MFMA(wu_, addr_) do { \
+        _Pragma("unroll") for (int h = 0; h < 2; ++h) { \
+            v4f pv_[MH]; \
+            _Pragma("unroll") for (int m = 0; m < MH; ++m) \
+                pv_[m] = *reinterpret_cast<const v4f*>(lds + (addr_) + h * HALF_B + MOFF(m)); \
+            _Pragma("unroll") for (int n = 0; n < NF; ++n) { \
+                const bf16x8 wv_ = __builtin_bit_cast(bf16x8, (wu_)[n]); \
+                _Pragma("unroll") for (int m = 0; m < MH; ++m) \
+                    acc[h * MH + m][n] = __builtin_amdgcn_mfma_f32_16x16x32_bf16(wv_, __builtin_bit_cast(bf16x8, pv_[m]), acc[h * MH + m][n], 0, 0, 0); \
+            } \
+            __builtin_amdgcn_sched_barrier(0);       \
+        } } while (0)
+#define SPL_STAGE(au_, al_, t_) do { \
+        gld_fs<NF>(al_, voffa, wcur); \
+        if ((t_) % 3 == 0) { \
+            unsigned vo_[2]; \
+            vo_[0] = cut ? OOB : goff[2 * ((t_) / 3)]; vo_[1] = cut ? OOB : goff[2 * ((t_) / 3) + 1]; \
+            gld_halo2_buf(hreg, vo_, rs, more ? (chunk + 1) * 64 : 0); \
+        } \
+        SPL_MFMA(au_, vcur + TOFF(t_)); \
+        SPL_MFMA(au_, vcur + TOFF(t_) + 32u); \
+        __builtin_amdgcn_sched_barrier(0); \
+        if ((t_) % 3 == 0) wait_cnt_fs<NF + 2, false, NF>(c0, hreg); else wait_cnt_fs<NF, false, NF>(c0, hreg); \
+        SPL_MFMA(c0, vcur3 + TOFF(t_)); \
+        __builtin_amdgcn_sched_barrier(0); \
+        if ((t_) % 3 == 0) wait_cnt_fs<2, false, NF>(al_, hreg); \
+        else if ((t_) % 3 == 1) wait_cnt_fs<0, true, NF>(al_, hreg); \
+        else wait_cnt_fs<0, false, NF>(al_, hreg); \
+        gld_fs<NF>(c0, voffb, wcur); \
+    } while (0)
+
+    for (;;) {
+        SPL_SETUP(tile);
+        {
+            v4f h6[HIT];
+            unsigned vo_[HIT];
+#pragma unroll
+            for (int it = 0; it < HIT; ++it) { h6[it] = (v4f){0.f, 0.f, 0.f, 0.f}; vo_[it] = (tail_cut && last == 0) ? OOB : goff[it]; }
+            gld_halo6_buf(h6, vo_, rs, 0);
+            gld_fs<NF>(a0, voffa, w0);
+            gld_fs<NF>(c0, voffb, w0);
+            wait_first_fs<NF>(a0, c0, h6);
+            __syncthreads();
+#pragma unroll
+            for (int it = 0; it < HIT; ++it) SPL_STORE_ITEM(0, it, h6[it]);
+            __syncthreads();
+        }
+#pragma unroll
+        for (int m = 0; m < M16; ++m)
+#pragma unroll
+            for (int n = 0; n < 4; ++n) acc[m][n] = (f32x4){0.f, 0.f, 0.f, 0.f};
+
+        const char* wcur = w0;
+        for (int chunk = 0; chunk < nchunks; ++chunk) {
+            const bool more = chunk + 1 < nchunks;
+            const unsigned vcur = vbase + (unsigned)((chunk & 1) * BUFB), vcur3 = vbase3 + (unsigned)((chunk & 1) * BUFB);
+            const int nb = (chunk + 1) & 1;
+            const bool cut = !more || (tail_cut && chunk + 1 == last);
+#pragma unroll
+            for (int t = 0; t < 9; ++t) {
+                if (t < 8) wcur += tap_step;
+                else wcur = more ? w0 + (size_t)(chunk + 1) * slab_b : wbase;
+                if (t & 1) SPL_STAGE(a1, a0, t); else SPL_STAGE(a0, a1, t);
+                if (t % 3 == 1 && more) {
+                    SPL_STORE_ITEM(nb, 2 * (t / 3), hreg[0]);
+                    SPL_STORE_ITEM(nb, 2 * (t / 3) + 1, hreg[1]);
+                }
+            }
+#pragma unroll
+            for (int n = 0; n < NF; ++n) a0[n] = a1[n];
+            if (more) __syncthreads();
+        }
+        wait_cnt_fs<0, false, NF>(c0, hreg);
+
+        const bool relu = a.flags & UNET_CONV_RELU;
+        const size_t img_pix = (size_t)img * a.OH * a.OW;
+        const float* resb = a.res ? a.res + img_pix * a.res_cs + a.res_co : nullptr;
+        const float* maskb = a.mask ? a.mask + img_pix * a.mask_cs + a.mask_co : nullptr;
+        auto pix_of = [&](int mm, int& pidx_, bool& pval_) {
+            const int oy = oy0 + wm * (M16 * 16 / TW) + (mm >> 1), ox = ox0 + (mm & 1) * 16 + l15;
+            pval_ = oy < a.OH && ox < a.OW;
+            pidx_ = pval_ ? (oy * a.OW + ox) : 0;
+        };
+        if (resb != nullptr || maskb != nullptr || a.bias != nullptr || relu) {
+#pragma unroll
+            for (int h = 0; h < 2; ++h) {
+                int pidx[MH];
+                bool pval[MH];
+#pragma unroll
+                for (int m = 0; m < MH; ++m) pix_of(h * MH + m, pidx[m], pval[m]);
+#pragma unroll
+                for (int n = 0; n < NF; ++n) {
+                    const int c4 = n0 + TILE_COL(n) + 4 * kq;
+                    const bool cvalid = c4 < a.n_end;
+                    const int cc = cvalid ? c4 : 0;
+                    f32x4 bv = {0.f, 0.f, 0.f, 0.f};
+                    if (a.bias != nullptr && cvalid) {
+#pragma unroll
+                        for (int q = 0; q < 4; ++q) bv[q] = (c4 + q < a.Cout) ? a.bias[c4 + q] : 0.f;
+                    }
+#pragma unroll
+                    for (int m = 0; m < MH; ++m) acc[h * MH + m][n] += bv;
+                    if (resb != nullptr) {
+#pragma unroll
+                        for (int m = 0; m < MH; ++m) acc[h * MH + m][n] += *reinterpret_cast<const f32x4*>(resb + (size_t)pidx[m] * a.res_cs + cc);
+                    }
+                    if (relu) {
+#pragma unroll
+                        for (int m = 0; m < MH; ++m)
+#pragma unroll
+                            for (int q = 0; q < 4; ++q) acc[h * MH + m][n][q] = fmaxf(acc[h * MH + m][n][q], 0.f);
+                    }
+                    if (maskb != nullptr) {
+#pragma unroll
+                        for (int m = 0; m < MH; ++m) {
+                            const f32x4 mv = *reinterpret_cast<const f32x4*>(maskb + (size_t)pidx[m] * a.mask_cs + cc);
+#pragma unroll
+                            for (int q = 0; q < 4; ++q) acc[h * MH + m][n][q] = mv[q] > 0.f ? acc[h * MH + m][n][q] : 0.f;
+                        }
+                    }
+                }
+            }
+        }
+        float* yb = a.y + img_pix * a.y_cs + a.y_co;
+#pragma unroll
+        for (int m = 0; m < M16; ++m) {
+            int pidx;
+            bool pval;
+            pix_of(m, pidx, pval);
+#pragma unroll
+            for (int n = 0; n < NF; ++n) {
+                const int c4 = n0 + TILE_COL(n) + 4 * kq;
+                if (c4 < a.n_end && pval) *reinterpret_cast<f32x4*>(yb + (size_t)pidx * a.y_cs + c4) = acc[m][n];
+            }
+        }
+        if (++tile >= tend) break;
+    }
+#undef SPL_STAGE
+#undef SPL_MFMA
+#undef SPL_SETUP
+#undef SPL_STORE_ITEM
+#undef MOFF
+#undef TOFF
+#undef TILE_COL
+}
+
+int launch_split_t256(const Plan& p, hipStream_t st) {
+    const int cols = p.k.n_end - p.k.n_base;
+    const int nf = p.k.ntn == 1 ? (cols + 31) / 32 : p.bn / 32;
+    const int ntiles = p.k.mtiles * p.k.ntn;
+    int tpw = p.tune.t256_tiles_per_wg > 0 ? p.tune.t256_tiles_per_wg : ntiles / 2048;
+    tpw = tpw < 1 ? 1 : (tpw > 16 ? 16 : tpw);
+    dim3 grid = p.grid;
+    grid.x = (unsigned)unet::roundup(unet::cdiv(ntiles, tpw), 8);
+    const size_t lds_b = (size_t)2 * 340 * SPL_ROWB;
+    switch (nf) {
+        case 4: return launch_big_lds<conv_split_t256_kernel<4>>(grid, dim3(256), lds_b, st, p.k, tpw, p.bn);
+        case 3: return launch_big_lds<conv_split_t256_kernel<3>>(grid, dim3(256), lds_b, st, p.k, tpw, p.bn);
+        case 2: return launch_big_lds<conv_split_t256_kernel<2>>(grid, dim3(256), lds_b, st, p.k, tpw, p.bn);
+        case 1: return launch_big_lds<conv_split_t256_kernel<1>>(grid, dim3(256), lds_b, st, p.k, tpw, p.bn);
+    }
+    unet::set_error("conv: %d channel tiles per wave in the split 256-pixel tile", nf);
+    return (int)UNET_E_UNSUPPORTED;
+}
+
+__global__ void pack_weights_split_kernel(const float* __restrict__ w, u16* __restrict__ wp, int Cout, int Cin, int T, int nchunks, int outPad, size_t total) {
+    for (size_t i = (size_t)blockIdx.x * blockDim.x + threadIdx.x; i < total; i += (size_t)gridDim.x * blockDim.x)
+        wp[i] = split_image_value(w, Cout, Cin, T, nchunks, outPad, i);
+}
+
 
 template <int NTOT, int TW, typename T, bool SLV = false>
 int launch_t256n(const Plan& p, int y_f32, hipStream_t st) {
@@ -891,9 +1201,19 @@
 int unetconv::conv_t256(const Plan& p0, int dtype, int y_f32, hipStream_t st) {
     Plan p = p0;
     p.k.sliver = p.k.taps[0].dy[0] > 0 ? 1 : 0;
+    if (p.dsplit) return launch_split_t256(p, st);
     if (dtype == UNET_BF16) return launch_t256<unsigned short>(p, y_f32, st);
     p.k.fold = 0;
     return launch_t256<float>(p, 1, st);
+}
+
+int unetconv::pack_weights_split(const float* w, void* wp, int Cout, int Cin, int T, hipStream_t st) {
+    const int nchunks = unet::cdiv(Cout, KC), outPad = unet::roundup(Cin, 128);
+    const size_t total = split_image_elems(Cout, Cin, T);
+    hipLaunchKernelGGL(pack_weights_split_kernel, dim3(unet::ew_grid((long long)total, 256)), dim3(256), 0, st, w, reinterpret_cast<u16*>(wp), Cout, Cin, T,
+                       nchunks, outPad, total);
+    UNET_CHECK_LAUNCH();
+    return UNET_OK;
 }
 
 extern "C" size_t unet_pack_weights_size_bf16(int Cout, int Cin, int ks, int mode) {
diff --git a/unet_amd/csrc/conv_common.h b/unet_amd/csrc/conv_common.h
--- a/unet_amd/csrc/conv_common.h
+++ b/unet_amd/csrc/conv_common.h
@@ -75,6 +75,34 @@
     if (mode == 2) return o < Cout ? w[((size_t)ps_filter_of(o, Cout) * Cin + r) * T + tap] : 0.f;
     if (mode == 0) return o < Cout ? w[((size_t)o * Cin + r) * T + tap] : 0.f;
     return o < Cin ? w[((size_t)r * Cin + o) * T + tap] : 0.f;
+}
+
+__host__ __device__ inline size_t split_image_elems(int red, int out, int T) {
+    return (size_t)T * ((red + 15) / 16) * 3 * ((out + 127) / 128 * 128) * 16;
+}
+__host__ __device__ inline unsigned short bf16_rne_bits(float f) {
+    unsigned u = __builtin_bit_cast(unsigned, f);
+    if ((u & 0x7fffffffu) > 0x7f800000u) return (unsigned short)((u >> 16) | 0x40u);
+    u += 0x7fffu + ((u >> 16) & 1u);
+    return (unsigned short)(u >> 16);
+}
+__host__ __device__ inline float bf16_bits_value(unsigned short h) { return __builtin_bit_cast(float, (unsigned)h << 16); }
+__host__ __device__ inline unsigned short split3_piece(float v, int piece) {
+    const unsigned short h1 = bf16_rne_bits(v);
+    if (piece == 0) return h1;
+    const float r1 = v - bf16_bits_value(h1);
+    const unsigned short h2 = bf16_rne_bits(r1);
+    return piece == 1 ? h2 : bf16_rne_bits(r1 - bf16_bits_value(h2));
+}
+__host__ __device__ inline unsigned short split_image_value(const float* __restrict__ w, int Cout, int Cin, int T, int nchunks, int outPad, size_t i) {
+    const int rr = (int)(i & 15);
+    size_t j = i >> 4;
+    const int o = (int)(j % outPad); j /= outPad;
+    const int piece = (int)(j % 3); j /= 3;
+    const int chunk = (int)(j % nchunks), tap = (int)(j / nchunks);
+    const int r = chunk * 16 + rr;
+    const float v = (o < Cin && r < Cout) ? w[((size_t)r * Cin + o) * T + tap] : 0.f;
+    return split3_piece(v, piece);
 }
 
 typedef float v4f __attribute__((ext_vector_type(4)));
@@ -195,6 +223,7 @@
     int splits, cp;
     size_t ws_floats;
     unet_tuning tune;
+    int dsplit;
 };
 
 
@@ -245,6 +274,7 @@
 int conv_generic_f32(const Plan& p, hipStream_t st);
 int conv_generic_bf16(const Plan& p, int y_f32, hipStream_t st);
 int conv_t256(const Plan& p, int dtype, int y_f32, hipStream_t st);
+int pack_weights_split(const float* w, void* wp, int Cout, int Cin, int T, hipStream_t st);
 int splitk_reduce(const unet_conv_desc* d, const Plan& p, hipStream_t st);
 bool conv_smallk_applies(const unet_conv_desc* d);
 int conv_smallk(const unet_conv_desc* d, hipStream_t st);
diff --git a/unet_amd/csrc/conv_dispatch.hip b/unet_amd/csrc/conv_dispatch.hip
--- a/unet_amd/csrc/conv_dispatch.hip
+++ b/unet_amd/csrc/conv_dispatch.hip
@@ -25,6 +25,7 @@
         v.wgrad_wgs = env_int("UNET_WGRAD_WGS", 0);
         v.conv_smallcin = env_int("UNET_CONV_SMALLCIN", 1);
         v.conv_head1x1 = env_int("UNET_CONV_HEAD1X1", 1);
+        v.dgrad_split = env_int("UNET_DGRAD_SPLIT", 0);
         return v;
     }();
     return t;
@@ -68,6 +69,7 @@
 
     KArgs& k = p->k;
     memset(&k, 0, sizeof(k));
+    p->dsplit = 0;
     k.x = d->x; k.wp = d->wp; k.bias = d->bias; k.res = d->res; k.mask = (d->flags & UNET_CONV_MASK) ? d->mask : nullptr;
     k.y = d->y; k.colsum = d->colsum; k.colsumsq = d->colsumsq;
     k.x_cs = d->x_cs; k.x_co = d->x_co; k.res_cs = d->res_cs; k.res_co = d->res_co;
@@ -252,6 +254,20 @@
     return d != nullptr && d->dtype == UNET_BF16 ? plan_bf16(d, p, splitk) : plan_f32(d, p, splitk);
 }
 
+bool dgrad_split_takes(const unet_conv_desc* d, const Plan& p) {
+    const KArgs& k = p.k;
+    const int cols = k.n_end - k.n_base;
+    return d->dtype == UNET_F32 && d->kind == UNET_CONV_DGRAD && d->ks == 3 && d->stride == 1 && p.hit == 6 && p.bm == 256 && p.tw == 32 &&
+           p.splits == 1 && d->wp_img_stride == 0 &&
+           k.n_base + (k.ntn == 1 ? unet::roundup(cols, 32) : k.ntn * p.bn) <= k.coutPad;
+}
+bool dgrad_split_admitted(const Plan& p) {
+    const KArgs& k = p.k;
+    const int nf = k.ntn == 1 ? (k.n_end - k.n_base + 31) / 32 : p.bn / 32;
+    const long long blocks = (long long)k.mtiles * k.ntn;
+    return nf >= 2 && k.nchunks >= 4 && blocks >= 128;
+}
+
 enum class Family { PixelShuffle, SmallK, SmallCin, Head1x1, Gemm1x1, T256, Generic };
 
 int choose(const unet_conv_desc* d, Family* f, Plan* p) {
@@ -267,6 +283,7 @@
     else if (conv_head1x1_applies(d)) *f = Family::Head1x1;
     else if (conv_gemm1x1_applies(d)) *f = Family::Gemm1x1;
     else *f = p->hit == 6 ? Family::T256 : Family::Generic;
+    if (*f == Family::T256 && p->tune.dgrad_split && dgrad_split_takes(d, *p) && (p->tune.dgrad_split == 2 || dgrad_split_admitted(*p))) p->dsplit = 1;
     return UNET_OK;
 }
 
@@ -312,6 +329,13 @@
     return rc == UNET_OK ? variant_id(f, p) : rc;
 }
 
+extern "C" int unet_conv2d_dgrad_split(const unet_conv_desc* d) {
+    Family f;
+    Plan p;
+    const int rc = choose(d, &f, &p);
+    return rc == UNET_OK ? (f != Family::PixelShuffle && p.dsplit ? 1 : 0) : rc;
+}
+
 extern "C" size_t unet_conv2d_splitk_workspace(const unet_conv_desc* d) {
     Plan p;
     if (d == nullptr || d->pixel_shuffle) return 0;
diff --git a/unet_amd/csrc/conv_igemm.hip b/unet_amd/csrc/conv_igemm.hip
--- a/unet_amd/csrc/conv_igemm.hip
+++ b/unet_amd/csrc/conv_igemm.hip
@@ -970,6 +970,7 @@
 
 extern "C" size_t unet_pack_weights_size(int Cout, int Cin, int ks, int mode) {
     const int T = ks * ks;
+    if (mode == 3) return unetconv::split_image_elems(Cout, Cin, T) / 2;
     const int red = mode == 1 ? Cout : Cin, out = mode == 1 ? Cin : Cout;
     return unetconv::f32_image_elems(red, out, T);
 }
@@ -986,8 +987,9 @@
 
 extern "C" int unet_pack_weights(const float* w, float* wp, int Cout, int Cin, int ks, int mode, void* stream) {
     UNET_CHECK_ARG(w && wp, "pack_weights: null pointer");
-    UNET_CHECK_ARG((ks == 1 || ks == 3) && (mode == 0 || mode == 1 || (mode == 2 && ks == 1 && Cout % 64 == 0)) && Cout > 0 && Cin > 0, "pack_weights: bad args");
+    UNET_CHECK_ARG((ks == 1 || ks == 3) && (mode == 0 || mode == 1 || (mode == 2 && ks == 1 && Cout % 64 == 0) || (mode == 3 && ks == 3)) && Cout > 0 && Cin > 0, "pack_weights: bad args");
     const int T = ks * ks;
+    if (mode == 3) return unetconv::pack_weights_split(w, wp, Cout, Cin, T, (hipStream_t)stream);
     const int red = mode == 1 ? Cout : Cin, out = mode == 1 ? Cin : Cout;
     const int nchunks = unet::cdiv(red, KC), outPad = unet::roundup(out, 128);
     const size_t total = (size_t)T * nchunks * outPad * KC;
diff --git a/unet_amd/csrc/pack_batch.hip b/unet_amd/csrc/pack_batch.hip
--- a/unet_amd/csrc/pack_batch.hip
+++ b/unet_amd/csrc/pack_batch.hip
@@ -25,13 +25,19 @@
     const int red = j.mode == 1 ? j.Cout : j.Cin;
     const int out = j.mode == 1 ? j.Cin : j.Cout;
     const size_t main_f32 = (size_t)j.T * j.nchunks * j.outPad * KC;
-    const size_t total = bf16 ? unetconv::bf16_image_elems(red, j.outPad, j.T) : unetconv::f32_image_elems(red, out, j.T);
+    const bool split = !bf16 && j.mode == 3;
+    const size_t total = split ? unetconv::split_image_elems(j.Cout, j.Cin, j.T)
+                               : (bf16 ? unetconv::bf16_image_elems(red, j.outPad, j.T) : unetconv::f32_image_elems(red, out, j.T));
     const size_t base = (size_t)(blockIdx.x - j.block_begin) * ELEMS_PER_BLOCK;
 #pragma unroll
     for (int k = 0; k < ELEMS_PER_BLOCK / 256; ++k) {
         const size_t i = base + threadIdx.x + k * 256;
         if (i >= total) break;
         const bool scaled = j.scale != nullptr && j.mode == 0;
+        if (split) {
+            reinterpret_cast<unsigned short*>(j.wp)[i] = unetconv::split_image_value(j.w, j.Cout, j.Cin, j.T, j.nchunks, j.outPad, i);
+            continue;
+        }
         if (bf16) {
             float v = unetconv::bf16_image_value(j.w, j.Cout, j.Cin, j.T, j.mode, j.nchunks, j.outPad, i);
             const int o = (int)((i >> 5) % j.outPad);
@@ -77,15 +83,18 @@
     unsigned long long blocks = 0;
     for (int i = 0; i < njobs; ++i) {
         const unet_pack_job& s = jobs[i];
-        UNET_CHECK_ARG(s.w && s.wp && (s.ks == 1 || s.ks == 3) && (s.mode == 0 || s.mode == 1 || s.mode == 2) && s.Cout > 0 && s.Cin > 0,
+        UNET_CHECK_ARG(s.w && s.wp && (s.ks == 1 || s.ks == 3) && (s.mode == 0 || s.mode == 1 || s.mode == 2 || s.mode == 3) && s.Cout > 0 && s.Cin > 0,
                        "pack_batch_build: bad job %d", i);
         UNET_CHECK_ARG(s.mode != 2 || (s.ks == 1 && s.Cout % 64 == 0 && s.out_scale == nullptr), "pack_batch_build: job %d: mode 2 is a 1x1 filter with Cout %% 64 == 0", i);
-        const int red = s.mode == 1 ? s.Cout : s.Cin, out = s.mode == 1 ? s.Cin : s.Cout;
+        UNET_CHECK_ARG(s.mode != 3 || (s.ks == 3 && dtype == UNET_F32 && s.out_scale == nullptr), "pack_batch_build: job %d: mode 3 is the split image of an fp32 3x3 filter", i);
+        const bool rev = s.mode == 1 || s.mode == 3;
+        const int red = rev ? s.Cout : s.Cin, out = rev ? s.Cin : s.Cout;
         Job& j = t[i];
         j.w = s.w; j.wp = s.wp; j.scale = s.out_scale; j.Cout = s.Cout; j.Cin = s.Cin; j.T = s.ks * s.ks; j.mode = s.mode;
         j.nchunks = unet::cdiv(red, KC); j.outPad = unet::roundup(out, 128);
         j.block_begin = (unsigned)blocks; j.pad_ = 0;
-        const size_t total = dtype == UNET_BF16 ? unetconv::bf16_image_elems(red, j.outPad, j.T) : unetconv::f32_image_elems(red, out, j.T);
+        const size_t total = s.mode == 3 ? unetconv::split_image_elems(s.Cout, s.Cin, j.T)
+                                         : (dtype == UNET_BF16 ? unetconv::bf16_image_elems(red, j.outPad, j.T) : unetconv::f32_image_elems(red, out, j.T));
         blocks += (total + ELEMS_PER_BLOCK - 1) / ELEMS_PER_BLOCK;
         UNET_CHECK_ARG(blocks < (1ull << 31), "pack_batch_build: too many blocks");
     }
@@ -101,3 +110,11 @@
     UNET_CHECK_LAUNCH();
     return UNET_OK;
 }
+
+extern "C" int unet_pack_weights_split_host(const float* w, unet_bf16* wp, int Cout, int Cin, int ks) {
+    UNET_CHECK_ARG(w && wp && ks == 3 && Cout > 0 && Cin > 0, "pack_weights_split_host: bad args");
+    const int T = ks * ks, nchunks = unet::cdiv(Cout, 16), outPad = unet::roundup(Cin, 128);
+    const size_t total = unetconv::split_image_elems(Cout, Cin, T);
+    for (size_t i = 0; i < total; ++i) wp[i] = unetconv::split_image_value(w, Cout, Cin, T, nchunks, outPad, i);
+    return UNET_OK;
+}
diff --git a/unet_amd/model.py b/unet_amd/model.py
--- a/unet_amd/model.py
+++ b/unet_amd/model.py
@@ -154,6 +154,7 @@
         if cxs is None:
             cxs = self.__dict__["_cxs"] = [m.cx for m in self.modules() if isinstance(getattr(m, "cx", None), _ConvExec)]
         jobs, marks = [], []
+        bf = self.ctx.act_dtype == torch.bfloat16
         for cx in cxs:
             cx.ensure_buffers(training)
             ver = cx.version()
@@ -163,18 +164,20 @@
             if training and cx._ver_d != ver:
                 jobs.append((cx.wsrc(), cx.wp_d, 1, None))
                 marks.append((cx, 1, ver))
+            if training and cx.wp_x is not None and cx._ver_x != ver and not bf:
+                jobs.append((cx.wsrc(), cx.wp_x, 3, None))
+                marks.append((cx, 3, ver))
             if cx.wp_s is not None and cx.wp_s.dtype == self.ctx.act_dtype and cx._ver_s != ver and not cx.gapped:
                 jobs.append((cx.conv.weight.data, cx.wp_s, 2, None))
                 marks.append((cx, 2, ver))
         if not jobs:
             return
-        bf = self.ctx.act_dtype == torch.bfloat16
         side = self.ctx.side() if (training and self.ctx.overlap_now()) else None
         if side is None:
             ops.pack_jobs(jobs, bf, self._device, self._pack_tables)
         else:
-            fwd = [j for j in jobs if j[2] != 1]
-            bwd = [j for j in jobs if j[2] == 1]
+            fwd = [j for j in jobs if j[2] not in (1, 3)]
+            bwd = [j for j in jobs if j[2] in (1, 3)]
             if fwd:
                 ops.pack_jobs(fwd, bf, self._device, self._pack_tables)
             if bwd:
@@ -191,6 +194,8 @@
                 cx._ver_f = ver
             elif mode == 2:
                 cx._ver_s = ver
+            elif mode == 3:
+                cx._ver_x = ver
             else:
                 cx._ver_d = ver
 
diff --git a/unet_amd/modules.py b/unet_amd/modules.py
--- a/unet_amd/modules.py
+++ b/unet_amd/modules.py
@@ -176,6 +176,9 @@
         self.stride = conv.stride[0]
         self.wp_f: Optional[torch.Tensor] = None
         self.wp_d: Optional[torch.Tensor] = None
+        self.wp_x: Optional[torch.Tensor] = None
+        self._ver_x = None
+        self._split_want: Dict[tuple, bool] = {}
         self.wp_s: Optional[torch.Tensor] = None
         self._ver_f = None
         self._ver_d = None
@@ -256,6 +259,14 @@
                 self.wp_s = ops.pack_weights(self.conv.weight.data, 2, self.wp_s, dtype=dt)
                 self._ver_s = ver
             return self.wp_s
+        if mode == 3:
+            if self.wp_x is None or self._ver_x != ver:
+                w = self.wsrc()
+                if self.wp_x is None:
+                    self.wp_x = torch.empty(ops.lib.unet_pack_weights_size(w.shape[0], w.shape[1], self.ks, 3), dtype=torch.float32, device=w.device)
+                ops.pack_jobs([(w, self.wp_x, 3, None)], False, w.device)
+                self._ver_x = ver
+            return self.wp_x
         if self.wp_d is None or self._ver_d != ver:
             self.ensure_buffers(True)
             ops.pack_jobs([(self.wsrc(), self.wp_d, 1, None)], self.wp_d.dtype == torch.bfloat16, self.wp_d.device)
@@ -343,7 +354,16 @@
         ops.conv2d_wgrad(x, dy, w.grad, self.ks, self.stride, workspace(n), dbias=None if b is None else b.grad)
 
     def bwd_x(self, dy: TS, dx: TS, res: Optional[TS] = None, mask: Optional[TS] = None):
-        ops.conv2d_dgrad(dy, self.packed(1), dx, self.ks, self.stride, res=res, mask=mask)
+        wp_x = None
+        if self.ks == 3 and self.stride == 1 and not dy.bf16:
+            t = ops._tuning_ptr()
+            key = (dy.N, dy.H, dy.W, dy.C, dy.cs, dy.co, dx.C, dx.cs, dx.co, None if t is None else bytes(t.contents))
+            want = self._split_want.get(key)
+            if want is None:
+                want = self._split_want[key] = ops.conv2d_dgrad_wants_split(dy, dx, self.ks, self.stride, res=res, mask=mask)
+            if want:
+                wp_x = self.packed(3)
+        ops.conv2d_dgrad(dy, self.packed(1), dx, self.ks, self.stride, res=res, mask=mask, wp_split=wp_x)
 
 
 class _BNExec:
diff --git a/unet_amd/ops.py b/unet_amd/ops.py
--- a/unet_amd/ops.py
+++ b/unet_amd/ops.py
@@ -350,8 +350,16 @@
     d.splitk_ws, d.splitk_ws_floats = buf.data_ptr(), buf.numel()
 
 
-def _launch_conv_part(d: ConvDesc, what: str, alg_flops: float):
+def _launch_conv_part(d: ConvDesc, what: str, alg_flops: float, wp_split: Optional[torch.Tensor] = None):
     _splitk_ws(d)
+    if wp_split is not None and int(lib.unet_conv2d_dgrad_split(C.byref(d))) == 1:
+        wp = d.wp
+        d.wp = wp_split.data_ptr()
+        try:
+            _launch_conv_part(d, what, alg_flops)
+        finally:
+            d.wp = wp
+        return
     pr = CONV_PROBE
     if pr is not None and lib.unet_conv2d_variant(C.byref(d)) % 1000000 == pr.variant:
         e0, e1 = torch.cuda.Event(enable_timing=True), torch.cuda.Event(enable_timing=True)
@@ -372,16 +380,16 @@
     check(lib.unet_conv2d(C.byref(d), _stream()), what)
 
 
-def _launch_conv(d: ConvDesc, what: str, alg_flops: float):
+def _launch_conv(d: ConvDesc, what: str, alg_flops: float, wp_split: Optional[torch.Tensor] = None):
     Co = d.Cout
     r = Co % 128
     if Co > 128 and 0 < r <= 64 and not d.colsum:
         for b, n in ((0, Co - r), (Co - r, r)):
             d.cout_begin, d.cout_count = b, n
-            _launch_conv_part(d, what, alg_flops * n / Co)
+            _launch_conv_part(d, what, alg_flops * n / Co, wp_split)
         d.cout_begin = d.cout_count = 0
         return
-    _launch_conv_part(d, what, alg_flops)
+    _launch_conv_part(d, what, alg_flops, wp_split)
 
 
 def conv2d(x: TS, wp: torch.Tensor, y: TS, ks: int, stride: int = 1, bias=None, res=None, mask=None, relu=False,
@@ -437,9 +445,45 @@
     return int(lib.unet_conv2d_variant(C.byref(d)))
 
 
-def conv2d_dgrad(dy: TS, wp_dgrad: torch.Tensor, dx: TS, ks: int, stride: int = 1, res=None, mask=None, colsum=None):
+_NO_DGRAD_SPLIT = None
+
+
+def _no_dgrad_split_ptr():
+    global _NO_DGRAD_SPLIT
+    cur = getattr(_TUNE, "cur", None)
+    if cur is None:
+        if _NO_DGRAD_SPLIT is None:
+            _NO_DGRAD_SPLIT = L.Tuning.default(dgrad_split=0)
+        return C.pointer(_NO_DGRAD_SPLIT)
+    t = L.Tuning.from_buffer_copy(cur)
+    t.dgrad_split = 0
+    return C.pointer(t)
+
+
+def _dgrad_can_split(dy: TS, ks: int, stride: int) -> bool:
+    return ks == 3 and stride == 1 and not dy.bf16
+
+
+def conv2d_dgrad_wants_split(dy: TS, dx: TS, ks: int, stride: int = 1, res=None, mask=None) -> bool:
+    if not _dgrad_can_split(dy, ks, stride):
+        return False
+    d = _conv_desc(dy, torch.empty(0), dx, ks, stride, L.CONV_DGRAD, None, res, mask, False, None, None)
+    d.wp = 16
+    Co, r = d.Cout, d.Cout % 128
+    parts = ((0, Co - r), (Co - r, r)) if (Co > 128 and 0 < r <= 64) else ((0, 0),)
+    for b, n in parts:
+        d.cout_begin, d.cout_count = b, n
+        if int(lib.unet_conv2d_dgrad_split(C.byref(d))) == 1:
+            return True
+    return False
+
+
+def conv2d_dgrad(dy: TS, wp_dgrad: torch.Tensor, dx: TS, ks: int, stride: int = 1, res=None, mask=None, colsum=None,
+                 wp_split: Optional[torch.Tensor] = None):
     d = _conv_desc(dy, wp_dgrad, dx, ks, stride, L.CONV_DGRAD, None, res, mask, False, colsum, None)
-    _launch_conv(d, "conv2d_dgrad", 2.0 * dy.P * dy.C * dx.C * ks * ks)
+    if _dgrad_can_split(dy, ks, stride) and wp_split is None:
+        d.tuning = _no_dgrad_split_ptr()
+    _launch_conv(d, "conv2d_dgrad", 2.0 * dy.P * dy.C * dx.C * ks * ks, wp_split if _dgrad_can_split(dy, ks, stride) else None)
 
 
 def conv_colsum_rows(x: TS, wp, y: TS, ks, stride, kind) -> int:
```
